# wildltr/ptranking

Measured on AMD Instinct MI355X. Metric: queries/sec fwd+bwd LambdaRank, MSLR-WEB30K-shaped list_len=128, higher is better.
Workload: dtype f32

## Files before the change

include/ptranking_amd.h:

```cpp
#ifndef PTRANKING_AMD_H
#define PTRANKING_AMD_H

#include <stddef.h>
#include <stdint.h>

#ifdef __cplusplus
extern "C" {
#endif

#define PTR_ABI_VERSION 8
#define PTR_MAX_LIST_LEN 4096
#define PTR_MAX_CUTOFFS 32
#define PTR_MAX_SUBTOPICS 32
#define PTR_MLP_ACT_LD 112

#define PTR_ERR_INVALID_ARG 1001
#define PTR_ERR_UNSUPPORTED 1002

#define PTR_LAMBDALOSS_NDCG_LOSS1 0
#define PTR_LAMBDALOSS_NDCG_LOSS2 1
#define PTR_LAMBDALOSS_NDCG_LOSS2PP 2

int ptr_abi_version(void);
const char *ptr_last_error(void);

int ptr_ranknet_fwd_bwd(const float *preds, const float *labels, const int32_t *lens, int B, int L, float sigma,
                        float *loss_out, float *loss_q, float *grad, void *stream);

int ptr_lambdarank_fwd_bwd(const float *preds, const float *labels, const int32_t *lens, int B, int L, float sigma,
                           float *loss_out, float *loss_q, float *grad, void *stream);

int ptr_lambdaloss_fwd_bwd(const float *preds, const float *labels, const int32_t *lens, int B, int L, int k,
                           float sigma, float mu, int loss_type, int presort, float *loss_out, float *loss_q,
                           float *grad, void *stream);

int ptr_softrank_fwd_bwd(const float *preds, const float *labels, const int32_t *lens, int B, int L, float delta, int top_k,
                         float *loss_out, float *loss_q, float *grad, void *stream);

int ptr_approxndcg_fwd_bwd(const float *preds, const float *labels, const int32_t *lens, int B, int L, float alpha,
                           int presort, int couple_batch, float grad_scale_override, float *loss_out, float *dcg_q,
                           float *inv_idcg_q, float *scale_out, float *grad, void *stream);

int ptr_listnet_fwd_bwd(const float *preds, const float *labels, const int32_t *lens, int B, int L, float *loss_out,
                        float *loss_q, float *grad, void *stream);

int ptr_stlistnet_fwd_bwd(const float *preds, const float *labels, const float *unif, const int32_t *lens, int B, int L,
                          float temperature, float *loss_out, float *loss_q, float *grad, void *stream);
int ptr_rankmse_fwd_bwd(const float *preds, const float *labels, const int32_t *lens, int B, int L, float *loss_out,
                        float *loss_q, float *grad, void *stream);
int ptr_rankcosine_fwd_bwd(const float *preds, const float *labels, const int32_t *lens, int B, int L, float *loss_out,
                           float *loss_q, float *grad, void *stream);

int ptr_listmle_fwd_bwd(const float *preds, const int64_t *perm, const int32_t *lens, int B, int L, float *loss_out,
                        float *loss_q, float *grad, void *stream);

int ptr_mdprank_fwd_bwd(const float *preds, const float *labels, const int64_t *perm, const int32_t *lens, int B, int L, int top_k,
                        float gamma, float *loss_out, float *loss_q, float *grad, void *stream);

#define PTR_WASS_COST_P1 0
#define PTR_WASS_COST_P2 1
#define PTR_WASS_COST_EG 2
#define PTR_WASS_COST_DG 3
#define PTR_WASS_COST_DDG 4

int ptr_wassrank_fwd_bwd(const float *preds, const float *labels, const int32_t *lens, int B, int L, int cost_type,
                         float gain_base, float non_rele_gap, float var_penalty, float lam, int sh_itr,
                         int scale_by_max_label, float *loss_out, float *loss_q, float *grad, void *stream);

#define PTR_ADCG_TOPK_SUBTOPICS 0
#define PTR_ADCG_TOPK_DOCUMENTS 1
int ptr_alphadcg_fwd_bwd(const float *preds, const float *rele, const int32_t *lens, const int32_t *ntopics, int B, int T, int L, float rt,
                         float alpha, int top_k, int top_k_axis, float *loss_out, float *loss_q, float *grad, void *stream);
int ptr_div_metrics_at_ks(const float *preds, const float *rele, const int32_t *lens, const int32_t *ntopics, int B, int T, int L,
                          const int32_t *ks, int nk, float alpha, float max_label, float *andcg, float *err_ia, float *nerr_ia,
                          int32_t *valid, void *stream);

#define PTR_DIVPROB_ANDCG 0
#define PTR_DIVPROB_ERRIA 1
#define PTR_DIVPROB_PAIRCLS 2
#define PTR_DIVPROB_LAMBDAPAIRCLS 3
int ptr_divprob_fwd_bwd(const float *mus, const float *vars, const float *rele, const int32_t *lens, const int32_t *ntopics, int B, int T, int L,
                        int objective, float beta, int top_k, int top_k_axis, float max_label, int norm, float *loss_out, float *loss_q,
                        float *grad_mu, float *grad_var, void *stream);
int ptr_divprob_expected_ranks(const float *mus, const float *vars, const int32_t *lens, int B, int L, float *ranks, void *stream);

#define PTR_TREE_PAIRS_ALL 0
#define PTR_TREE_PAIRS_NOTIES 1
#define PTR_TREE_PAIRS_NO00 2
#define PTR_TREE_PAIRS_00 3
#define PTR_TREE_W_NONE 0
#define PTR_TREE_W_DELTA_NDCG 1
#define PTR_TREE_W_DELTA_GAIN 2
#define PTR_TREE_HESS_REFERENCE 0
#define PTR_TREE_HESS_SUM 1
#define PTR_TREE_HESS_CONSTANT 2
#define PTR_TREE_GAIN_POWER 0
#define PTR_TREE_GAIN_LABEL 1
int ptr_tree_pair_grad_hess(const float *preds, const float *labels, const int64_t *offsets, int B, const int32_t *queries, int nq, int max_len,
                            int pair_type, int weighting, float epsilon, int hessian, float *grad, float *hess, void *stream);
int ptr_tree_listnet_grad_hess(const float *preds, const float *labels, const int64_t *offsets, int B, const int32_t *queries, int nq, int max_len,
                               int gain_type, int hessian, float *grad, float *hess, void *stream);

#define PTR_SMOOTH_P 0
#define PTR_SMOOTH_AP 1
#define PTR_SMOOTH_NERR 2
#define PTR_SMOOTH_NDCG 3
int ptr_smoothmetric_fwd_bwd(const float *preds, const float *labels, const int32_t *lens, int B, int L, int metric, int opt_ideal, int top_k,
                             float alpha, float max_label, float *loss_out, float *loss_q, float *valid_q, float *ranks, float *max_label_ws,
                             float *grad, void *stream);

#define PTR_PL_DIST_PL 0
#define PTR_PL_DIST_STPL 1
int ptr_pl_uniforms(int B, int L, int S, uint64_t seed, int64_t q0, float *unif, void *stream);
int ptr_pl_sample(const float *preds, const int32_t *lens, int B, int L, int S, float temperature, int distribution, uint64_t seed, int64_t q0,
                  const float *unif, int64_t *perm, float *action, void *stream);
int ptr_mdprank_sample_fwd_bwd(const float *preds, const float *labels, const int32_t *lens, int B, int L, int S, int top_k, float gamma,
                               float temperature, int distribution, uint64_t seed, int64_t q0, const float *unif, float *loss_out,
                               float *loss_q, float *grad, int64_t *perm_out, void *stream);

int ptr_shuffle_ties_order(const float *labels, const int32_t *lens, int B, int L, uint64_t seed, int64_t *perm,
                           void *stream);

int ptr_sort_desc(const float *preds, const int32_t *lens, int B, int L, float *vals, int64_t *idx, void *stream);

#define PTR_LABEL_MULTILABEL 0
#define PTR_LABEL_PERMUTATION 1
int ptr_metrics_at_ks(const float *preds, const float *labels, const int32_t *lens, int B, int L, const int32_t *ks,
                      int nk, int presort, int label_type, float max_label, float *max_label_ws, float *ndcg, float *nerr,
                      float *ap, float *prec, void *stream);

int ptr_sum_f32(const float *x, int n, float scale, float *out, void *stream);

size_t ptr_mlp_num_params(int F, int NL);
size_t ptr_mlp_backward_ws_floats(int F, int NL);
size_t ptr_mlp_backward_dz_floats(int R, int F, int NL);
size_t ptr_mlp_acts_floats(int R, int NL);
int ptr_mlp_forward(const float *X, const float *params, int R, int F, int NL, int train, float p_drop, uint64_t seed,
                    float *preds, float *acts, void *stream);
int ptr_mlp_backward(const float *X, const float *params, const float *acts, const float *dpreds, int R, int F, int NL,
                     float p_drop, uint64_t seed, float *dz, float *ws, float *grad, void *stream);
#define PTR_OPT_ADAM 1
#define PTR_OPT_ADAGRAD 2
#define PTR_OPT_RMSPROP 3
int ptr_mlp_backward_step(const float *X, float *params, const float *acts, const float *dpreds, int R, int F, int NL, float p_drop,
                          uint64_t seed, float *dz, float *ws, float *grad, int opt_kind, float lr, float hyper1, float hyper2, float eps,
                          float weight_decay, int step, float *state1, float *state2, const float *loss_q, int nq, float *loss_out,
                          void *stream);
int ptr_opt_step_loss(float *params, const float *grad, int64_t n, int opt_kind, float lr, float hyper1, float hyper2, float eps,
                      float weight_decay, int step, float *state1, float *state2, const float *loss_q, int nq, float *loss_out, void *stream);
int ptr_adam_step(float *param, const float *grad, float *exp_avg, float *exp_avg_sq, int64_t n, float lr, float beta1,
                  float beta2, float eps, float weight_decay, int step, void *stream);
int ptr_adagrad_step(float *param, const float *grad, float *state_sum, int64_t n, float lr, float lr_decay, float eps,
                     float weight_decay, int step, void *stream);
int ptr_rmsprop_step(float *param, const float *grad, float *square_avg, int64_t n, float lr, float alpha, float eps,
                     float weight_decay, void *stream);
size_t ptr_mlp_x6_ws_bytes(int F, int NL);
int ptr_mlp_forward_x6(const float *X, const float *params, int R, int F, int NL, int train, float p_drop, uint64_t seed,
                       float *preds, float *acts, void *wimg, void *stream);
#define PTR_LOSS_RANKNET 1
#define PTR_LOSS_LAMBDARANK 2
#define PTR_LOSS_LAMBDALOSS 3
#define PTR_LOSS_LISTNET 4
typedef struct ptr_train_step_desc {
    int32_t struct_bytes;
    int32_t loss_kind;
    int32_t B, L, F, NL;
    int32_t opt_kind, step;
    int32_t loss_i[4];
    float loss_f[4];
    float p_drop, lr, hyper1, hyper2, eps, weight_decay;
    uint64_t seed;
    const float *X, *labels;
    const int32_t *lens;
    float *params, *grad, *state1, *state2;
    float *preds, *acts, *loss_q, *dpreds, *dz, *ws;
    void *wimg;
    float *loss_out;
    void *events[4];
    int32_t wimg_current;
    int32_t reserved;
} ptr_train_step_desc;
int ptr_train_step(const ptr_train_step_desc *d, void *stream);
int ptr_mlp_dropout_mask(int R, int n_feat, int site, float p_drop, uint64_t seed, float *out, void *stream);

#define PTR_LINEAR_NONE 0
#define PTR_LINEAR_RELU 1
#define PTR_LINEAR_RELU_DROPOUT 2
#define PTR_LINEAR_GATE 3
int ptr_linear_forward(const float *X, int ldx, const float *W, const float *bias, int R, int K, int N, int act, float p_drop,
                       uint64_t seed, int site, float *Y, int ldy, void *stream);
int ptr_linear_backward_input(const float *dY, int ldy, const float *W, int R, int K, int N, const float *gate, int ldg, float p_drop,
                              float *dX, int ldx, void *stream);
size_t ptr_linear_backward_weight_ws_floats(int R, int K, int N);
int ptr_linear_backward_weight(const float *X, int ldx, const float *dY, int ldy, int R, int K, int N, float *ws, float *dW, float *db,
                               void *stream);
int ptr_dropout_apply(const float *x, int ldx, int R, int C, float p_drop, uint64_t seed, int site, float *out, int ldo, void *stream);
int ptr_relu_gate(const float *dy, const float *y, int64_t n, float *out, void *stream);

#define PTR_AF_NONE 0
#define PTR_AF_RELU 1
#define PTR_AF_LEAKY 2
#define PTR_AF_ELU 3
#define PTR_AF_SELU 4
#define PTR_AF_GELU 5
#define PTR_AF_SIGMOID 6
#define PTR_AF_TANH 7
size_t ptr_bn_ws_floats(int R, int N, int group_rows);
int ptr_bn_stats(const float *z, int ld, int R, int N, int group_rows, const int32_t *lens, int rows_per_query, float eps, float *ws,
                 float *mean, float *rstd, void *stream);
int ptr_bnact_forward(const float *z, int ld, int R, int N, int group_rows, const int32_t *lens, int rows_per_query, const float *mean,
                      const float *rstd, const float *gamma, const float *beta, int af, float p_drop, uint64_t seed, int site, float *out,
                      void *stream);
int ptr_bnact_backward(const float *z, const float *da, int ld, int R, int N, int group_rows, const int32_t *lens, int rows_per_query,
                       const float *mean, const float *rstd, const float *gamma, const float *beta, int af, float p_drop, uint64_t seed,
                       int site, float *ws, float *dz, float *dgamma, float *dbeta, void *stream);

size_t ptr_bn_slot_floats(int N);
int ptr_bn_stats_partial(const float *z, int ld, int R, int N, int group_rows, const int32_t *lens, int rows_per_query, float *ws,
                         float *slot, void *stream);
int ptr_bn_stats_combine(const float *slots, int W, int slot_stride, int N, float eps, float *mean, float *rstd, float *total_count,
                         void *stream);
int ptr_bnact_backward_sums(const float *z, const float *da, int ld, int R, int N, int group_rows, const int32_t *lens, int rows_per_query,
                            const float *mean, const float *rstd, const float *gamma, const float *beta, int af, float p_drop,
                            uint64_t seed, int site, float *ws, float *sums, void *stream);
int ptr_bnact_backward_apply(const float *z, const float *da, int ld, int R, int N, int group_rows, const int32_t *lens, int rows_per_query,
                             const float *mean, const float *rstd, const float *gamma, const float *beta, int af, float p_drop,
                             uint64_t seed, int site, const float *sums, int W, const float *total_count, float *ws, float *dz,
                             void *stream);

#define PTR_MHSA_MAX_HEAD_DIM 352
int ptr_mhsa_forward(const float *Q, const float *K, const float *V, int ld_qkv, const int32_t *lens, int B, int L, int F,
                     int n_heads, float p_drop, uint64_t seed, int site, float *O, float *lse, void *stream);
int ptr_mhsa_backward(const float *Q, const float *K, const float *V, int ld_qkv, const float *O, const float *dO, const float *lse,
                      const int32_t *lens, int B, int L, int F, int n_heads, float p_drop, uint64_t seed, int site, float *dvec,
                      float *dQ, float *dK, float *dV, float *ds_ws, void *stream);
int ptr_mhsa_dropout_mask(int B, int L, int n_heads, float p_drop, uint64_t seed, int site, float *out, void *stream);
int ptr_layernorm_forward(const float *X, const float *a2, const float *b2, int64_t R, int F, float eps, float *Y, float *stats,
                          void *stream);
size_t ptr_layernorm_backward_ws_floats(int F);
int ptr_layernorm_backward(const float *X, const float *a2, const float *dY, const float *stats, int64_t R, int F, float *ws,
                           float *dX, float *da2, float *db2, void *stream);

int ptr_letor_scan(const char *path, int one_indexed, int64_t *n_docs, int32_t *n_features, int64_t *n_queries);
int ptr_letor_load(const char *path, int one_indexed, float missing, int64_t n_docs, int32_t n_features, int64_t n_queries,
                   void *X, int x_is_f64, float *y, int64_t *qids, int64_t *qoff);

#ifdef __cplusplus
}
#endif
#endif
```

ptranking_amd/_lib.py:

```python
import ctypes as C
import os

import torch

_PKG = os.path.dirname(os.path.abspath(__file__))
LIB_PATH = os.environ.get("PTR_LIB") or os.path.join(_PKG, "libptranking_amd.so")

ABI_VERSION = 8
MAX_LIST_LEN = 4096
MAX_CUTOFFS = 32
MAX_SUBTOPICS = 32

_vp, _i, _f, _u64 = C.c_void_p, C.c_int, C.c_float, C.c_uint64

SIGNATURES = {
    "ptr_abi_version": [],
    "ptr_last_error": [],
    "ptr_ranknet_fwd_bwd": [_vp, _vp, _vp, _i, _i, _f, _vp, _vp, _vp, _vp],
    "ptr_lambdarank_fwd_bwd": [_vp, _vp, _vp, _i, _i, _f, _vp, _vp, _vp, _vp],
    "ptr_lambdaloss_fwd_bwd": [_vp, _vp, _vp, _i, _i, _i, _f, _f, _i, _i, _vp, _vp, _vp, _vp],
    "ptr_approxndcg_fwd_bwd": [_vp, _vp, _vp, _i, _i, _f, _i, _i, _f, _vp, _vp, _vp, _vp, _vp, _vp],
    "ptr_softrank_fwd_bwd": [_vp, _vp, _vp, _i, _i, _f, _i, _vp, _vp, _vp, _vp],
    "ptr_listnet_fwd_bwd": [_vp, _vp, _vp, _i, _i, _vp, _vp, _vp, _vp],
    "ptr_mdprank_fwd_bwd": [_vp, _vp, _vp, _vp, _i, _i, _i, _f, _vp, _vp, _vp, _vp],
    "ptr_listmle_fwd_bwd": [_vp, _vp, _vp, _i, _i, _vp, _vp, _vp, _vp],
    "ptr_stlistnet_fwd_bwd": [_vp, _vp, _vp, _vp, _i, _i, _f, _vp, _vp, _vp, _vp],
    "ptr_rankmse_fwd_bwd": [_vp, _vp, _vp, _i, _i, _vp, _vp, _vp, _vp],
    "ptr_rankcosine_fwd_bwd": [_vp, _vp, _vp, _i, _i, _vp, _vp, _vp, _vp],
    "ptr_wassrank_fwd_bwd": [_vp, _vp, _vp, _i, _i, _i, _f, _f, _f, _f, _i, _i, _vp, _vp, _vp, _vp],
    "ptr_alphadcg_fwd_bwd": [_vp, _vp, _vp, _vp, _i, _i, _i, _f, _f, _i, _i, _vp, _vp, _vp, _vp],
    "ptr_div_metrics_at_ks": [_vp, _vp, _vp, _vp, _i, _i, _i, C.POINTER(C.c_int32), _i, _f, _f, _vp, _vp, _vp, _vp, _vp],
    "ptr_divprob_fwd_bwd": [_vp, _vp, _vp, _vp, _vp, _i, _i, _i, _i, _f, _i, _i, _f, _i, _vp, _vp, _vp, _vp, _vp],
    "ptr_divprob_expected_ranks": [_vp, _vp, _vp, _i, _i, _vp, _vp],
    "ptr_tree_pair_grad_hess": [_vp, _vp, _vp, _i, _vp, _i, _i, _i, _i, _f, _i, _vp, _vp, _vp],
    "ptr_tree_listnet_grad_hess": [_vp, _vp, _vp, _i, _vp, _i, _i, _i, _i, _vp, _vp, _vp],
    "ptr_smoothmetric_fwd_bwd": [_vp, _vp, _vp, _i, _i, _i, _i, _i, _f, _f, _vp, _vp, _vp, _vp, _vp, _vp, _vp],
    "ptr_pl_uniforms": [_i, _i, _i, _u64, C.c_int64, _vp, _vp],
    "ptr_pl_sample": [_vp, _vp, _i, _i, _i, _f, _i, _u64, C.c_int64, _vp, _vp, _vp, _vp],
    "ptr_mdprank_sample_fwd_bwd": [_vp, _vp, _vp, _i, _i, _i, _i, _f, _f, _i, _u64, C.c_int64, _vp, _vp, _vp, _vp, _vp, _vp],
    "ptr_shuffle_ties_order": [_vp, _vp, _i, _i, _u64, _vp, _vp],
    "ptr_sort_desc": [_vp, _vp, _i, _i, _vp, _vp, _vp],
    "ptr_metrics_at_ks": [_vp, _vp, _vp, _i, _i, C.POINTER(C.c_int32), _i, _i, _i, _f, _vp, _vp, _vp, _vp, _vp, _vp],
    "ptr_sum_f32": [_vp, _i, _f, _vp, _vp],
    "ptr_mlp_num_params": [_i, _i],
    "ptr_mlp_backward_ws_floats": [_i, _i],
    "ptr_mlp_backward_dz_floats": [_i, _i, _i],
    "ptr_mlp_acts_floats": [_i, _i],
    "ptr_mlp_forward": [_vp, _vp, _i, _i, _i, _i, _f, _u64, _vp, _vp, _vp],
    "ptr_mlp_backward": [_vp, _vp, _vp, _vp, _i, _i, _i, _f, _u64, _vp, _vp, _vp, _vp],
    "ptr_mlp_backward_step": [_vp, _vp, _vp, _vp, _i, _i, _i, _f, _u64, _vp, _vp, _vp, _i, _f, _f, _f, _f, _f, _i, _vp, _vp, _vp, _i, _vp, _vp],
    "ptr_opt_step_loss": [_vp, _vp, C.c_int64, _i, _f, _f, _f, _f, _f, _i, _vp, _vp, _vp, _i, _vp, _vp],
    "ptr_train_step": [_vp, _vp],
    "ptr_mlp_x6_ws_bytes": [_i, _i],
    "ptr_mlp_forward_x6": [_vp, _vp, _i, _i, _i, _i, _f, _u64, _vp, _vp, _vp, _vp],
    "ptr_adam_step": [_vp, _vp, _vp, _vp, C.c_int64, _f, _f, _f, _f, _f, _i, _vp],
    "ptr_adagrad_step": [_vp, _vp, _vp, C.c_int64, _f, _f, _f, _f, _i, _vp],
    "ptr_rmsprop_step": [_vp, _vp, _vp, C.c_int64, _f, _f, _f, _f, _vp],
    "ptr_mlp_dropout_mask": [_i, _i, _i, _f, _u64, _vp, _vp],
    "ptr_linear_forward": [_vp, _i, _vp, _vp, _i, _i, _i, _i, _f, _u64, _i, _vp, _i, _vp],
    "ptr_linear_backward_input": [_vp, _i, _vp, _i, _i, _i, _vp, _i, _f, _vp, _i, _vp],
    "ptr_linear_backward_weight_ws_floats": [_i, _i, _i],
    "ptr_linear_backward_weight": [_vp, _i, _vp, _i, _i, _i, _i, _vp, _vp, _vp, _vp],
    "ptr_bn_ws_floats": [_i, _i, _i],
    "ptr_bn_stats": [_vp, _i, _i, _i, _i, _vp, _i, _f, _vp, _vp, _vp, _vp],
    "ptr_bnact_forward": [_vp, _i, _i, _i, _i, _vp, _i, _vp, _vp, _vp, _vp, _i, _f, _u64, _i, _vp, _vp],
    "ptr_bnact_backward": [_vp, _vp, _i, _i, _i, _i, _vp, _i, _vp, _vp, _vp, _vp, _i, _f, _u64, _i, _vp, _vp, _vp, _vp, _vp],
    "ptr_bn_slot_floats": [_i],
    "ptr_bn_stats_partial": [_vp, _i, _i, _i, _i, _vp, _i, _vp, _vp, _vp],
    "ptr_bn_stats_combine": [_vp, _i, _i, _i, _f, _vp, _vp, _vp, _vp],
    "ptr_bnact_backward_sums": [_vp, _vp, _i, _i, _i, _i, _vp, _i, _vp, _vp, _vp, _vp, _i, _f, _u64, _i, _vp, _vp, _vp],
    "ptr_bnact_backward_apply": [_vp, _vp, _i, _i, _i, _i, _vp, _i, _vp, _vp, _vp, _vp, _i, _f, _u64, _i, _vp, _i, _vp, _vp, _vp, _vp],
    "ptr_dropout_apply": [_vp, _i, _i, _i, _f, _u64, _i, _vp, _i, _vp],
    "ptr_relu_gate": [_vp, _vp, C.c_int64, _vp, _vp],
    "ptr_mhsa_forward": [_vp, _vp, _vp, _i, _vp, _i, _i, _i, _i, _f, _u64, _i, _vp, _vp, _vp],
    "ptr_mhsa_backward": [_vp, _vp, _vp, _i, _vp, _vp, _vp, _vp, _i, _i, _i, _i, _f, _u64, _i, _vp, _vp, _vp, _vp, _vp, _vp],
    "ptr_mhsa_dropout_mask": [_i, _i, _i, _f, _u64, _i, _vp, _vp],
    "ptr_layernorm_forward": [_vp, _vp, _vp, C.c_int64, _i, _f, _vp, _vp, _vp],
    "ptr_layernorm_backward_ws_floats": [_i],
    "ptr_layernorm_backward": [_vp, _vp, _vp, _vp, C.c_int64, _i, _vp, _vp, _vp, _vp, _vp],
    "ptr_letor_scan": [C.c_char_p, _i, _vp, _vp, _vp],
    "ptr_letor_load": [C.c_char_p, _i, _f, C.c_int64, C.c_int32, C.c_int64, _vp, _i, _vp, _vp, _vp],
}
_RESTYPES = {"ptr_last_error": C.c_char_p, "ptr_mlp_num_params": C.c_size_t, "ptr_mlp_backward_ws_floats": C.c_size_t,
             "ptr_mlp_backward_dz_floats": C.c_size_t, "ptr_mlp_acts_floats": C.c_size_t, "ptr_mlp_x6_ws_bytes": C.c_size_t, "ptr_linear_backward_weight_ws_floats": C.c_size_t, "ptr_bn_ws_floats": C.c_size_t,
             "ptr_bn_slot_floats": C.c_size_t,
             "ptr_layernorm_backward_ws_floats": C.c_size_t}
OPTIONAL = set()

_lib = None


class Loss:

    def __init__(self, entry, kind, params=()):
        self.entry, self.kind, self.params = entry, kind, tuple(params)

    def c_args(self, **values):
        return [C.c_float(float(values[n])) if t is _f else int(values[n]) for n, t in self.params]

    def desc_arrays(self, **values):
        return (tuple(int(values[n]) for n, t in self.params if t is _i), tuple(C.c_float(float(values[n])).value for n, t in self.params if t is _f))


LOSSES = {
    "ranknet": Loss("ptr_ranknet_fwd_bwd", 1, [("sigma", _f)]),
    "lambdarank": Loss("ptr_lambdarank_fwd_bwd", 2, [("sigma", _f)]),
    "lambdaloss": Loss("ptr_lambdaloss_fwd_bwd", 3, [("k", _i), ("sigma", _f), ("mu", _f), ("loss_type", _i), ("presort", _i)]),
    "listnet": Loss("ptr_listnet_fwd_bwd", 4),
}


class TrainStepDesc(C.Structure):
    _fields_ = [("struct_bytes", C.c_int32), ("loss_kind", C.c_int32),
                ("B", C.c_int32), ("L", C.c_int32), ("F", C.c_int32), ("NL", C.c_int32),
                ("opt_kind", C.c_int32), ("step", C.c_int32),
                ("loss_i", C.c_int32 * 4), ("loss_f", C.c_float * 4),
                ("p_drop", C.c_float), ("lr", C.c_float), ("hyper1", C.c_float), ("hyper2", C.c_float), ("eps", C.c_float), ("weight_decay", C.c_float),
                ("seed", C.c_uint64),
                ("X", C.c_void_p), ("labels", C.c_void_p), ("lens", C.c_void_p),
                ("params", C.c_void_p), ("grad", C.c_void_p), ("state1", C.c_void_p), ("state2", C.c_void_p),
                ("preds", C.c_void_p), ("acts", C.c_void_p), ("loss_q", C.c_void_p), ("dpreds", C.c_void_p), ("dz", C.c_void_p), ("ws", C.c_void_p),
                ("wimg", C.c_void_p), ("loss_out", C.c_void_p), ("events", C.c_void_p * 4), ("wimg_current", C.c_int32), ("reserved", C.c_int32)]


class NativeLibraryError(RuntimeError):
    pass


def load():
    global _lib
    if _lib is not None:
        return _lib
    if not os.path.exists(LIB_PATH):
        raise NativeLibraryError(
            f"{LIB_PATH} is missing: build the HIP extension first (python -m ptranking_amd.build, or "
            f"__graft_entry__.build()).  ptranking_amd has no CPU / eager fallback by design.")
    lib = C.CDLL(LIB_PATH, mode=C.RTLD_GLOBAL)
    for name, argtypes in SIGNATURES.items():
        try:
            fn = getattr(lib, name)
        except AttributeError:
            if name in OPTIONAL:
                continue
            raise NativeLibraryError(f"{LIB_PATH} does not export {name}; rebuild it")
        fn.argtypes = argtypes
        fn.restype = _RESTYPES.get(name, C.c_int)
    v = lib.ptr_abi_version()
    if v != ABI_VERSION:
        raise NativeLibraryError(f"ABI version mismatch: library {v}, binding {ABI_VERSION}")
    _lib = lib
    return lib


def has(name):
    return hasattr(load(), name)


TIMING = None


def query(name, *args):
    return getattr(load(), name)(*args)


def call(name, *args):
    lib = load()
    if TIMING is not None:
        ev0, ev1 = torch.cuda.Event(enable_timing=True), torch.cuda.Event(enable_timing=True)
        ev0.record()
        rc = getattr(lib, name)(*args)
        ev1.record()
        TIMING.setdefault(name, []).append((ev0, ev1))
    else:
        rc = getattr(lib, name)(*args)
    if rc != 0:
        msg = lib.ptr_last_error()
        raise RuntimeError(f"{name} failed (code {rc}): {msg.decode() if msg else ''}")


def ptr(t):
    return None if t is None else C.c_void_p(t.data_ptr())


def current_stream(device):
    return C.c_void_p(torch.cuda.current_stream(device).cuda_stream)
```

ptranking_amd/csrc/ptr_mlp.h:

```cpp
#pragma once
#include <stdlib.h>
#include <utility>

#include "ptr_device.h"
#include "ptr_dropout.h"
#include "ptr_x6.h"

namespace ptr {

constexpr int kH = 100;
constexpr int kHP = 112;
constexpr int kMT = 7;
constexpr int kMaxLayers = 8;
constexpr int kAL = 112;
constexpr int kActTile = 16 * kAL;
__host__ __device__ inline int act_row_tiles(int R) { return (R + 15) >> 4; }
__host__ __device__ inline size_t act_layer_floats(int R) { return (size_t)act_row_tiles(R) * kActTile; }
__host__ __device__ inline size_t act_off(int row, int col) {
    return (size_t)(row >> 4) * kActTile + (size_t)(((col >> 4) << 8) + ((row & 15) << 4) + (col & 15));
}

__host__ __device__ inline size_t off_W(int l, int F) { return l == 0 ? 0 : (size_t)kH * F + kH + (size_t)(l - 1) * (kH * kH + kH); }
__host__ __device__ inline size_t off_b(int l, int F) { return off_W(l, F) + (l == 0 ? (size_t)kH * F : (size_t)kH * kH); }
__host__ __device__ inline size_t off_wout(int NL, int F) { return off_W(NL, F); }
__host__ __device__ inline size_t n_params(int NL, int F) { return off_wout(NL, F) + kH + 1; }

struct MlpArgs {
    int R, F, NL;
    float p_drop;
    uint32_t seed_lo, seed_hi;
};

constexpr int kX6Rows = kHP;
constexpr int kX6PlaneBytes = kX6Rows * 32 * 2;
constexpr int kX6SliceBytes = 3 * kX6PlaneBytes;
__host__ __device__ inline int x6_n1(int F) { return (F + 31) / 32; }
__host__ __device__ inline int x6_nslices(int F, int NL) { return x6_n1(F) + 4 * (NL - 1); }
#if defined(__HIPCC__)
__device__ __forceinline__ void x6_img_put(uint8_t *__restrict__ img, int F, int NL, size_t i, float x) {
    const size_t w1 = (size_t)kH * F;
    int sl, row, g, e;
    if (i < w1) {
        row = (int)(i / F);
        const int k = (int)(i - (size_t)row * F), kk = k & 31;
        sl = k >> 5; g = kk >> 3; e = kk & 7;
    } else {
        if (i < w1 + kH) return;
        const size_t jv = i - (w1 + kH);
        const int l = 1 + (int)(jv / (kH * kH + kH));
        if (l > NL - 1) return;
        const int jj = (int)(jv - (size_t)(l - 1) * (kH * kH + kH));
        int k;
        if (jj < kH * kH) { row = jj / kH; k = jj - row * kH; } else { row = jj - kH * kH; k = kH; }
        const int kk = k & 31;
        sl = x6_n1(F) + 4 * (l - 1) + (k >> 5);
        g = (kk & 15) >> 2; e = 4 * (kk >> 4) + (kk & 3);
    }
    uint16_t p1, p2, p3;
    split_pack1(x, p1, p2, p3);
    uint8_t *at = img + (size_t)sl * kX6SliceBytes + (size_t)(row >> 4) * 1024 + g * 256 + (row & 15) * 16 + e * 2;
    *reinterpret_cast<uint16_t *>(at) = p1;
    *reinterpret_cast<uint16_t *>(at + kX6PlaneBytes) = p2;
    *reinterpret_cast<uint16_t *>(at + 2 * kX6PlaneBytes) = p3;
}
#endif

template <int N, class Fn> __device__ __forceinline__ void static_for(Fn &&f) {
    [&]<int... I>(std::integer_sequence<int, I...>) { (f(std::integral_constant<int, I>{}), ...); }(std::make_integer_sequence<int, N>{});
}

bool bwd_fused_supported(int F, int NL, const void *X, const void *acts);
int bwd_fused_grid(int R);
int launch_bwd_fused(const float *X, const float *params, const float *acts, const float *dpreds, const MlpArgs &a, float *ws,
                     hipStream_t st, const char *who);

bool bwd_tail_supported(int NL, const void *acts);
int launch_bwd_tail(const float *params, const float *acts, const float *dpreds, const MlpArgs &a, float *ws, float *dz0, hipStream_t st,
                    const char *who);

bool bwd_x6_supported(int R, int F, int NL, const void *X, const void *acts);
int launch_bwd_x6(const float *X, const float *params, const float *acts, const float *dpreds, const MlpArgs &a, float *ws, hipStream_t st,
                  const char *who);

bool bwd_x6_tail_supported(int R, int NL, const void *acts);
int launch_bwd_x6_tail(const float *params, const float *acts, const float *dpreds, const MlpArgs &a, float *ws, float *dz0, hipStream_t st,
                       const char *who);

bool dw_x6_supported(int R, int K, int lda, const void *A);
int launch_dw_x6(const float *A, int lda, const float *dZ, int K, int ntk, const MlpArgs &a, float *ws, size_t np_stride, size_t w_off, size_t b_off,
                 int nblk, hipStream_t st, const char *who);

int mlp_forward_x6_impl(const float *X, const float *params, int R, int F, int NL, int train, float p_drop, uint64_t seed, float *preds, float *acts,
                        void *wimg, bool prep, void *stream);
int mlp_backward_step_impl(const float *X, float *params, const float *acts, const float *dpreds, int R, int F, int NL, float p_drop, uint64_t seed, float *dz,
                           float *ws, float *grad, int opt_kind, float lr, float hyper1, float hyper2, float eps, float weight_decay, int step, float *state1,
                           float *state2, const float *loss_q, int nq, float *loss_out, void *wimg, void *stream);

}
```

ptranking_amd/csrc/scorer.hip:

```cpp
#include "ptr_mlp.h"

namespace ptr {

__host__ __device__ inline int ld_w1(int F) { return (F + 3) / 4 * 4 + 4; }


constexpr int kTailNone = 0, kTailSpread = 1, kTailReplicate = 2;
__device__ __forceinline__ void stage_matrix(float *dst, int ld, const float *src, int rows, int cols, bool transpose, int tid, int nthr,
                                             int tail = kTailNone) {
    constexpr int U = 8;
    const int n = rows * cols;
    const bool vec = ((cols & 3) == 0) && ((reinterpret_cast<uintptr_t>(src) & 15) == 0);
    const int reps = tail == kTailReplicate ? 4 : 1;
    if (vec) {
        const int n4 = n >> 2;
        for (int base = tid; base < n4; base += U * nthr) {
            f32x4 v[U];
#pragma unroll
            for (int u = 0; u < U; ++u) {
                const int i4 = base + u * nthr;
                v[u] = *reinterpret_cast<const f32x4 *>(src + 4 * (size_t)(i4 < n4 ? i4 : n4 - 1));
            }
#pragma unroll
            for (int u = 0; u < U; ++u) {
                const int i4 = base + u * nthr;
                if (i4 < n4) {
                    const int idx = 4 * i4, r = idx / cols, c = idx - r * cols;
                    if (!transpose) {
                        for (int rep = 0; rep < (r >= 96 ? reps : 1); ++rep) *reinterpret_cast<f32x4 *>(dst + (size_t)(r + 4 * rep) * ld + c) = v[u];
                    } else {
#pragma unroll
                        for (int e = 0; e < 4; ++e) dst[(size_t)(c + e) * ld + r] = v[u][e];
                    }
                }
            }
        }
    } else {
        for (int base = tid; base < n; base += U * nthr) {
            float v[U];
#pragma unroll
            for (int u = 0; u < U; ++u) { const int idx = base + u * nthr; v[u] = src[idx < n ? idx : n - 1]; }
#pragma unroll
            for (int u = 0; u < U; ++u) {
                const int idx = base + u * nthr;
                if (idx < n) {
                    const int r = idx / cols, c = idx - r * cols;
                    if (transpose) dst[(size_t)c * ld + r] = v[u];
                    else for (int rep = 0; rep < (r >= 96 ? reps : 1); ++rep) dst[(size_t)(r + 4 * rep) * ld + c] = v[u];
                }
            }
        }
    }
    const int vr = transpose ? cols : rows, vc = transpose ? rows : cols;
    for (int idx = tid; idx < kHP * ld; idx += nthr) {
        const int r = idx / ld, c = idx - r * ld;
        const bool real_row = (tail == kTailReplicate && r >= 96) ? 96 + ((r - 96) & 3) < vr : r < vr;
        if (!real_row || c >= vc) dst[idx] = 0.0f;
    }
}
__device__ __forceinline__ void stage_vector(float *dst, const float *src, int n, int tid, int nthr, int tail = kTailNone) {
    for (int i = tid; i < kHP; i += nthr) {
        if (tail != kTailSpread || i < 96) dst[i] = i < n ? src[i] : 0.0f;
        else dst[i] = (((i - 96) & 3) == 0 && 96 + ((i - 96) >> 2) < n) ? src[96 + ((i - 96) >> 2)] : 0.0f;
    }
}

constexpr int kSlabK = 48, kSlabLd = kSlabK + 4;
__host__ __device__ inline size_t fwd_lds_floats(int F, int NL, int w1_mode) {
    const size_t w1 = w1_mode == 0 ? (size_t)kHP * ld_w1(F) : (w1_mode == 2 ? (size_t)2 * kHP * kSlabLd : 0);
    return w1 + (size_t)(NL - 1) * kHP * kH + (size_t)NL * kHP + kHP + 16;
}
__host__ __device__ inline int fwd_w1_mode(int F, int NL) {
    if (fwd_lds_floats(F, NL, 0) * sizeof(float) <= 160 * 1024) return 0;
    return fwd_lds_floats(F, NL, 2) * sizeof(float) <= 160 * 1024 ? 2 : 1;
}

#ifdef PTR_FWD_TRACE
#define FWD_STAMP(i) do { if (blockIdx.x == 0 && lane == 0 && ntile_done < 8) { unsigned long long *tr_ = reinterpret_cast<unsigned long long *>(preds + ((R + 3) & ~3) + 4) + (ntile_done * 16 + wave) * 8; tr_[(i)] = clock64(); if ((i) == 0) tr_[4] = wall_clock64(); if ((i) == 3) tr_[5] = wall_clock64(); } } while (0)
#else
#define FWD_STAMP(i) do { } while (0)
#endif

template <int RT, int NTHR, bool TRAIN, bool VEC, int W1G>
__global__ void __launch_bounds__(NTHR)
mlp_fwd_kernel(const float *__restrict__ X, const float *__restrict__ P, MlpArgs a, float *__restrict__ preds,
               float *__restrict__ acts) {
    extern __shared__ __attribute__((aligned(16))) float smem[];
    const int F = a.F, NL = a.NL, R = a.R, ld1 = ld_w1(F), R16 = act_row_tiles(a.R) * 16;
    float *W1s = smem;
    float *Wh = W1s + (W1G == 0 ? (size_t)kHP * ld1 : (W1G == 2 ? (size_t)2 * kHP * kSlabLd : 0));
    float *Bs = Wh + (size_t)(NL - 1) * kHP * kH;
    float *Wo = Bs + (size_t)NL * kHP;
    const int tid = threadIdx.x, nthr = blockDim.x;
    if constexpr (W1G == 0) stage_matrix(W1s, ld1, P + off_W(0, F), kH, F, false, tid, nthr, kTailReplicate);
    for (int l = 1; l < NL; ++l) stage_matrix(Wh + (size_t)(l - 1) * kHP * kH, kH, P + off_W(l, F), kH, kH, false, tid, nthr, kTailReplicate);
    for (int l = 0; l < NL; ++l) stage_vector(Bs + (size_t)l * kHP, P + off_b(l, F), kH, tid, nthr);
    stage_vector(Wo, P + off_wout(NL, F), kH, tid, nthr, kTailSpread);
    if (tid < 16) Wo[kHP + tid] = tid == 0 ? P[off_wout(NL, F) + kH] : 0.0f;
    __syncthreads();
    const float b_out = Wo[kHP];

    const int lane = tid & 63, j = lane & 15, g = lane >> 4;
    const int wpb = nthr >> 6, wave = tid >> 6;
    const int rows_per_tile = 16 * RT;
    const int ntiles = (R + rows_per_tile - 1) / rows_per_tile;
    const uint32_t thr = drop_thr(a.p_drop);
    const float scale = TRAIN ? 1.0f / (1.0f - a.p_drop) : 1.0f;
    const int nS1 = (F + 15) >> 4;

    int ntile_done = 0;
    (void)ntile_done;
    auto prefetch_first = [&](int t, f32x4 (&xb)[RT]) {
        const int tt = t < ntiles ? t : ntiles - 1;
        const int k0 = 4 * g;
#pragma unroll
        for (int rt = 0; rt < RT; ++rt) {
            const int r = tt * rows_per_tile + 16 * rt + j;
            const float *xr = X + (size_t)(r < R ? r : R - 1) * F;
            if constexpr (VEC) {
                xb[rt] = *reinterpret_cast<const f32x4 *>(xr + (k0 < F ? k0 : 0));
            } else {
#pragma unroll
                for (int c = 0; c < 4; ++c) xb[rt][c] = xr[k0 + c < F ? k0 + c : 0];
            }
        }
    };
    f32x4 xpre[RT];
    constexpr bool kQueue = W1G != 2;
    const int tiles_per_block = (ntiles + gridDim.x - 1) / gridDim.x;
    const int tile_lo = kQueue ? blockIdx.x * tiles_per_block : 0, tile_hi = kQueue ? min(ntiles, tile_lo + tiles_per_block) : ntiles;
    int *queue = reinterpret_cast<int *>(Wo + kHP + 8);
    int tile = blockIdx.x * wpb + wave;
    if constexpr (kQueue) {
        if (tid == 0) *queue = tile_lo + wpb;
        __syncthreads();
        tile = tile_lo + wave;
    }
    constexpr int kSlabV = kHP * (kSlabK / 4);
    constexpr int kSlabU = (kSlabV + NTHR - 1) / NTHR;
    f32x4 slab_r[W1G == 2 ? kSlabU : 1];
    int slab_buf = 0;
    auto slab_load = [&](int sl) {
        if constexpr (W1G == 2) {
#pragma unroll
            for (int u = 0; u < kSlabU; ++u) {
                const int i4 = tid + u * NTHR, r = i4 / (kSlabK / 4), c = 4 * (i4 - r * (kSlabK / 4));
                const int wr = r < 96 ? r : 96 + ((r - 96) & 3), k = kSlabK * sl + c;
                slab_r[u] = *reinterpret_cast<const f32x4 *>(P + (size_t)(wr < kHP ? wr : 0) * F + (k < F ? k : 0));
            }
        }
    };
    auto slab_store = [&](int sl, int buf) {
        if constexpr (W1G == 2) {
#pragma unroll
            for (int u = 0; u < kSlabU; ++u) {
                const int i4 = tid + u * NTHR, r = i4 / (kSlabK / 4), c = 4 * (i4 - r * (kSlabK / 4));
                const bool real = kSlabK * sl + c < F;
                f32x4 v = slab_r[u];
                if (!real) v = f32x4{0.f, 0.f, 0.f, 0.f};
                if (i4 < kSlabV) *reinterpret_cast<f32x4 *>(W1s + (size_t)buf * kHP * kSlabLd + (size_t)r * kSlabLd + c) = v;
            }
        }
    };
    if constexpr (W1G == 2) { slab_load(0); slab_store(0, 0); }
    prefetch_first(tile, xpre);
    for (; (kQueue ? tile : tile - wave) < tile_hi; ++ntile_done) {
        int next_tile = tile_hi;
        auto advance = [&]() {
            if constexpr (kQueue) {
                int nxt = 0;
                if (lane == 0) nxt = atomicAdd(queue, 1);
                next_tile = __builtin_amdgcn_readfirstlane(nxt);
            } else {
                next_tile = tile + gridDim.x * wpb;
            }
            prefetch_first(next_tile, xpre);
        };
        const int row0 = tile * rows_per_tile;
        const bool tile_full = row0 + rows_per_tile <= R;
        int row[RT];
#pragma unroll
        for (int rt = 0; rt < RT; ++rt) row[rt] = row0 + 16 * rt + j;
        FWD_STAMP(0);

        const float *xrow[RT];
        bool rok[RT];
#pragma unroll
        for (int rt = 0; rt < RT; ++rt) {
            rok[rt] = row[rt] < R;
            xrow[rt] = X + (size_t)(rok[rt] ? row[rt] : R - 1) * F;
        }
        auto load_raw = [&](int S, f32x4 (&xb)[RT]) {
            const int k0 = 16 * S + 4 * g;
#pragma unroll
            for (int rt = 0; rt < RT; ++rt) {
                if constexpr (VEC) {
                    xb[rt] = *reinterpret_cast<const f32x4 *>(xrow[rt] + (k0 < F ? k0 : 0));
                } else {
#pragma unroll
                    for (int c = 0; c < 4; ++c) xb[rt][c] = xrow[rt][k0 + c < F ? k0 + c : 0];
                }
            }
        };
        auto finish_x = [&](int S, f32x4 (&xb)[RT]) {
            const int k0 = 16 * S + 4 * g;
#pragma unroll
            for (int rt = 0; rt < RT; ++rt) {
                f32x4 v = xb[rt];
                if (16 * S + 16 > F || !tile_full) {
#pragma unroll
                    for (int c = 0; c < 4; ++c) v[c] *= ((k0 + c < F) && rok[rt]) ? 1.0f : 0.0f;
                }
                if constexpr (TRAIN) {
                    uint32_t w0, w1;
                    drop_bits(a.seed_lo, a.seed_hi, 0, row[rt], k0 >> 2, w0, w1);
                    v = drop4(v, w0, w1, thr, scale);
                }
                xb[rt] = v;
            }
        };

        auto tail_store = [&](float v, float ones) -> f32x4 {
            const float h1 = __shfl(v, j + 16, 64), h2 = __shfl(v, j + 32, 64), h3 = __shfl(v, j + 48, 64);
            f32x4 o = f32x4{g == 1 ? ones : 0.0f, 0.0f, 0.0f, 0.0f};
            if (g == 0) o = f32x4{v, h1, h2, h3};
            return o;
        };
        auto mma = [&](auto mt_, float aop, float bop, f32x4 c) -> f32x4 {
            if constexpr (decltype(mt_)::value == kMT - 1) return __builtin_amdgcn_mfma_f32_4x4x1f32(aop, bop, c, 0, 0, 0);
            else return __builtin_amdgcn_mfma_f32_16x16x4f32(aop, bop, c, 0, 0, 0);
        };
        f32x4 acc[kMT][RT];
        auto tile6_finish = [&]() {
#pragma unroll
            for (int rt = 0; rt < RT; ++rt) {
                f32x4 t = acc[kMT - 1][rt];
#pragma unroll
                for (int c = 0; c < 4; ++c) { t[c] += __shfl_xor(t[c], 16, 64); t[c] += __shfl_xor(t[c], 32, 64); }
                acc[kMT - 1][rt][0] = g == 0 ? t[0] : (g == 1 ? t[1] : (g == 2 ? t[2] : t[3]));
            }
        };
        auto mma_tiles = [&](const f32x4 (&wa)[kMT], const f32x4 (&b)[RT], int nc) {
            auto one = [&]<int MT>(std::integral_constant<int, MT> mt_, int c) {
#pragma unroll
                for (int rt = 0; rt < RT; ++rt) acc[MT][rt] = mma(mt_, wa[MT][c], b[rt][c], acc[MT][rt]);
            };
            using std::integral_constant;
#pragma unroll
            for (int c = 0; c < 4; ++c) if (c < nc) { one(integral_constant<int, 0>{}, c); one(integral_constant<int, 1>{}, c); }
#pragma unroll
            for (int c = 0; c < 4; ++c) if (c < nc) { one(integral_constant<int, 2>{}, c); one(integral_constant<int, 3>{}, c); }
#pragma unroll
            for (int c = 0; c < 4; ++c) if (c < nc) { one(integral_constant<int, 4>{}, c); one(integral_constant<int, 5>{}, c); one(integral_constant<int, 6>{}, c); }
        };
        auto bias_init = [&](const float *b) {
#pragma unroll
            for (int mt = 0; mt < kMT; ++mt) {
                f32x4 b4 = *reinterpret_cast<const f32x4 *>(b + (mt < kMT - 1 ? 16 * mt + 4 * g : 96));
                if (mt == kMT - 1) { const float on = g == 0 ? 1.0f : 0.0f; b4 = b4 * on; }
#pragma unroll
                for (int rt = 0; rt < RT; ++rt) acc[mt][rt] = b4;
            }
        };
        bias_init(Bs);
        f32x4 xa[RT], xb[RT], xc[RT];
#pragma unroll
        for (int rt = 0; rt < RT; ++rt) xa[rt] = xpre[rt];
        if (NL == 1) advance();
        finish_x(0, xa);
        auto read_w1 = [&](int S, int sin, int mt) -> f32x4 {
            const int k0 = 16 * S + 4 * g;
            if constexpr (W1G == 2) {
                return *reinterpret_cast<const f32x4 *>(W1s + (size_t)slab_buf * kHP * kSlabLd + (size_t)(16 * mt + j) * kSlabLd + 16 * sin + 4 * g);
            } else if constexpr (W1G == 1) {
                const int wr = mt < kMT - 1 ? 16 * mt + j : 96 + (j & 3);
                return *reinterpret_cast<const f32x4 *>(P + (size_t)wr * F + (k0 < F ? k0 : 0));
            } else {
                return *reinterpret_cast<const f32x4 *>(W1s + (size_t)(16 * mt + j) * ld1 + k0);
            }
        };
        auto l1_step = [&](int S, int sin, f32x4 (&cur)[RT], f32x4 (&nxt)[RT], f32x4 (&nn)[RT]) {
            load_raw(S + 2 < nS1 ? S + 2 : 0, nn);
            __builtin_amdgcn_sched_barrier(0);
            f32x4 wa[kMT];
#pragma unroll
            for (int mt = 0; mt < kMT; ++mt) wa[mt] = read_w1(S, sin, mt);
            if constexpr (RT > 1) __builtin_amdgcn_sched_barrier(0);
            mma_tiles(wa, cur, 4);
            finish_x(S + 1, nxt);
        };
        auto slab_enter = [&](int S) {
            if constexpr (W1G == 2) {
                __syncthreads();
                slab_load(S + 3 < nS1 ? S / 3 + 1 : 0);
            }
        };
        auto slab_leave = [&](int S) {
            if constexpr (W1G == 2) {
                slab_store(S + 3 < nS1 ? S / 3 + 1 : 0, slab_buf ^ 1);
                slab_buf ^= 1;
            }
        };
        load_raw(nS1 > 1 ? 1 : 0, xb);
        int S1 = 0;
        for (; S1 + 3 <= nS1; S1 += 3) {
            slab_enter(S1);
            l1_step(S1, 0, xa, xb, xc);
            l1_step(S1 + 1, 1, xb, xc, xa);
            l1_step(S1 + 2, 2, xc, xa, xb);
            slab_leave(S1);
        }
        const int left = nS1 - S1;
        if (left == 0) {
        } else if (left == 1) {
            slab_enter(S1);
            l1_step(S1, 0, xa, xb, xc);
            slab_leave(S1);
        } else {
            slab_enter(S1);
            l1_step(S1, 0, xa, xb, xc);
            l1_step(S1 + 1, 1, xb, xc, xa);
            slab_leave(S1);
        }
        tile6_finish();

        FWD_STAMP(1);
        for (int l = 1; l < NL; ++l) {
            f32x4 hin[kMT][RT];
#pragma unroll
            for (int mt = 0; mt < kMT; ++mt)
#pragma unroll
                for (int rt = 0; rt < RT; ++rt) {
                    f32x4 h = acc[mt][rt];
#pragma unroll
                    for (int c = 0; c < 4; ++c) h[c] = fmaxf(h[c], 0.0f);
                    if constexpr (TRAIN) {
                        if (mt < kMT - 1) {
                            uint32_t w0, w1;
                            drop_bits(a.seed_lo, a.seed_hi, l, row[rt], 4 * mt + g, w0, w1);
                            h = drop4(h, w0, w1, thr, scale);
                        } else {
                            h[0] *= drop_keep1(a.seed_lo, a.seed_hi, l, row[rt], 96 + g, thr) ? scale : 0.0f;
                        }
                    }
                    hin[mt][rt] = h;
                }
            if (l == NL - 1) advance();
            const float *Wl = Wh + (size_t)(l - 1) * kHP * kH;
            bias_init(Bs + (size_t)l * kHP);
#pragma unroll
            for (int S = 0; S < kMT; ++S) {
                constexpr int kLast = kMT - 1;
                f32x4 wa[kMT];
#pragma unroll
                for (int mt = 0; mt < kMT; ++mt) {
                    const float *wp = Wl + (size_t)(16 * mt + j) * kH;
                    if (S < kLast) wa[mt] = *reinterpret_cast<const f32x4 *>(wp + 16 * S + 4 * g);
                    else wa[mt] = f32x4{wp[96 + g], 0.0f, 0.0f, 0.0f};
                }
                if constexpr (RT > 1) __builtin_amdgcn_sched_barrier(0);
                if constexpr (TRAIN) {
#pragma unroll
                    for (int rt = 0; rt < RT; ++rt) {
                        if (row[rt] < R16) {
                            float *arow = acts + (size_t)(l - 1) * act_layer_floats(R) + act_off(row[rt], 0);
                            *reinterpret_cast<f32x4 *>(arow + 256 * S + 4 * g) = S < kLast ? hin[S][rt] : tail_store(hin[S][rt][0], 1.0f);
                        }
                    }
                    if constexpr (RT > 1) __builtin_amdgcn_sched_barrier(0);
                }
                mma_tiles(wa, hin[S], S < kLast ? 4 : 1);
            }
            tile6_finish();
        }

        FWD_STAMP(2);
        float sc[RT];
#pragma unroll
        for (int rt = 0; rt < RT; ++rt) sc[rt] = 0.0f;
#pragma unroll
        for (int mt = 0; mt < kMT; ++mt) {
            const f32x4 w4 = *reinterpret_cast<const f32x4 *>(Wo + 16 * mt + 4 * g);
#pragma unroll
            for (int rt = 0; rt < RT; ++rt) {
                f32x4 h = acc[mt][rt];
#pragma unroll
                for (int c = 0; c < (mt == kMT - 1 ? 1 : 4); ++c) { h[c] = fmaxf(h[c], 0.0f); sc[rt] = fmaf(h[c], w4[c], sc[rt]); }
                if constexpr (TRAIN) {
                    if (row[rt] < R16) {
                        float *arow = acts + (size_t)(NL - 1) * act_layer_floats(R) + act_off(row[rt], 0);
                        *reinterpret_cast<f32x4 *>(arow + 256 * mt + 4 * g) = mt < kMT - 1 ? h : tail_store(h[0], 0.0f);
                    }
                }
            }
        }
#pragma unroll
        for (int rt = 0; rt < RT; ++rt) {
            float s = sc[rt];
            s += __shfl_xor(s, 16, 64);
            s += __shfl_xor(s, 32, 64);
            if (g == 0 && row[rt] < R) preds[row[rt]] = s + b_out;
        }
        FWD_STAMP(3);
        tile = next_tile;
    }
}

__host__ __device__ inline size_t dz_lds_floats(int NL) { return (size_t)(NL - 1) * kHP * kH + (kHP + 16) + 16 * (kHP + 16); }

template <int RT, int NTHR>
__global__ void __launch_bounds__(NTHR)
mlp_bwd_dz_kernel(const float *__restrict__ P, const float *__restrict__ acts, const float *__restrict__ dpreds, MlpArgs a,
                  float *__restrict__ dz, float *__restrict__ ws, size_t np_stride, size_t wout_off) {
    extern __shared__ __attribute__((aligned(16))) float smem[];
    const int F = a.F, NL = a.NL, R = a.R;
    float *WT = smem;
    float *Wo = WT + (size_t)(NL - 1) * kHP * kH;
    float *wrow = Wo + kHP + 16;
    const int tid = threadIdx.x, nthr = blockDim.x;
    for (int l = 1; l < NL; ++l) stage_matrix(WT + (size_t)(l - 1) * kHP * kH, kH, P + off_W(l, F), kH, kH, true, tid, nthr);
    stage_vector(Wo, P + off_wout(NL, F), kH, tid, nthr);
    if (tid < 16) Wo[kHP + tid] = 0.0f;
    __syncthreads();

    const int lane = tid & 63, j = lane & 15, g = lane >> 4;
    const int wpb = nthr >> 6, wave = tid >> 6;
    const int rows_per_tile = 16 * RT;
    const int ntiles = (R + rows_per_tile - 1) / rows_per_tile;
    const float inv_keep = a.p_drop > 0.0f ? 1.0f / (1.0f - a.p_drop) : 1.0f;

    f32x4 dwo[kMT];
#pragma unroll
    for (int mt = 0; mt < kMT; ++mt) dwo[mt] = f32x4{0.f, 0.f, 0.f, 0.f};
    float dbo = 0.0f;

    f32x4 hpf[kMT][RT];
    float dspf[RT];
    auto prefetch_top = [&](int tile) {
#pragma unroll
        for (int rt = 0; rt < RT; ++rt) {
            const int r = tile * rows_per_tile + 16 * rt + j;
            const int rc = r < R ? r : R - 1;
            dspf[rt] = dpreds[rc];
#pragma unroll
            for (int mt = 0; mt < kMT; ++mt)
                hpf[mt][rt] = *reinterpret_cast<const f32x4 *>(acts + (size_t)(NL - 1) * act_layer_floats(R) + act_off(rc, 16 * mt + 4 * g));
        }
    };
    const int tile_first = blockIdx.x * wpb + wave, tile_step = gridDim.x * wpb;
    if (tile_first < ntiles) prefetch_top(tile_first);
    for (int tile = tile_first; tile < ntiles; tile += tile_step) {
        const int row0 = tile * rows_per_tile;
        int row[RT];
        float ds[RT];
        f32x4 htop[kMT][RT];
#pragma unroll
        for (int rt = 0; rt < RT; ++rt) {
            row[rt] = row0 + 16 * rt + j;
            ds[rt] = dspf[rt] * (row[rt] < R ? 1.0f : 0.0f);
            if (g == 0) dbo += ds[rt];
#pragma unroll
            for (int mt = 0; mt < kMT; ++mt) htop[mt][rt] = hpf[mt][rt];
        }
        if (tile + tile_step < ntiles) prefetch_top(tile + tile_step);
        f32x4 cur[kMT][RT];
#pragma unroll
        for (int mt = 0; mt < kMT; ++mt) {
            const f32x4 w4 = *reinterpret_cast<const f32x4 *>(Wo + 16 * mt + 4 * g);
#pragma unroll
            for (int rt = 0; rt < RT; ++rt) {
                const bool ok = row[rt] < R;
                const size_t o = ((size_t)(NL - 1) * R + row[rt]) * kAL + 16 * mt + 4 * g;
                f32x4 h = htop[mt][rt];
                const float okf = ok ? 1.0f : 0.0f;
#pragma unroll
                for (int c = 0; c < 4; ++c) h[c] *= okf;
                f32x4 d;
#pragma unroll
                for (int c = 0; c < 4; ++c) { d[c] = (ds[rt] * w4[c]) * (h[c] > 0.0f ? 1.0f : 0.0f); dwo[mt][c] = fmaf(h[c], ds[rt], dwo[mt][c]); }
                if (ok) *reinterpret_cast<f32x4 *>(dz + o) = d;
                cur[mt][rt] = d;
            }
        }
        for (int l = NL - 1; l >= 1; --l) {
            const float *Wl = WT + (size_t)(l - 1) * kHP * kH;
            f32x4 gate[kMT][RT];
#pragma unroll
            for (int mt = 0; mt < kMT; ++mt)
#pragma unroll
                for (int rt = 0; rt < RT; ++rt) {
                    const bool ok = row[rt] < R;
                    const size_t o = (size_t)(l - 1) * act_layer_floats(R) + act_off(row[rt], 16 * mt + 4 * g);
                    gate[mt][rt] = *reinterpret_cast<const f32x4 *>(acts + (ok ? o : 0));
                }
            f32x4 acc[kMT][RT];
#pragma unroll
            for (int mt = 0; mt < kMT; ++mt)
#pragma unroll
                for (int rt = 0; rt < RT; ++rt) acc[mt][rt] = f32x4{0.f, 0.f, 0.f, 0.f};
#pragma unroll
            for (int S = 0; S < kMT; ++S) {
                f32x4 wa[kMT];
#pragma unroll
                for (int mt = 0; mt < kMT; ++mt) wa[mt] = *reinterpret_cast<const f32x4 *>(Wl + (size_t)(16 * mt + j) * kH + 16 * S + 4 * g);
                auto group = [&](int m0, int m1) {
#pragma unroll
                    for (int c = 0; c < 4; ++c)
#pragma unroll
                        for (int mt = m0; mt < m1; ++mt)
#pragma unroll
                            for (int rt = 0; rt < RT; ++rt)
                                acc[mt][rt] = __builtin_amdgcn_mfma_f32_16x16x4f32(wa[mt][c], cur[S][rt][c], acc[mt][rt], 0, 0, 0);
                };
                group(0, 2); group(2, 4); group(4, kMT);
            }
#pragma unroll
            for (int mt = 0; mt < kMT; ++mt)
#pragma unroll
                for (int rt = 0; rt < RT; ++rt) {
                    const bool ok = row[rt] < R;
                    const size_t o = ((size_t)(l - 1) * R + row[rt]) * kAL + 16 * mt + 4 * g;
                    f32x4 d;
#pragma unroll
                    for (int c = 0; c < 4; ++c) d[c] = acc[mt][rt][c] * ((ok && gate[mt][rt][c] > 0.0f) ? inv_keep : 0.0f);
                    if (ok) *reinterpret_cast<f32x4 *>(dz + o) = d;
                    cur[mt][rt] = d;
                }
        }
    }
#pragma unroll
    for (int mt = 0; mt < kMT; ++mt)
#pragma unroll
        for (int c = 0; c < 4; ++c) {
            float v = dwo[mt][c];
            v += __shfl_xor(v, 1, 64); v += __shfl_xor(v, 2, 64); v += __shfl_xor(v, 4, 64); v += __shfl_xor(v, 8, 64);
            if (j == 0) wrow[(size_t)wave * (kHP + 16) + 16 * mt + 4 * g + c] = v;
        }
    {
        float v = dbo;
        v += __shfl_xor(v, 1, 64); v += __shfl_xor(v, 2, 64); v += __shfl_xor(v, 4, 64); v += __shfl_xor(v, 8, 64);
        if (lane == 0) wrow[(size_t)wave * (kHP + 16) + kHP] = v;
    }
    __syncthreads();
    for (int i = tid; i < kH + 1; i += nthr) {
        const int src = i < kH ? i : kHP;
        float s = 0.0f;
        for (int w = 0; w < wpb; ++w) s += wrow[(size_t)w * (kHP + 16) + src];
        ws[(size_t)blockIdx.x * np_stride + wout_off + i] = s;
    }
}

template <int NTW, bool SITE0, int NWV>
__global__ void __launch_bounds__(NWV * 64)
mlp_bwd_dw_kernel(const float *__restrict__ A, int lda, const float *__restrict__ dZ, int K, int nt_base, MlpArgs a,
                  float *__restrict__ ws, size_t np_stride, size_t w_off, size_t b_off) {
    const int R = a.R;
    const int tid = threadIdx.x, lane = tid & 63, j = lane & 15, g = lane >> 4, wave = tid >> 6;
    constexpr int U = 4;
    const int chunk = ((R + gridDim.x - 1) / gridDim.x + 4 * U - 1) / (4 * U) * (4 * U);
    const int r_begin = blockIdx.x * chunk, r_end = min(R, r_begin + chunk);
    const uint32_t thr = drop_thr(a.p_drop);
    const float scale = (SITE0 && a.p_drop > 0.0f) ? 1.0f / (1.0f - a.p_drop) : 1.0f;
    const int ntk = (K + 15) >> 4;
    (void)ntk;

    f32x4 acc[NTW][kMT];
#pragma unroll
    for (int t = 0; t < NTW; ++t)
#pragma unroll
        for (int mt = 0; mt < kMT; ++mt) acc[t][mt] = f32x4{0.f, 0.f, 0.f, 0.f};
    float dbv[kMT];
#pragma unroll
    for (int mt = 0; mt < kMT; ++mt) dbv[mt] = 0.0f;

    int fa[kMT], kb[NTW];
    bool fa_ok[kMT], kb_ok[NTW];
#pragma unroll
    for (int mt = 0; mt < kMT; ++mt) { const int f = 16 * mt + j; fa_ok[mt] = true; fa[mt] = f; }
#pragma unroll
    for (int t = 0; t < NTW; ++t) { const int k = 16 * (nt_base + wave + NWV * t) + j; kb_ok[t] = k < K; kb[t] = kb_ok[t] ? k : 0; }
    float av[U][kMT], bv[U][NTW], avn[U][kMT], bvn[U][NTW];
    auto load = [&](int r0, bool guard, float (&pa)[U][kMT], float (&pb)[U][NTW]) {
#pragma unroll
        for (int u = 0; u < U; ++u) {
            const int r = r0 + 4 * u + g;
            const bool rok = !guard || r < r_end;
            const int rc = rok ? r : r_end - 1;
            const float *dzr = dZ + (size_t)rc * kAL;
            const float *ar = SITE0 ? A + (size_t)rc * lda : A + act_off(rc, 0);
#pragma unroll
            for (int mt = 0; mt < kMT; ++mt) pa[u][mt] = dzr[fa[mt]] * ((rok & fa_ok[mt]) ? 1.0f : 0.0f);
#pragma unroll
            for (int t = 0; t < NTW; ++t) {
                float v = SITE0 ? ar[kb[t]] : ar[((kb[t] >> 4) << 8) + (kb[t] & 15)];
                bool keep = rok & kb_ok[t];
                if constexpr (SITE0) keep = keep & drop_keep1(a.seed_lo, a.seed_hi, 0, rc, kb[t], thr);
                pb[u][t] = v * (keep ? scale : 0.0f);
            }
        }
    };
    auto mma = [&]() {
#pragma unroll
        for (int u = 0; u < U; ++u) {
#pragma unroll
            for (int mt = 0; mt < kMT; ++mt) dbv[mt] += av[u][mt];
#pragma unroll
            for (int t = 0; t < NTW; ++t)
#pragma unroll
                for (int mt = 0; mt < kMT; ++mt)
                    acc[t][mt] = __builtin_amdgcn_mfma_f32_16x16x4f32(av[u][mt], bv[u][t], acc[t][mt], 0, 0, 0);
        }
    };
    const int n_full = r_end > r_begin ? (r_end - r_begin) / (4 * U) : 0;
    int r0 = r_begin;
    if (n_full > 0) {
        load(r0, false, av, bv);
        for (int it = 0; it < n_full; ++it, r0 += 4 * U) {
            if (it + 1 < n_full) load(r0 + 4 * U, false, avn, bvn);
            mma();
#pragma unroll
            for (int u = 0; u < U; ++u) {
#pragma unroll
                for (int mt = 0; mt < kMT; ++mt) av[u][mt] = avn[u][mt];
#pragma unroll
                for (int t = 0; t < NTW; ++t) bv[u][t] = bvn[u][t];
            }
        }
    }
    if (r0 < r_end) { load(r0, true, av, bv); mma(); }
    float *out = ws + (size_t)blockIdx.x * np_stride + w_off;
    float *outb = ws + (size_t)blockIdx.x * np_stride + b_off;
#pragma unroll
    for (int t = 0; t < NTW; ++t) {
        const int nt = nt_base + wave + NWV * t, k = 16 * nt + j;
#pragma unroll
        for (int mt = 0; mt < kMT; ++mt)
#pragma unroll
            for (int c = 0; c < 4; ++c) {
                const int o = 16 * mt + 4 * g + c;
                if (nt < ntk && k < K && o < kH) out[(size_t)o * K + k] = acc[t][mt][c];
            }
    }
    if (wave == 0 && nt_base == 0) {
#pragma unroll
        for (int mt = 0; mt < kMT; ++mt) {
            float v = dbv[mt];
            v += __shfl_xor(v, 16, 64);
            v += __shfl_xor(v, 32, 64);
            const int f = 16 * mt + j;
            if (g == 0 && f < kH) outb[f] = v;
        }
    }
}

template <int NTW, bool SITE0, int RB>
__global__ void __launch_bounds__(256)
mlp_bwd_dw_lds_kernel(const float *__restrict__ A, int lda, const float *__restrict__ dZ, int K, int nt_base, MlpArgs a,
                      float *__restrict__ ws, size_t np_stride, size_t w_off, size_t b_off) {
    constexpr int WA4 = 16 * NTW;
    constexpr int LDA = 64 * NTW + 16;
    constexpr int LDZ = kAL;
    constexpr int SA = RB * WA4 / 256;
    constexpr int SZ = (RB * (kAL / 4) + 255) / 256;
    extern __shared__ __attribute__((aligned(16))) float smem[];
    auto zb = [&](int b) -> float * { return smem + b * (RB * LDZ); };
    auto ab = [&](int b) -> float * { return smem + 2 * RB * LDZ + b * (RB * LDA); };

    const int R = a.R;
    const int tid = threadIdx.x, lane = tid & 63, j = lane & 15, g = lane >> 4, wave = tid >> 6;
    const int chunk = ((R + gridDim.x - 1) / gridDim.x + RB - 1) / RB * RB;
    const int r_begin = blockIdx.x * chunk, r_end = min(R, r_begin + chunk);
    const uint32_t thr = drop_thr(a.p_drop);
    const float scale = (SITE0 && a.p_drop > 0.0f) ? 1.0f / (1.0f - a.p_drop) : 1.0f;
    const int col0 = 16 * nt_base;

    int a_row[SA], a_col[SA], z_row[SZ], z_col[SZ];
    bool a_ok[SA], z_ok[SZ];
#pragma unroll
    for (int s_ = 0; s_ < SA; ++s_) {
        const int idx = s_ * 256 + tid;
        a_row[s_] = idx / WA4;
        a_col[s_] = col0 + 4 * (idx % WA4);
        a_ok[s_] = a_col[s_] < K;
    }
#pragma unroll
    for (int s_ = 0; s_ < SZ; ++s_) {
        const int idx = s_ * 256 + tid;
        z_ok[s_] = idx < RB * (kAL / 4);
        z_row[s_] = z_ok[s_] ? idx / (kAL / 4) : 0;
        z_col[s_] = z_ok[s_] ? 4 * (idx % (kAL / 4)) : 0;
    }
    f32x4 ra[SA], rz[SZ];
    auto gload = [&](int r0) {
#pragma unroll
        for (int s_ = 0; s_ < SA; ++s_) {
            const int r = r0 + a_row[s_];
            const int rc = r < r_end ? r : r_end - 1;
            const int cc = a_ok[s_] ? a_col[s_] : 0;
            ra[s_] = *reinterpret_cast<const f32x4 *>(SITE0 ? A + (size_t)rc * lda + cc : A + act_off(rc, cc));
        }
#pragma unroll
        for (int s_ = 0; s_ < SZ; ++s_) {
            const int r = r0 + z_row[s_];
            const int rc = r < r_end ? r : r_end - 1;
            rz[s_] = *reinterpret_cast<const f32x4 *>(dZ + (size_t)rc * kAL + z_col[s_]);
        }
    };
    auto lstore = [&](int buf, int r0) {
#pragma unroll
        for (int s_ = 0; s_ < SA; ++s_) {
            const int r = r0 + a_row[s_];
            const bool rok = r < r_end;
            f32x4 v = ra[s_];
            if constexpr (SITE0) {
                uint32_t w0, w1;
                drop_bits(a.seed_lo, a.seed_hi, 0, rok ? r : r_end - 1, a_col[s_] >> 2, w0, w1);
                v = drop4(v, w0, w1, thr, scale);
            }
            const float okf = (rok & a_ok[s_]) ? 1.0f : 0.0f;
#pragma unroll
            for (int c = 0; c < 4; ++c) v[c] *= okf;
            *reinterpret_cast<f32x4 *>(ab(buf) + a_row[s_] * LDA + (a_col[s_] - col0)) = v;
        }
#pragma unroll
        for (int s_ = 0; s_ < SZ; ++s_) {
            if (z_ok[s_]) {
                const float okf = (r0 + z_row[s_] < r_end) ? 1.0f : 0.0f;
                f32x4 v = rz[s_];
#pragma unroll
                for (int c = 0; c < 4; ++c) v[c] *= okf;
                *reinterpret_cast<f32x4 *>(zb(buf) + z_row[s_] * LDZ + z_col[s_]) = v;
            }
        }
    };

    f32x4 acc[NTW][kMT];
#pragma unroll
    for (int t = 0; t < NTW; ++t)
#pragma unroll
        for (int mt = 0; mt < kMT; ++mt) acc[t][mt] = f32x4{0.f, 0.f, 0.f, 0.f};
    float dbv[kMT];
#pragma unroll
    for (int mt = 0; mt < kMT; ++mt) dbv[mt] = 0.0f;

    if (r_begin < r_end) {
        gload(r_begin);
        lstore(0, r_begin);
    }
    __syncthreads();
    int buf = 0;
    for (int r0 = r_begin; r0 < r_end; r0 += RB, buf ^= 1) {
        const bool more = r0 + RB < r_end;
        if (more) gload(r0 + RB);
        const float *zs = zb(buf), *as = ab(buf);
#pragma unroll
        for (int u = 0; u < RB / 4; ++u) {
            float av[kMT], bv[NTW];
#pragma unroll
            for (int mt = 0; mt < kMT; ++mt) { av[mt] = zs[(4 * u + g) * LDZ + 16 * mt + j]; dbv[mt] += av[mt]; }
#pragma unroll
            for (int t = 0; t < NTW; ++t) bv[t] = as[(4 * u + g) * LDA + 16 * (wave + 4 * t) + j];
#pragma unroll
            for (int t = 0; t < NTW; ++t)
#pragma unroll
                for (int mt = 0; mt < kMT; ++mt)
                    acc[t][mt] = __builtin_amdgcn_mfma_f32_16x16x4f32(av[mt], bv[t], acc[t][mt], 0, 0, 0);
        }
        if (more) lstore(buf ^ 1, r0 + RB);
        __syncthreads();
    }
    float *out = ws + (size_t)blockIdx.x * np_stride + w_off;
    float *outb = ws + (size_t)blockIdx.x * np_stride + b_off;
#pragma unroll
    for (int t = 0; t < NTW; ++t) {
        const int k = col0 + 16 * (wave + 4 * t) + j;
#pragma unroll
        for (int mt = 0; mt < kMT; ++mt)
#pragma unroll
            for (int c = 0; c < 4; ++c) {
                const int o = 16 * mt + 4 * g + c;
                if (k < K && o < kH) out[(size_t)o * K + k] = acc[t][mt][c];
            }
    }
    if (wave == 0 && nt_base == 0) {
#pragma unroll
        for (int mt = 0; mt < kMT; ++mt) {
            float v = dbv[mt];
            v += __shfl_xor(v, 16, 64);
            v += __shfl_xor(v, 32, 64);
            const int f = 16 * mt + j;
            if (g == 0 && f < kH) outb[f] = v;
        }
    }
}
__host__ __device__ constexpr size_t dw_lds_bytes(int NTW, int RB) { return (size_t)(2 * RB * kAL + 2 * RB * (64 * NTW + 16)) * sizeof(float); }

struct OptStep {
    int kind;
    float lr, h1, h2, eps, wd, bc1, bc2_sqrt;
    float *param, *s1, *s2;
    const float *loss_q; int nq; float *loss_out;
    uint8_t *wimg; int F, NL;
};
__global__ void __launch_bounds__(1024)
reduce_partials_kernel(const float *__restrict__ ws, int nblk, int nblk_tail, size_t tail_begin, size_t stride, size_t n,
                       float *__restrict__ grad, OptStep o) {
    __shared__ float part[16][64];
    const int lane = threadIdx.x & 63, w = threadIdx.x >> 6;
    if (o.loss_out && blockIdx.x == gridDim.x - 1) {
        const float tot = block1024_sum(o.loss_q, o.nq, &part[0][0]);
        if (threadIdx.x == 0) o.loss_out[0] = tot;
        return;
    }
    const size_t i = (size_t)blockIdx.x * 64 + lane;
    const bool ok = i < n;
    const size_t ic = ok ? i : n - 1;
    const int nb = ic >= tail_begin ? nblk_tail : nblk;
    float s0 = 0.f, s1 = 0.f, s2 = 0.f, s3 = 0.f;
    int b = w;
    for (; b + 48 < nb; b += 64) {
        s0 += ws[(size_t)b * stride + ic];
        s1 += ws[(size_t)(b + 16) * stride + ic];
        s2 += ws[(size_t)(b + 32) * stride + ic];
        s3 += ws[(size_t)(b + 48) * stride + ic];
    }
    for (; b < nb; b += 16) s0 += ws[(size_t)b * stride + ic];
    part[w][lane] = (s0 + s1) + (s2 + s3);
    __syncthreads();
    if (w == 0 && ok) {
        float s = part[0][lane];
#pragma unroll
        for (int k = 1; k < 16; ++k) s += part[k][lane];
        if (grad) grad[i] = s;
        if (o.kind == PTR_OPT_ADAM) {
            const float pi = o.param[i];
            const float gi = s + o.wd * pi;
            const float mi = o.h1 * o.s1[i] + (1.0f - o.h1) * gi;
            const float vi = o.h2 * o.s2[i] + (1.0f - o.h2) * gi * gi;
            o.s1[i] = mi; o.s2[i] = vi;
            const float denom = sqrtf(vi) / o.bc2_sqrt + o.eps;
            const float pn = pi - (o.lr / o.bc1) * (mi / denom);
            o.param[i] = pn;
            if (o.wimg) x6_img_put(o.wimg, o.F, o.NL, i, pn);
        } else if (o.kind == PTR_OPT_ADAGRAD) {
            const float pi = o.param[i];
            const float gi = s + o.wd * pi;
            const float si = o.s1[i] + gi * gi;
            o.s1[i] = si;
            const float pn = pi - o.lr * (gi / (sqrtf(si) + o.eps));
            o.param[i] = pn;
            if (o.wimg) x6_img_put(o.wimg, o.F, o.NL, i, pn);
        } else if (o.kind == PTR_OPT_RMSPROP) {
            const float pi = o.param[i];
            const float gi = s + o.wd * pi;
            const float si = o.h1 * o.s1[i] + (1.0f - o.h1) * gi * gi;
            o.s1[i] = si;
            const float pn = pi - o.lr * (gi / (sqrtf(si) + o.eps));
            o.param[i] = pn;
            if (o.wimg) x6_img_put(o.wimg, o.F, o.NL, i, pn);
        }
    }
}

__global__ void __launch_bounds__(256)
adam_kernel(float *__restrict__ p, const float *__restrict__ grad, float *__restrict__ m, float *__restrict__ v, size_t n, float lr,
            float b1, float b2, float eps, float wd, float bc1, float bc2_sqrt) {
    const size_t i = (size_t)blockIdx.x * 256 + threadIdx.x;
    if (i >= n) return;
    const float pi = p[i];
    const float gi = grad[i] + wd * pi;
    const float mi = b1 * m[i] + (1.0f - b1) * gi;
    const float vi = b2 * v[i] + (1.0f - b2) * gi * gi;
    m[i] = mi; v[i] = vi;
    const float denom = sqrtf(vi) / bc2_sqrt + eps;
    p[i] = pi - (lr / bc1) * (mi / denom);
}

__global__ void __launch_bounds__(256)
dropout_mask_kernel(MlpArgs a, int site, int n_feat, float *__restrict__ out) {
    const size_t i = (size_t)blockIdx.x * 256 + threadIdx.x;
    if (i >= (size_t)a.R * n_feat) return;
    const int row = (int)(i / n_feat), k = (int)(i % n_feat);
    out[i] = drop_keep1(a.seed_lo, a.seed_hi, site, row, k, drop_thr(a.p_drop)) ? 1.0f : 0.0f;
}

static int check_mlp(const char *who, int R, int F, int NL, float p) {
    if (R < 0 || F <= 0 || NL < 1 || NL > kMaxLayers) { set_error("%s: bad shape R=%d F=%d NL=%d", who, R, F, NL); return PTR_ERR_INVALID_ARG; }
    if (!(p >= 0.0f && p < 1.0f)) { set_error("%s: dropout p=%g out of [0,1)", who, (double)p); return PTR_ERR_INVALID_ARG; }
    const int w1g = fwd_w1_mode(F, NL);
    if (fwd_lds_floats(F, NL, w1g) * sizeof(float) > 160 * 1024 || (w1g && F % 4 != 0) || (F + 15) / 16 > 48) {
        set_error("%s: F=%d with %d hidden layers is outside the fused scorer's range (LDS %zu KB, max 160; F %% 4 == 0 needed "
                  "above ~157 features; F <= 768)", who, F, NL, fwd_lds_floats(F, NL, w1g) * sizeof(float) / 1024);
        return PTR_ERR_UNSUPPORTED;
    }
    return 0;
}

constexpr int kDwBlocksPerCu = 2;
constexpr int kDwRB = 16;

}

extern "C" size_t ptr_mlp_num_params(int F, int NL) { return ptr::n_params(NL, F); }

extern "C" size_t ptr_mlp_backward_ws_floats(int F, int NL) {
    return (size_t)ptr::kDwBlocksPerCu * ptr::num_cus() * ptr::n_params(NL, F);
}

extern "C" size_t ptr_mlp_acts_floats(int R, int NL) { return R > 0 && NL > 0 ? (size_t)NL * ptr::act_layer_floats(R) : 0; }
extern "C" size_t ptr_mlp_backward_dz_floats(int R, int F, int NL) {
    return ptr::bwd_fused_supported(F, NL, nullptr, nullptr) ? 0 : (size_t)NL * (size_t)R * ptr::kAL;
}

extern "C" int ptr_mlp_forward(const float *X, const float *params, int R, int F, int NL, int train, float p_drop, uint64_t seed,
                               float *preds, float *acts, void *stream) {
    using namespace ptr;
    const char *who = "ptr_mlp_forward";
    if (int rc = check_mlp(who, R, F, NL, p_drop)) return rc;
    if (R > 0 && (!X || !params || !preds || (train && !acts))) { set_error("%s: NULL pointer", who); return PTR_ERR_INVALID_ARG; }
    if (R == 0) return 0;
    MlpArgs a{R, F, NL, train ? p_drop : 0.0f, (uint32_t)seed, (uint32_t)(seed >> 32)};
    const int w1g = fwd_w1_mode(F, NL);
    const size_t lds = fwd_lds_floats(F, NL, w1g) * sizeof(float);
    const bool vec = (F % 4 == 0) && ((reinterpret_cast<uintptr_t>(X) & 15) == 0);
    const bool wide = train && !w1g;
    const int rows_per_tile = wide ? 16 : 32, wpb = wide ? 16 : 8;
    const int ntiles = (R + rows_per_tile - 1) / rows_per_tile;
    const int grid = ntiles < num_cus() ? ntiles : num_cus();
    auto launch = [&](auto kern) -> int {
        if (int e = allow_lds(kern, lds)) return e;
        hipLaunchKernelGGL(kern, dim3(grid > 0 ? grid : 1), dim3(wpb * 64), lds, as_stream(stream), X, params, a, preds, acts);
        return check_hip(hipGetLastError(), who);
    };
    if (w1g) {
        if (!vec) { set_error("%s: X must be 16-byte aligned for F=%d", who, F); return PTR_ERR_INVALID_ARG; }
        if (w1g == 2 && !env_int("PTR_FWD_W1_STREAM", 0))
            return train ? launch(mlp_fwd_kernel<2, 512, true, true, 2>) : launch(mlp_fwd_kernel<2, 512, false, true, 2>);
        return train ? launch(mlp_fwd_kernel<2, 512, true, true, 1>) : launch(mlp_fwd_kernel<2, 512, false, true, 1>);
    }
    if (wide) return vec ? launch(mlp_fwd_kernel<1, 1024, true, true, 0>) : launch(mlp_fwd_kernel<1, 1024, true, false, 0>);
    return vec ? launch(mlp_fwd_kernel<2, 512, false, true, 0>) : launch(mlp_fwd_kernel<2, 512, false, false, 0>);
}

namespace ptr {
int mlp_backward_impl(const char *who, const float *X, const float *params, const float *acts, const float *dpreds, int R, int F, int NL,
                             float p_drop, uint64_t seed, float *dz, float *ws, float *grad, void *stream, const OptStep &opt);
}
extern "C" int ptr_mlp_backward(const float *X, const float *params, const float *acts, const float *dpreds, int R, int F, int NL,
                                float p_drop, uint64_t seed, float *dz, float *ws, float *grad, void *stream) {
    return ptr::mlp_backward_impl("ptr_mlp_backward", X, params, acts, dpreds, R, F, NL, p_drop, seed, dz, ws, grad, stream, ptr::OptStep{});
}

extern "C" int ptr_mlp_backward_step(const float *X, float *params, const float *acts, const float *dpreds, int R, int F, int NL, float p_drop,
                                     uint64_t seed, float *dz, float *ws, float *grad, int opt_kind, float lr, float hyper1, float hyper2,
                                     float eps, float weight_decay, int step, float *state1, float *state2, const float *loss_q, int nq,
                                     float *loss_out, void *stream) {
    return ptr::mlp_backward_step_impl(X, params, acts, dpreds, R, F, NL, p_drop, seed, dz, ws, grad, opt_kind, lr, hyper1, hyper2, eps, weight_decay, step, state1,
                                       state2, loss_q, nq, loss_out, nullptr, stream);
}

int ptr::mlp_backward_step_impl(const float *X, float *params, const float *acts, const float *dpreds, int R, int F, int NL, float p_drop, uint64_t seed,
                                float *dz, float *ws, float *grad, int opt_kind, float lr, float hyper1, float hyper2, float eps, float weight_decay, int step,
                                float *state1, float *state2, const float *loss_q, int nq, float *loss_out, void *wimg, void *stream) {
    using namespace ptr;
    const char *who = "ptr_mlp_backward_step";
    if (opt_kind < PTR_OPT_ADAM || opt_kind > PTR_OPT_RMSPROP) { set_error("%s: unknown optimiser %d", who, opt_kind); return PTR_ERR_INVALID_ARG; }
    if (step < 1 || !state1 || (opt_kind == PTR_OPT_ADAM && !state2) || (loss_out && nq > 0 && !loss_q) || nq < 0) {
        set_error("%s: bad optimiser / loss arguments", who);
        return PTR_ERR_INVALID_ARG;
    }
    OptStep o{};
    o.kind = opt_kind; o.h1 = hyper1; o.h2 = hyper2; o.eps = eps; o.wd = weight_decay;
    o.param = params; o.s1 = state1; o.s2 = state2; o.loss_q = loss_q; o.nq = nq; o.loss_out = loss_out;
    o.wimg = reinterpret_cast<uint8_t *>(wimg); o.F = F; o.NL = NL;
    if (opt_kind == PTR_OPT_ADAM) {
        o.lr = lr; o.bc1 = 1.0f - powf(hyper1, (float)step); o.bc2_sqrt = sqrtf(1.0f - powf(hyper2, (float)step));
    } else if (opt_kind == PTR_OPT_ADAGRAD) {
        o.lr = lr / (1.0f + (float)(step - 1) * hyper1);
    } else {
        o.lr = lr;
    }
    return mlp_backward_impl(who, X, params, acts, dpreds, R, F, NL, p_drop, seed, dz, ws, grad, stream, o);
}

extern "C" int ptr_opt_step_loss(float *params, const float *grad, int64_t n, int opt_kind, float lr, float hyper1, float hyper2, float eps,
                                 float weight_decay, int step, float *state1, float *state2, const float *loss_q, int nq, float *loss_out,
                                 void *stream) {
    using namespace ptr;
    const char *who = "ptr_opt_step_loss";
    if (opt_kind < PTR_OPT_ADAM || opt_kind > PTR_OPT_RMSPROP) { set_error("%s: unknown optimiser %d", who, opt_kind); return PTR_ERR_INVALID_ARG; }
    if (n < 0 || step < 1 || nq < 0 || (n > 0 && (!params || !grad || !state1 || (opt_kind == PTR_OPT_ADAM && !state2))) || (loss_out && nq > 0 && !loss_q)) {
        set_error("%s: bad optimiser / loss arguments", who);
        return PTR_ERR_INVALID_ARG;
    }
    if (n == 0 && !loss_out) return 0;
    OptStep o{};
    o.kind = opt_kind; o.h1 = hyper1; o.h2 = hyper2; o.eps = eps; o.wd = weight_decay;
    o.param = params; o.s1 = state1; o.s2 = state2; o.loss_q = loss_q; o.nq = nq; o.loss_out = loss_out;
    if (opt_kind == PTR_OPT_ADAM) { o.lr = lr; o.bc1 = 1.0f - powf(hyper1, (float)step); o.bc2_sqrt = sqrtf(1.0f - powf(hyper2, (float)step)); }
    else if (opt_kind == PTR_OPT_ADAGRAD) o.lr = lr / (1.0f + (float)(step - 1) * hyper1);
    else o.lr = lr;
    const size_t nn = (size_t)n;
    hipLaunchKernelGGL(reduce_partials_kernel, dim3((unsigned)((nn + 63) / 64) + (loss_out ? 1 : 0)), dim3(1024), 0, as_stream(stream), grad, 1, 1, nn,
                       nn, nn, (float *)nullptr, o);
    return check_hip(hipGetLastError(), who);
}

int ptr::mlp_backward_impl(const char *who, const float *X, const float *params, const float *acts, const float *dpreds, int R, int F, int NL,
                                  float p_drop, uint64_t seed, float *dz, float *ws, float *grad, void *stream, const OptStep &opt) {
    using namespace ptr;
    if (int rc = check_mlp(who, R, F, NL, p_drop)) return rc;
    if (!X || !params || !acts || !dpreds || !ws || !grad) { set_error("%s: NULL pointer", who); return PTR_ERR_INVALID_ARG; }
    hipStream_t st = as_stream(stream);
    MlpArgs a{R, F, NL, p_drop, (uint32_t)seed, (uint32_t)(seed >> 32)};
    if (R > 0 && bwd_fused_supported(F, NL, X, acts)) {
        if (int e = bwd_x6_supported(R, F, NL, X, acts) ? launch_bwd_x6(X, params, acts, dpreds, a, ws, st, who)
                                                        : launch_bwd_fused(X, params, acts, dpreds, a, ws, st, who)) return e;
        const int nb = bwd_fused_grid(R);
        const size_t NPf = n_params(NL, F);
        hipLaunchKernelGGL(reduce_partials_kernel, dim3((unsigned)((NPf + 63) / 64) + (opt.loss_out ? 1 : 0)), dim3(1024), 0, st, ws, nb, nb, NPf, NPf, NPf,
                           grad, opt);
        return check_hip(hipGetLastError(), who);
    }
    if (!dz) { set_error("%s: dz scratch is required for this configuration (ptr_mlp_backward_dz_floats)", who); return PTR_ERR_INVALID_ARG; }
    const int ncu = num_cus();
    const int nblk = kDwBlocksPerCu * ncu;
    const size_t NP = n_params(NL, F);
    constexpr int wpb = 8;
    const int ntiles = (R + 15) / 16;
    int grid_dz = ntiles < wpb * ncu ? (ntiles + wpb - 1) / wpb : ncu;
    if (grid_dz < 1) grid_dz = 1;
    const bool tail = R > 0 && bwd_tail_supported(NL, acts);
    if (tail) {
        if (int e = bwd_x6_tail_supported(R, NL, acts) ? launch_bwd_x6_tail(params, acts, dpreds, a, ws, dz, st, who)
                                                       : launch_bwd_tail(params, acts, dpreds, a, ws, dz, st, who)) return e;
    } else {
        const size_t lds = dz_lds_floats(NL) * sizeof(float);
        auto go = [&](auto kern) -> int {
            if (int e = allow_lds(kern, lds)) return e;
            hipLaunchKernelGGL(kern, dim3(grid_dz), dim3(wpb * 64), lds, st, params, acts, dpreds, a, dz, ws, NP, off_wout(NL, F));
            return check_hip(hipGetLastError(), who);
        };
        if (int e = go(mlp_bwd_dz_kernel<1, 512>)) return e;
    }
    for (int l = 0; l < (tail ? 1 : NL); ++l) {
        const int K = l == 0 ? F : kH;
        const float *A = l == 0 ? X : acts + (size_t)(l - 1) * act_layer_floats(R);
        const int lda = l == 0 ? F : kAL;
        const float *dZ = dz + (size_t)l * R * kAL;
        const int ntk = (K + 15) / 16;
        auto go = [&](auto kern, int nt_base) -> int {
            hipLaunchKernelGGL(kern, dim3(nblk), dim3(256), 0, st, A, lda, dZ, K, nt_base, a, ws, NP, off_W(l, F), off_b(l, F));
            return check_hip(hipGetLastError(), who);
        };
        auto go_lds = [&](auto kern, int ntw, int nt_base) -> int {
            if (int e0 = allow_lds(kern, dw_lds_bytes(ntw, kDwRB))) return e0;
            hipLaunchKernelGGL(kern, dim3(nblk), dim3(256), dw_lds_bytes(ntw, kDwRB), st, A, lda, dZ, K, nt_base, a, ws, NP, off_W(l, F),
                               off_b(l, F));
            return check_hip(hipGetLastError(), who);
        };
        const bool aligned = (lda % 4 == 0) && ((reinterpret_cast<uintptr_t>(A) & 15) == 0);
        int e = 0;
        if (l == 0) {
            if (aligned) {
                if (ntk <= 12) e = go_lds(mlp_bwd_dw_lds_kernel<3, true, kDwRB>, 3, 0);
                else if (dw_x6_supported(R, K, lda, A))
                    e = launch_dw_x6(A, lda, dZ, K, ntk, a, ws, NP, off_W(l, F), off_b(l, F), nblk, st, who);
                else for (int base = 0; base < ntk && !e; base += 24) e = go_lds(mlp_bwd_dw_lds_kernel<6, true, kDwRB>, 6, base);
            } else if (ntk <= 12) e = go(mlp_bwd_dw_kernel<3, true, 4>, 0);
            else if (ntk <= 24) e = go(mlp_bwd_dw_kernel<6, true, 4>, 0);
            else if (ntk <= 48) { e = go(mlp_bwd_dw_kernel<6, true, 4>, 0); if (!e) e = go(mlp_bwd_dw_kernel<6, true, 4>, 24); }
            else { set_error("%s: F=%d not supported by the dW kernel", who, F); return PTR_ERR_UNSUPPORTED; }
        } else {
            if (!aligned) e = go(mlp_bwd_dw_kernel<2, false, 4>, 0);
            else e = go_lds(mlp_bwd_dw_lds_kernel<2, false, kDwRB>, 2, 0);
        }
        if (e) return e;
    }
    hipLaunchKernelGGL(reduce_partials_kernel, dim3((unsigned)((NP + 63) / 64) + (opt.loss_out ? 1 : 0)), dim3(1024), 0, st, ws, nblk,
                       tail ? bwd_fused_grid(R) : grid_dz, tail ? off_W(1, F) : off_wout(NL, F), NP, NP, grad, opt);
    return check_hip(hipGetLastError(), who);
}

namespace ptr {
__global__ void __launch_bounds__(256)
adagrad_kernel(float *__restrict__ p, const float *__restrict__ grad, float *__restrict__ sum, size_t n, float clr, float eps, float wd) {
    const size_t i = (size_t)blockIdx.x * 256 + threadIdx.x;
    if (i >= n) return;
    const float pi = p[i];
    const float gi = grad[i] + wd * pi;
    const float si = sum[i] + gi * gi;
    sum[i] = si;
    p[i] = pi - clr * (gi / (sqrtf(si) + eps));
}
__global__ void __launch_bounds__(256)
rmsprop_kernel(float *__restrict__ p, const float *__restrict__ grad, float *__restrict__ sq, size_t n, float lr, float alpha, float eps, float wd) {
    const size_t i = (size_t)blockIdx.x * 256 + threadIdx.x;
    if (i >= n) return;
    const float pi = p[i];
    const float gi = grad[i] + wd * pi;
    const float si = alpha * sq[i] + (1.0f - alpha) * gi * gi;
    sq[i] = si;
    p[i] = pi - lr * (gi / (sqrtf(si) + eps));
}
}

extern "C" int ptr_adagrad_step(float *param, const float *grad, float *state_sum, int64_t n, float lr, float lr_decay, float eps,
                                float weight_decay, int step, void *stream) {
    using namespace ptr;
    if (n < 0 || step < 1 || (n > 0 && (!param || !grad || !state_sum))) { set_error("ptr_adagrad_step: bad arguments"); return PTR_ERR_INVALID_ARG; }
    if (n == 0) return 0;
    const float clr = lr / (1.0f + (float)(step - 1) * lr_decay);
    hipLaunchKernelGGL(adagrad_kernel, dim3((unsigned)((n + 255) / 256)), dim3(256), 0, as_stream(stream), param, grad, state_sum, (size_t)n, clr, eps,
                       weight_decay);
    return check_hip(hipGetLastError(), "ptr_adagrad_step");
}

extern "C" int ptr_rmsprop_step(float *param, const float *grad, float *square_avg, int64_t n, float lr, float alpha, float eps,
                                float weight_decay, void *stream) {
    using namespace ptr;
    if (n < 0 || (n > 0 && (!param || !grad || !square_avg))) { set_error("ptr_rmsprop_step: bad arguments"); return PTR_ERR_INVALID_ARG; }
    if (n == 0) return 0;
    hipLaunchKernelGGL(rmsprop_kernel, dim3((unsigned)((n + 255) / 256)), dim3(256), 0, as_stream(stream), param, grad, square_avg, (size_t)n, lr, alpha,
                       eps, weight_decay);
    return check_hip(hipGetLastError(), "ptr_rmsprop_step");
}

extern "C" int ptr_adam_step(float *param, const float *grad, float *exp_avg, float *exp_avg_sq, int64_t n, float lr, float beta1,
                             float beta2, float eps, float weight_decay, int step, void *stream) {
    using namespace ptr;
    if (n < 0 || step < 1 || (n > 0 && (!param || !grad || !exp_avg || !exp_avg_sq))) { set_error("ptr_adam_step: bad arguments"); return PTR_ERR_INVALID_ARG; }
    if (n == 0) return 0;
    const float bc1 = 1.0f - powf(beta1, (float)step), bc2_sqrt = sqrtf(1.0f - powf(beta2, (float)step));
    hipLaunchKernelGGL(adam_kernel, dim3((unsigned)((n + 255) / 256)), dim3(256), 0, as_stream(stream), param, grad, exp_avg, exp_avg_sq,
                       (size_t)n, lr, beta1, beta2, eps, weight_decay, bc1, bc2_sqrt);
    return check_hip(hipGetLastError(), "ptr_adam_step");
}

extern "C" int ptr_mlp_dropout_mask(int R, int n_feat, int site, float p_drop, uint64_t seed, float *out, void *stream) {
    using namespace ptr;
    if (R < 0 || n_feat <= 0 || !out) { set_error("ptr_mlp_dropout_mask: bad arguments"); return PTR_ERR_INVALID_ARG; }
    MlpArgs a{R, n_feat, 1, p_drop, (uint32_t)seed, (uint32_t)(seed >> 32)};
    const size_t n = (size_t)R * n_feat;
    if (n == 0) return 0;
    hipLaunchKernelGGL(dropout_mask_kernel, dim3((unsigned)((n + 255) / 256)), dim3(256), 0, as_stream(stream), a, site, n_feat, out);
    return check_hip(hipGetLastError(), "ptr_mlp_dropout_mask");
}
```

ptranking_amd/csrc/scorer_bwd.hip:

```cpp
#include "ptr_mlp.h"

namespace ptr {

constexpr int kSR = 32;
constexpr int kBW = 8;
constexpr int kBT = kBW * 64;
constexpr int kSlabF = kSR * kAL;
#define PREP_BEGIN() __builtin_amdgcn_s_setprio(2)
#define PREP_END() __builtin_amdgcn_s_setprio(0)

__host__ __device__ constexpr int ldx_of(int NT1) { return (NT1 & 1) ? 16 * NT1 : 16 * NT1 + 16; }
__host__ __device__ constexpr size_t bwd_fused_lds_floats(int NL, int NT1) {
    return (size_t)2 * NL * kSlabF + (size_t)(NL - 1) * kSlabF + (size_t)2 * kSR * ldx_of(NT1) + 2 * kSR + kHP + kAL + 256 * 4;
}

template <int NL, int NT1> struct TileMap {
    static constexpr int CH = NL - 1;
    static constexpr int NPH = CH + 1;
    static constexpr int NT = 7 * NT1 + (NL - 1) * 49;
    static constexpr int MAXL = 64;
    int tl[NT], tn[NT], tm[NT], slot[NT];
    int cnt[kBW][NPH];
    int lst[kBW][NPH][MAXL];
    int ntiles[kBW];
    int maxtiles;
    static constexpr int ntl(int l) { return l == 0 ? NT1 : 7; }
    constexpr TileMap() : tl{}, tn{}, tm{}, slot{}, cnt{}, lst{}, ntiles{}, maxtiles(0) {
        int id = 0;
        for (int l = 0; l < NL; ++l)
            for (int n = 0; n < ntl(l); ++n)
                for (int m = 0; m < 7; ++m) { tl[id] = l; tn[id] = n; tm[id] = m; ++id; }
        bool taken[NT] = {};
        for (int c = 0; c < CH; ++c) {
            const int l = NL - 1 - c;
            for (int v = 7; v < kBW; ++v) {
                const int e = v - 7, n0 = ntl(l) - 2 - 2 * (e / 2), m0 = 3 * (e % 2);
                for (int t = 0; t < NT; ++t)
                    if (tl[t] == l && tn[t] >= n0 && tn[t] < n0 + 2 && tm[t] >= m0 && tm[t] < m0 + 3 && n0 >= 0) { taken[t] = true; lst[v][c][cnt[v][c]++] = t; }
            }
        }
        int T[NL] = {}, k[NL] = {}, take[NL] = {}, left[NL] = {};
        int rem = 0;
        for (int t = 0; t < NT; ++t)
            if (!taken[t]) { ++T[tl[t]]; ++rem; }
        const int base = rem / kBW;
        const int quota7 = base;
        int C[NL] = {}, Ctot = 0;
        for (int t = 0; t < NT; ++t)
            if (!taken[t]) { const int c = (tm[t] == 6 || (tl[t] >= 1 && tn[t] == 6)) ? 14 : 32; C[tl[t]] += c; Ctot += c; }
        const int budget = Ctot / kBW;
        int ksum = 0;
        for (int l = 0; l < NL; ++l) { k[l] = base > 0 ? T[l] / base : 0; ksum += k[l]; }
        while (ksum > kBW - 1) {
            int best = -1;
            for (int l = 0; l < NL; ++l)
                if (k[l] > 0 && (best < 0 || T[l] - k[l] * base < T[best] - k[best] * base)) best = l;
            --k[best]; --ksum;
        }
        while (ksum < kBW - 1) {
            int best = 0;
            for (int l = 1; l < NL; ++l)
                if (T[l] - k[l] * base > T[best] - k[best] * base) best = l;
            ++k[best]; ++ksum;
        }
        int L = 0;
        (void)quota7;
        for (int l = 0; l < NL; ++l) {
            int tk = k[l] > 0 && C[l] > 0 ? (budget * T[l]) / C[l] : 0;
            if (k[l] > 0 && tk > T[l] / k[l]) tk = T[l] / k[l];
            take[l] = tk; left[l] = T[l] - k[l] * take[l]; L += left[l];
        }
        {
            int w = 0;
            for (int l = 0; l < NL; ++l) {
                int given = 0, run = 0;
                for (int t = 0; t < NT; ++t) {
                    if (taken[t] || tl[t] != l) continue;
                    if (run < k[l]) {
                        lst[w][CH][cnt[w][CH]++] = t;
                        if (++given == take[l]) { given = 0; ++run; ++w; }
                    } else {
                        lst[kBW - 1][CH][cnt[kBW - 1][CH]++] = t;
                    }
                }
            }
        }
        for (int v = 0; v < kBW; ++v) {
            int s = 0;
            for (int ph = 0; ph < NPH; ++ph)
                for (int k = 0; k < cnt[v][ph]; ++k) slot[lst[v][ph][k]] = s++;
            ntiles[v] = s;
            if (s > maxtiles) maxtiles = s;
        }
    }
    constexpr bool first_a(int w, int ph, int k) const {
        const int t = lst[w][ph][k];
        for (int i = 0; i < k; ++i) { const int u = lst[w][ph][i]; if (tl[u] == tl[t] && tm[u] == tm[t]) return false; }
        return true;
    }
    constexpr bool is_nstrip(int t) const { return tl[t] >= 1 && tn[t] == 6 && tm[t] < 6; }
    constexpr bool first_nstrip(int w, int ph, int k) const {
        const int t = lst[w][ph][k];
        if (!is_nstrip(t)) return false;
        for (int i = 0; i < k; ++i) { const int u = lst[w][ph][i]; if (tl[u] == tl[t] && is_nstrip(u)) return false; }
        return true;
    }
    constexpr bool first_b(int w, int ph, int k) const {
        const int t = lst[w][ph][k];
        if (is_nstrip(t)) return false;
        for (int i = 0; i < k; ++i) { const int u = lst[w][ph][i]; if (tl[u] == tl[t] && tn[u] == tn[t] && !is_nstrip(u)) return false; }
        return true;
    }
};
template <int NL, int NT1> inline constexpr TileMap<NL, NT1> kTM{};

using lds_f = __attribute__((address_space(3))) float;

#ifdef PTR_BWD_TRACE
#define BWD_STAMP(i)                                                                                                    \
    do {                                                                                                                \
        if (blockIdx.x == 0 && lane == 0 && nslab_done < 8)                                                             \
        {                                                                                                               \
            unsigned long long *tr_ = reinterpret_cast<unsigned long long *>(ws + (size_t)gridDim.x * np_stride) + (nslab_done * kBW + W) * 16; \
            tr_[(i)] = clock64();                                                                                       \
            if ((i) == 0) tr_[15] = wall_clock64();                        \
        }                                                                                                               \
    } while (0)
#else
#define BWD_STAMP(i) do { } while (0)
#endif

template <int NL, int NT1, int W>
__device__ __forceinline__ void bwd_body(const float *__restrict__ X, const float *__restrict__ P, const float *__restrict__ acts,
                                         const float *__restrict__ dpreds, const MlpArgs a, float *__restrict__ ws, size_t np_stride,
                                         float *smem, float *__restrict__ dz0) {
    using TMt = TileMap<NL, NT1>;
    constexpr int CH = NL - 1, LDX = ldx_of(NT1), NTMAX = NT1 > 7 ? NT1 : 7;
    constexpr int NACC = kTM<NL, NT1>.ntiles[W] > 0 ? kTM<NL, NT1>.ntiles[W] : 1;
    constexpr bool TAIL = NT1 == 0;
    constexpr bool loader = W < 4;
    constexpr bool topper = W >= 4 && W < 8;
    const int F = a.F, R = a.R;
    const int tid = threadIdx.x, lane = tid & 63, j = lane & 15, g = lane >> 4;
    float *bufA = smem;
    float *Zb = bufA + 2 * NL * kSlabF;
    float *XSb = Zb + CH * kSlabF;
    float *dsb = XSb + 2 * kSR * LDX;
    float *wo = dsb + 2 * kSR;
    float *junk_row = wo + kHP;
    float *junk_x = junk_row + kAL;
    const uint32_t bufA_addr = lds_byte_addr(bufA);
    const int nslabs = (R + kSR - 1) / kSR;
    const uint32_t thr = drop_thr(a.p_drop);
    const float inv_keep = a.p_drop > 0.0f ? 1.0f / (1.0f - a.p_drop) : 1.0f;

    for (int i = tid; i < kHP; i += kBT) { wo[i] = i < kH ? P[off_wout(NL, F) + i] : 0.0f; junk_row[i] = 0.0f; }
    float wf[CH > 0 ? CH : 1][25];
    static_for<CH>([&](auto c_) {
        constexpr int c = c_, l = NL - 1 - c;
        const float *Wl = P + off_W(l, F);
        const int k = 16 * W + j;
        const bool kok = W < 7 && k < kH;
        const int kc = kok ? k : 0;
#pragma unroll
        for (int S = 0; S < 6; ++S)
#pragma unroll
            for (int c4 = 0; c4 < 4; ++c4) {
                const float v = Wl[(size_t)(16 * S + 4 * g + c4) * kH + kc];
                wf[c][4 * S + c4] = kok ? v : 0.0f;
            }
        const float v = Wl[(size_t)(96 + g) * kH + kc];
        wf[c][24] = kok ? v : 0.0f;
    });
#pragma unroll
    for (int c = 0; c < (CH > 0 ? CH : 1); ++c)
#pragma unroll
        for (int i = 0; i < 25; ++i) asm volatile("" : "+v"(wf[c][i]));

    constexpr int XTOT = kSR * 4 * NT1, XSL = (XTOT + 255) / 256, XW4 = TAIL ? 1 : 4 * NT1;
    auto x_slot = [&](int t, int u, int &xr, int &xc) -> bool {
        const int idx = t + 256 * u;
        const bool in = idx < XTOT;
        xr = in ? idx / XW4 : 0;
        xc = in ? idx - xr * XW4 : 0;
        return in;
    };
    f32x4 xraw[(loader && XSL > 0) ? XSL : 1];
    float dsraw = 0.0f;

    auto issue_dma = [&](int slab, int buf, int lane_o) {
        const int nrt = act_row_tiles(R);
#pragma unroll
        for (int q = 0; q < (NL * 14 + kBW - 1) / kBW; ++q) {
            const int k = W + kBW * q;
            if (k < NL * 14) {
                const int layer = k / 14, ch = k - 14 * layer;
                const int rt = min(2 * slab + (ch >= 7 ? 1 : 0), nrt - 1);
                const float *src = acts + (size_t)layer * act_layer_floats(R) + (size_t)rt * kActTile + (ch >= 7 ? ch - 7 : ch) * 256 + 4 * lane_o;
                const uint32_t dst = bufA_addr + (uint32_t)(((buf * NL + layer) * kSlabF + ch * 256) * 4);
                glds16(src, __builtin_amdgcn_readfirstlane(dst));
            }
        }
    };
    auto load_x = [&](int slab, int tid_o) {
        const int row0 = slab * kSR;
        if constexpr (loader) {
#pragma unroll
            for (int u = 0; u < XSL; ++u) {
                int xr, xc;
                x_slot(tid_o, u, xr, xc);
                const int gr = min(row0 + xr, R - 1);
                const int cc = 4 * xc < F ? 4 * xc : 0;
                xraw[u] = *reinterpret_cast<const f32x4 *>(X + (size_t)gr * F + cc);
            }
        }
        dsraw = dpreds[min(row0 + (tid_o & (kSR - 1)), R - 1)];
    };
    auto finish_x = [&](int slab, int buf, int tid_o) {
      if constexpr (loader) {
        const int row0 = slab * kSR;
        float *XS = XSb + buf * kSR * LDX;
        const uint32_t thr_e = a.p_drop > 0.0f ? thr : 0u;
#pragma unroll
        for (int u = 0; u < XSL; ++u) {
            int xr, xc;
            const bool in = x_slot(tid_o, u, xr, xc);
            uint32_t w0, w1;
            drop_bits(a.seed_lo, a.seed_hi, 0, min(row0 + xr, R - 1), xc, w0, w1);
            f32x4 v = drop4(xraw[u], w0, w1, thr_e, inv_keep);
            const float okf = 4 * xc < F ? 1.0f : 0.0f;
#pragma unroll
            for (int c = 0; c < 4; ++c) v[c] *= okf;
            v[0] = 4 * xc == F ? 1.0f : v[0];
            float *dst = in ? XS + xr * LDX + 4 * xc : junk_x + 4 * tid_o;
            *reinterpret_cast<f32x4 *>(dst) = v;
        }
      }
    };
    f32x4 dwo4 = f32x4{0.f, 0.f, 0.f, 0.f};
    float dbo = 0.0f;
    f32x4 dbc[CH > 1 ? CH - 1 : 1];
#pragma unroll
    for (int i = 0; i < (CH > 1 ? CH - 1 : 1); ++i) dbc[i] = f32x4{0.f, 0.f, 0.f, 0.f};
    f32x4 dbt4 = f32x4{0.f, 0.f, 0.f, 0.f};
    auto top_pass = [&](int buf, int tid_o) {
      if constexpr (topper) {
        const int t = tid_o - 256;
        const int rs = t / 28, f4 = t - rs * 28;
        const f32x4 w4 = *reinterpret_cast<const f32x4 *>(wo + 4 * f4);
        float *img = bufA + (buf * NL + NL - 1) * kSlabF;
        const float first = f4 == 0 ? 1.0f : 0.0f;
        float *pa[4];
        f32x4 h4[4];
        float ds[4];
#pragma unroll
        for (int h = 0; h < 4; ++h) {
            const int r = rs + 9 * h;
            const bool ok = rs < 9 && r < kSR;
            pa[h] = ok ? img + (r >> 4) * kActTile + (f4 >> 2) * 256 + (r & 15) * 16 + (f4 & 3) * 4 : junk_row + 4 * f4;
            h4[h] = *reinterpret_cast<const f32x4 *>(pa[h]);
            const float dsr = dsb[buf * kSR + (ok ? r : 0)];
            ds[h] = ok ? dsr : 0.0f;
        }
#pragma unroll
        for (int h = 0; h < 4; ++h) {
            f32x4 d;
#pragma unroll
            for (int c = 0; c < 4; ++c) {
                d[c] = (ds[h] * w4[c]) * (h4[h][c] > 0.0f ? 1.0f : 0.0f);
                dwo4[c] = fmaf(h4[h][c], ds[h], dwo4[c]);
                dbt4[c] += d[c];
            }
            *reinterpret_cast<f32x4 *>(pa[h]) = d;
            dbo = fmaf(first, ds[h], dbo);
        }
      }
    };

    f32x4 acc[NACC];
#pragma unroll
    for (int i = 0; i < NACC; ++i) acc[i] = f32x4{0.f, 0.f, 0.f, 0.f};

    auto dw_phase = [&](auto wv_, auto ph_, const float *cur, const float *XS) {
        constexpr int WV = wv_, PH = ph_;
        constexpr int CNT = kTM<NL, NT1>.cnt[WV][PH];
        if constexpr (CNT > 0) {
            float av[2][NL][kMT], bv[2][NL][NTMAX], bv6[2][NL];
            uint32_t zb[NL], ab[NL], zb6[NL], ab6[NL];
#pragma unroll
            for (int l = 0; l < NL; ++l) {
                zb[l] = lds_byte_addr(l == NL - 1 ? cur + (NL - 1) * kSlabF : Zb + l * kSlabF) + (uint32_t)((g * 16 + j) * 4);
                ab[l] = l == 0 ? lds_byte_addr(XS) + (uint32_t)((g * LDX + j) * 4)
                               : lds_byte_addr(cur + (l - 1) * kSlabF) + (uint32_t)((g * 16 + j) * 4);
                zb6[l] = zb[l] - (uint32_t)((j - (j & 3)) * 4);
                ab6[l] = ab[l] - (uint32_t)((j - (j & 3)) * 4);
                asm volatile("" : "+v"(zb[l]), "+v"(ab[l]), "+v"(zb6[l]), "+v"(ab6[l]));
            }
            auto rd = [&](int ks, auto set_) {
                constexpr int set = set_;
                static_for<CNT>([&](auto k_) {
                    constexpr int t = kTM<NL, NT1>.lst[WV][PH][k_];
                    constexpr int l = kTM<NL, NT1>.tl[t], n = kTM<NL, NT1>.tn[t], m = kTM<NL, NT1>.tm[t];
                    const int kso = (ks >> 2) * kActTile + (ks & 3) * 64;
                    if constexpr (kTM<NL, NT1>.first_a(WV, PH, k_))
                        av[set][l][m] = *reinterpret_cast<lds_f *>((uintptr_t)((m == kMT - 1 ? zb6[l] : zb[l]) + (uint32_t)((kso + 256 * m) * 4)));
                    if constexpr (kTM<NL, NT1>.first_b(WV, PH, k_))
                        bv[set][l][n] = *reinterpret_cast<lds_f *>((uintptr_t)(ab[l] + (uint32_t)((l == 0 ? 4 * ks * LDX + 16 * n : kso + 256 * n) * 4)));
                    if constexpr (kTM<NL, NT1>.first_nstrip(WV, PH, k_))
                        bv6[set][l] = *reinterpret_cast<lds_f *>((uintptr_t)(ab6[l] + (uint32_t)((kso + 256 * 6) * 4)));
                });
            };
            auto mma = [&](auto set_) {
                constexpr int set = set_;
                static_for<CNT>([&](auto k_) {
                    constexpr int t = kTM<NL, NT1>.lst[WV][PH][k_];
                    constexpr int l = kTM<NL, NT1>.tl[t], n = kTM<NL, NT1>.tn[t], m = kTM<NL, NT1>.tm[t], s = kTM<NL, NT1>.slot[t];
                    if constexpr (m == kMT - 1) {
                        acc[s] = __builtin_amdgcn_mfma_f32_4x4x1f32(av[set][l][m], bv[set][l][n], acc[s], 0, 0, 0);
                    } else if constexpr (kTM<NL, NT1>.is_nstrip(t)) {
                        acc[s] = __builtin_amdgcn_mfma_f32_4x4x1f32(bv6[set][l], av[set][l][m], acc[s], 0, 0, 0);
                    } else {
                        acc[s] = __builtin_amdgcn_mfma_f32_16x16x4f32(av[set][l][m], bv[set][l][n], acc[s], 0, 0, 0);
                    }
                });
            };
            using S0 = std::integral_constant<int, 0>;
            using S1 = std::integral_constant<int, 1>;
            rd(0, S0{});
#pragma unroll
            for (int ks = 0; ks < kSR / 4; ks += 2) {
                rd(ks + 1, S1{});
                mma(S0{});
                rd(ks + 2 < kSR / 4 ? ks + 2 : ks + 1, S0{});
                mma(S1{});
            }
        }
    };
    int slab = blockIdx.x, p = 0;
    int nslab_done = 0;
    (void)nslab_done;
    issue_dma(slab, 0, lane);
    load_x(slab, tid);
    asm volatile("s_waitcnt vmcnt(0)" ::: "memory");
    {
        const float dsv = slab * kSR + (tid & (kSR - 1)) < R ? dsraw : 0.0f;
        if (tid < kSR) dsb[tid] = dsv;
    }
    if (loader) finish_x(slab, 0, tid);
    wg_barrier();
    if (topper) top_pass(0, tid);
    wg_barrier();

    for (; slab < nslabs; slab += gridDim.x, p ^= 1) {
        const bool real_next = slab + gridDim.x < nslabs;
        const int next = real_next ? slab + gridDim.x : slab;
        float *cur = bufA + p * NL * kSlabF;
        int tid_o = tid, lane_o = lane;
        asm volatile("" : "+v"(tid_o), "+v"(lane_o));
        BWD_STAMP(0);

        static_for<CH>([&](auto c_) {
            constexpr int c = c_, l = NL - 1 - c;
            if constexpr (c == 0) {
                if constexpr (loader) { PREP_BEGIN(); issue_dma(next, p ^ 1, lane_o); load_x(next, tid_o); PREP_END(); }
            }
            if constexpr (W < 7) {
                const float *src = c == 0 ? cur + (NL - 1) * kSlabF : Zb + l * kSlabF;
                float *dst = Zb + (l - 1) * kSlabF;
                const float *gate = cur + (l - 1) * kSlabF;
#pragma unroll
                for (int rt = 0; rt < kSR / 16; ++rt) {
                    const int rbase = rt * kActTile + j * 16;
                    f32x4 b[6];
#pragma unroll
                    for (int S = 0; S < 6; ++S) b[S] = *reinterpret_cast<const f32x4 *>(src + rbase + 256 * S + 4 * g);
                    const float bt = src[rbase + 256 * 6 + g];
                    const f32x4 gt = *reinterpret_cast<const f32x4 *>(gate + rbase + 256 * W + 4 * g);
                    f32x4 ac0 = f32x4{0.f, 0.f, 0.f, 0.f}, ac1 = f32x4{0.f, 0.f, 0.f, 0.f};
#pragma unroll
                    for (int S = 0; S < 6; ++S) {
                        ac0 = __builtin_amdgcn_mfma_f32_16x16x4f32(wf[c][4 * S + 0], b[S][0], ac0, 0, 0, 0);
                        ac1 = __builtin_amdgcn_mfma_f32_16x16x4f32(wf[c][4 * S + 1], b[S][1], ac1, 0, 0, 0);
                        ac0 = __builtin_amdgcn_mfma_f32_16x16x4f32(wf[c][4 * S + 2], b[S][2], ac0, 0, 0, 0);
                        ac1 = __builtin_amdgcn_mfma_f32_16x16x4f32(wf[c][4 * S + 3], b[S][3], ac1, 0, 0, 0);
                    }
                    ac0 = __builtin_amdgcn_mfma_f32_16x16x4f32(wf[c][24], bt, ac0, 0, 0, 0);
                    f32x4 d;
#pragma unroll
                    for (int e = 0; e < 4; ++e) d[e] = (ac0[e] + ac1[e]) * (gt[e] > 0.0f ? inv_keep : 0.0f);
                    *reinterpret_cast<f32x4 *>(dst + rbase + 256 * W + 4 * g) = d;
                    if constexpr (c < CH - 1) dbc[c] += d;
                }
            } else {
                dw_phase(std::integral_constant<int, W>{}, c_, cur, XSb + p * kSR * LDX);
            }
            if constexpr (c == 0) {
                if constexpr (!loader) { PREP_BEGIN(); issue_dma(next, p ^ 1, lane_o); load_x(next, tid_o); PREP_END(); }
            }
            if constexpr (c == CH - 1) {
                asm volatile("s_waitcnt vmcnt(0)" ::: "memory");
                const float dsv = (real_next && next * kSR + (tid_o & (kSR - 1)) < R) ? dsraw : 0.0f;
                if (tid_o < kSR) dsb[(p ^ 1) * kSR + tid_o] = dsv;
            }
            BWD_STAMP(1 + 2 * c);
            wg_barrier();
            BWD_STAMP(2 + 2 * c);
        });

        if constexpr (loader && !TAIL) { PREP_BEGIN(); finish_x(next, p ^ 1, tid_o); PREP_END(); }
        if constexpr (loader && TAIL) {
            const int row0 = slab * kSR;
#pragma unroll
            for (int u = 0; u < (kSR * (kAL / 4) + 255) / 256; ++u) {
                const int idx = tid_o + 256 * u;
                const int r = idx / (kAL / 4), c4 = idx - r * (kAL / 4);
                if (idx < kSR * (kAL / 4) && row0 + r < R)
                    *reinterpret_cast<f32x4 *>(dz0 + (size_t)(row0 + r) * kAL + 4 * c4) = *reinterpret_cast<const f32x4 *>(Zb + act_off(r, 4 * c4));
            }
        }
        BWD_STAMP(1 + 2 * CH);
        dw_phase(std::integral_constant<int, W>{}, std::integral_constant<int, CH>{}, cur, XSb + p * kSR * LDX);
        BWD_STAMP(2 + 2 * CH);
        if constexpr (topper) { PREP_BEGIN(); top_pass(p ^ 1, tid_o); PREP_END(); }
        BWD_STAMP(3 + 2 * CH);
        wg_barrier();
        BWD_STAMP(4 + 2 * CH);
        ++nslab_done;
    }

    float *out = ws + (size_t)blockIdx.x * np_stride;
    auto store_tiles = [&](auto wv_) {
        constexpr int WV = wv_;
        static_for<TMt::NPH>([&](auto ph_) {
            constexpr int PH = ph_;
            static_for<kTM<NL, NT1>.cnt[WV][PH]>([&](auto k_) {
                constexpr int t = kTM<NL, NT1>.lst[WV][PH][k_];
                constexpr int l = kTM<NL, NT1>.tl[t], n = kTM<NL, NT1>.tn[t], m = kTM<NL, NT1>.tm[t], s = kTM<NL, NT1>.slot[t];
                const int K = l == 0 ? F : kH;
                const int k = 16 * n + j;
                float *o = out + off_W(l, F);
                if constexpr (m == kMT - 1) {
#pragma unroll
                    for (int c = 0; c < 4; ++c) {
                        float v = acc[s][c];
                        v += __shfl_xor(v, 16, 64);
                        v += __shfl_xor(v, 32, 64);
                        if (g == 0 && k < K) o[(size_t)(96 + c) * K + k] = v;
                        if (l == 0 && g == 0 && k == K) out[off_b(l, F) + 96 + c] = v;
                    }
                } else if constexpr (kTM<NL, NT1>.is_nstrip(t)) {
                    const int of = 16 * m + j;
#pragma unroll
                    for (int c = 0; c < 4; ++c) {
                        float v = acc[s][c];
                        v += __shfl_xor(v, 16, 64);
                        v += __shfl_xor(v, 32, 64);
                        if (g == 0) o[(size_t)of * K + 96 + c] = v;
                    }
                } else {
#pragma unroll
                    for (int c = 0; c < 4; ++c) {
                        const int of = 16 * m + 4 * g + c;
                        if (of < kH && k < K) o[(size_t)of * K + k] = acc[s][c];
                        if (l == 0 && of < kH && k == K) out[off_b(l, F) + of] = acc[s][c];
                    }
                }
            });
        });
    };
    store_tiles(std::integral_constant<int, W>{});
    if (topper) {
        const int t = tid - 256, rs = t / 28, f4 = t - rs * 28;
        if (rs < 9) {
            *reinterpret_cast<f32x4 *>(Zb + rs * kAL + 4 * f4) = dwo4;
            *reinterpret_cast<f32x4 *>(Zb + (9 + rs) * kAL + 4 * f4) = dbt4;
            if (f4 == 0) Zb[18 * kAL + rs] = dbo;
        }
    }
    if constexpr (W < 7) {
        static_for<(CH > 1 ? CH - 1 : 0)>([&](auto c_) {
            constexpr int c = c_, lyr = NL - 2 - c;
#pragma unroll
            for (int e = 0; e < 4; ++e) {
                float v = dbc[c][e];
                v += __shfl_xor(v, 1, 64); v += __shfl_xor(v, 2, 64); v += __shfl_xor(v, 4, 64); v += __shfl_xor(v, 8, 64);
                const int of = 16 * W + 4 * g + e;
                if (j == 0 && of < kH) out[off_b(lyr, F) + of] = v;
            }
        });
    }
    wg_barrier();
    if (tid < kH) {
        float s = 0.0f, sb = 0.0f;
#pragma unroll
        for (int r = 0; r < 9; ++r) { s += Zb[r * kAL + tid]; sb += Zb[(9 + r) * kAL + tid]; }
        out[off_wout(NL, F) + tid] = s;
        out[off_b(NL - 1, F) + tid] = sb;
    } else if (tid == kH) {
        float s = 0.0f;
#pragma unroll
        for (int r = 0; r < 9; ++r) s += Zb[18 * kAL + r];
        out[off_wout(NL, F) + kH] = s;
    }
}

template <int NL, int NT1>
__global__ void __launch_bounds__(kBT)
mlp_bwd_fused_kernel(const float *__restrict__ X, const float *__restrict__ P, const float *__restrict__ acts,
                     const float *__restrict__ dpreds, MlpArgs a, float *__restrict__ ws, size_t np_stride, float *__restrict__ dz0) {
    extern __shared__ __attribute__((aligned(16))) float smem[];
    const int wave = __builtin_amdgcn_readfirstlane(threadIdx.x >> 6);
    switch (wave) {
        case 0: bwd_body<NL, NT1, 0>(X, P, acts, dpreds, a, ws, np_stride, smem, dz0); break;
        case 1: bwd_body<NL, NT1, 1>(X, P, acts, dpreds, a, ws, np_stride, smem, dz0); break;
        case 2: bwd_body<NL, NT1, 2>(X, P, acts, dpreds, a, ws, np_stride, smem, dz0); break;
        case 3: bwd_body<NL, NT1, 3>(X, P, acts, dpreds, a, ws, np_stride, smem, dz0); break;
        case 4: bwd_body<NL, NT1, 4>(X, P, acts, dpreds, a, ws, np_stride, smem, dz0); break;
        case 5: bwd_body<NL, NT1, 5>(X, P, acts, dpreds, a, ws, np_stride, smem, dz0); break;
        case 6: bwd_body<NL, NT1, 6>(X, P, acts, dpreds, a, ws, np_stride, smem, dz0); break;
        default: bwd_body<NL, NT1, 7>(X, P, acts, dpreds, a, ws, np_stride, smem, dz0); break;
    }
}

bool bwd_fused_supported(int F, int NL, const void *X, const void *acts) {
    if (!env_int("PTR_BWD_FUSED", 1)) return false;
    const int NT1 = (F + 15) / 16;
    return NL == 3 && NT1 == 9 && F % 4 == 0 && F < 16 * NT1 && (reinterpret_cast<uintptr_t>(X) & 15) == 0 && (reinterpret_cast<uintptr_t>(acts) & 15) == 0;
}

int bwd_fused_grid(int R) {
    const int nslabs = (R + kSR - 1) / kSR;
    return nslabs < num_cus() ? nslabs : num_cus();
}

int launch_bwd_fused(const float *X, const float *params, const float *acts, const float *dpreds, const MlpArgs &a, float *ws,
                     hipStream_t st, const char *who) {
    const int grid = bwd_fused_grid(a.R);
    const size_t NP = n_params(a.NL, a.F);
    auto go = [&](auto kern, int NT1) -> int {
        const size_t lds = bwd_fused_lds_floats(a.NL, NT1) * sizeof(float);
        if (int e = allow_lds(kern, lds)) return e;
        hipLaunchKernelGGL(kern, dim3(grid), dim3(kBT), lds, st, X, params, acts, dpreds, a, ws, NP, (float *)nullptr);
        return check_hip(hipGetLastError(), who);
    };
    return go(mlp_bwd_fused_kernel<3, 9>, 9);
}

bool bwd_tail_supported(int NL, const void *acts) {
    if (!env_int("PTR_BWD_TAIL", 1)) return false;
    return (NL == 2 || NL == 3) && (reinterpret_cast<uintptr_t>(acts) & 15) == 0;
}

int launch_bwd_tail(const float *params, const float *acts, const float *dpreds, const MlpArgs &a, float *ws, float *dz0, hipStream_t st,
                    const char *who) {
    const int grid = bwd_fused_grid(a.R);
    const size_t NP = n_params(a.NL, a.F);
    auto go = [&](auto kern) -> int {
        const size_t lds = bwd_fused_lds_floats(a.NL, 0) * sizeof(float);
        if (int e = allow_lds(kern, lds)) return e;
        hipLaunchKernelGGL(kern, dim3(grid), dim3(kBT), lds, st, (const float *)nullptr, params, acts, dpreds, a, ws, NP, dz0);
        return check_hip(hipGetLastError(), who);
    };
    return a.NL == 2 ? go(mlp_bwd_fused_kernel<2, 0>) : go(mlp_bwd_fused_kernel<3, 0>);
}

}
```

ptranking_amd/csrc/scorer_bwd_x6.hip:

```cpp
#include "ptr_mlp.h"

namespace ptr {

constexpr int kB6S = 32;
constexpr int kB6ZRS = 224, kB6ZPL = kB6S * kB6ZRS, kB6ZIMG = 3 * kB6ZPL;
constexpr int kB6XRS = 288, kB6XPL = kB6S * kB6XRS, kB6XIMG = 3 * kB6XPL;
constexpr int kB6STG = kB6S * kAL * 4;
constexpr int kB6_ZA = 0, kB6_ZB = kB6ZIMG, kB6_A1 = 2 * kB6ZIMG, kB6_A2 = 3 * kB6ZIMG, kB6_XI = 4 * kB6ZIMG, kB6_ST = kB6_XI + kB6XIMG;
constexpr int kB6_WO = kB6_ST + 3 * kB6STG;
constexpr int kB6Lds = kB6_WO + 512;
static_assert(kB6Lds <= 160 * 1024, "LDS budget");

using b6_srd = __attribute__((ext_vector_type(4))) int;
using b6_rsrc = __amdgpu_buffer_rsrc_t;
__device__ __forceinline__ b6_srd b6_make_srd(const void *p, uint32_t bytes) {
    const uint64_t a = reinterpret_cast<uint64_t>(p);
    return b6_srd{(int)(uint32_t)a, (int)((uint32_t)(a >> 32) & 0xffffu), (int)bytes, 0x00020000};
}
__device__ __forceinline__ void b6_bdma16(b6_srd srd, uint32_t voff, uint32_t soff, uint32_t lds_dst) {
    unsigned keep;
    asm volatile("s_mov_b32 %0, m0\n\ts_mov_b32 m0, %4\n\ts_nop 0\n\tbuffer_load_dwordx4 %1, %2, %3 offen lds\n\ts_mov_b32 m0, %0"
                 : "=&s"(keep) : "v"(voff), "s"(srd), "s"(soff), "s"(lds_dst) : "memory");
}
__device__ __forceinline__ uint32_t b6_opaque(uint32_t x) { asm volatile("" : "+s"(x)); return x; }

template <int NT1>
__global__ void __launch_bounds__(512, 2)
mlp_bwd_x6_kernel(const float *__restrict__ X, const float *__restrict__ P, const float *__restrict__ acts, const float *__restrict__ dpreds,
                  MlpArgs a, float *__restrict__ ws, size_t np_stride, float *__restrict__ dz0) {
    static_assert(NT1 == 9 || NT1 == 0, "the X image is laid out for nine in-feature tiles; NT1 = 0 is the TAIL form");
    constexpr bool TAIL = NT1 == 0;
    extern __shared__ __attribute__((aligned(16))) uint8_t smem_b6[];
    constexpr int NL = 3;
    const int F = a.F, R = a.R;
    const int tid = threadIdx.x, lane = tid & 63, j = lane & 15, g = lane >> 4, W = __builtin_amdgcn_readfirstlane(tid >> 6);
    const uint32_t lds0 = lds_byte_addr(smem_b6);
#ifdef PTR_B6_TRACE_EDGE
    unsigned long long *etrace = reinterpret_cast<unsigned long long *>(ws + (size_t)gridDim.x * np_stride) + 8 * 256 + W * 16;
    int nedge = 0;
#define B6_EDGE() do { if (blockIdx.x == 0 && lane == 0 && nedge < 16) etrace[nedge++] = clock64(); } while (0)
#else
#define B6_EDGE() do { } while (0)
#endif
    B6_EDGE();
    const int nslabs = (R + kB6S - 1) / kB6S;
    const uint32_t thr = a.p_drop > 0.0f ? drop_thr(a.p_drop) : 0u;
    const float scale = a.p_drop > 0.0f ? 1.0f / (1.0f - a.p_drop) : 1.0f;
    const bool chain = W < 7;
    for (int i = tid; i < kB6Lds / 16; i += 512) reinterpret_cast<u32x4 *>(smem_b6)[i] = u32x4{0u, 0u, 0u, 0u};
    __syncthreads();
    B6_EDGE();

    f32x4 st[39];
#pragma unroll
    for (int i = 0; i < 39; ++i) st[i] = f32x4{0.0f, 0.0f, 0.0f, 0.0f};
    if (chain) {
#pragma unroll
        for (int c = 0; c < 2; ++c) {
            const float *Wl = P + off_W(2 - c, F);
            const int ri = 16 * W + j;
#pragma unroll
            for (int s = 0; s < 3; ++s) {
                float v[8];
#pragma unroll
                for (int e = 0; e < 8; ++e) {
                    const int k = 32 * s + 8 * g + e;
                    v[e] = ri < kH ? Wl[(size_t)k * kH + ri] : 0.0f;
                }
                Frag pl[3];
#pragma unroll
                for (int d = 0; d < 4; ++d) split_pack2(v[2 * d], v[2 * d + 1], pl[0].u[d], pl[1].u[d], pl[2].u[d]);
#pragma unroll
                for (int p = 0; p < 3; ++p) st[18 + 3 * (3 * c + s) + p] = __builtin_bit_cast(f32x4, pl[p].q);
            }
            {
                float v[4];
#pragma unroll
                for (int e = 0; e < 4; ++e) { const int k = 96 + 4 * g + e; v[e] = (ri < kH && k < kH) ? Wl[(size_t)k * kH + ri] : 0.0f; }
                uint32_t t0[3], t1[3];
                split_pack2(v[0], v[1], t0[0], t0[1], t0[2]);
                split_pack2(v[2], v[3], t1[0], t1[1], t1[2]);
#pragma unroll
                for (int p = 0; p < 3; ++p) {
                    const int d = 2 * (3 * c + p);
                    st[36 + d / 4][d % 4] = __uint_as_float(t0[p]);
                    st[36 + d / 4][d % 4 + 1] = __uint_as_float(t1[p]);
                }
            }
        }
    }
    B6_EDGE();
    if (tid < kHP) reinterpret_cast<float *>(smem_b6 + kB6_WO)[tid] = tid < kH ? P[off_wout(NL, F) + tid] : 0.0f;
    float awo[4] = {0.0f, 0.0f, 0.0f, 0.0f}, abo = 0.0f;

    const uint32_t swz = (uint32_t)((j >> 2) & 1);
    const uint32_t wr_z = (uint32_t)(j * kB6ZRS) + 8u * ((uint32_t)g ^ (2u * swz));
    const uint32_t wr_x = (uint32_t)(j * kB6XRS) + 8u * ((uint32_t)g ^ (2u * swz));
    const uint32_t rd_b = (uint32_t)(j * kB6ZRS + 32 * (g >> 1)) + 16u * (((uint32_t)g & 1u) ^ swz);
    const uint32_t tr_z = (uint32_t)((4 * g + (j >> 2)) * kB6ZRS) + 8u * (((uint32_t)j & 3u) ^ (2u * ((uint32_t)g & 1u)));
    const uint32_t tr_x = (uint32_t)((4 * g + (j >> 2)) * kB6XRS) + 8u * (((uint32_t)j & 3u) ^ (2u * ((uint32_t)g & 1u)));

    auto mma6w = [&](f32x4 &c, int w0, const Frag (&bf)[3]) __attribute__((always_inline)) {
        Frag af[3];
#pragma unroll
        for (int p = 0; p < 3; ++p) af[p].q = __builtin_bit_cast(u32x4, st[w0 + p]);
        mma6(c, af, bf);
    };
    auto mma6t = [&](f32x4 &c, int cl, const u32x2 (&bt)[3]) __attribute__((always_inline)) {
        i16x4 at[3], bb[3];
#pragma unroll
        for (int p = 0; p < 3; ++p) {
            const int d = 2 * (3 * cl + p);
            at[p] = __builtin_bit_cast(i16x4, u32x2{__float_as_uint(st[36 + d / 4][d % 4]), __float_as_uint(st[36 + d / 4][d % 4 + 1])});
            bb[p] = __builtin_bit_cast(i16x4, bt[p]);
        }
#pragma unroll
        for (int q = 0; q < 6; ++q) c = __builtin_amdgcn_mfma_f32_16x16x16bf16_1k(at[kSixA[q]], bb[kSixB[q]], c, 0, 0, 0);
    };
    auto dw_row = [&](auto nn_, auto pipe_, int acc0, uint32_t zimg, int mo, uint32_t aimg_lane, int a_plane, int a_row, int n0) __attribute__((always_inline)) {
        constexpr int NN = decltype(nn_)::value;
        constexpr bool PIPE = decltype(pipe_)::value;
        Frag za[3];
        read_tr(za, zimg + tr_z + (uint32_t)(32 * mo), kB6ZPL, kB6ZRS, 0);
        if constexpr (PIPE && NN > 1) {
            Frag ab[2][3];
            read_tr(ab[0], aimg_lane, a_plane, a_row, n0);
#pragma unroll
            for (int n = 0; n < NN; ++n) {
                if (n + 1 < NN) read_tr(ab[(n + 1) & 1], aimg_lane, a_plane, a_row, n0 + n + 1);
                __builtin_amdgcn_sched_barrier(0);
                mma6(st[acc0 + n], za, ab[n & 1]);
                __builtin_amdgcn_sched_barrier(0);
            }
        } else {
#pragma unroll
            for (int n = 0; n < NN; ++n) {
                Frag ab[3];
                read_tr(ab, aimg_lane, a_plane, a_row, n0 + n);
                mma6(st[acc0 + n], za, ab);
                __builtin_amdgcn_sched_barrier(0);
            }
        }
    };

    f32x4 xr[2][2];
    float dsv[2];
    const b6_rsrc xsrd = __builtin_amdgcn_make_buffer_rsrc(const_cast<float *>(X), 0, TAIL ? 0 : (int)((uint32_t)R * (uint32_t)(F * 4)), 0x00020000);
    const b6_rsrc zsrd = __builtin_amdgcn_make_buffer_rsrc(dz0, 0, TAIL ? (int)((uint32_t)R * (uint32_t)(kAL * 4)) : 0, 0x00020000);
    const b6_rsrc dsrd = __builtin_amdgcn_make_buffer_rsrc(const_cast<float *>(dpreds), 0, (int)((uint32_t)R * 4u), 0x00020000);
    const b6_srd asrd = b6_make_srd(acts, (uint32_t)NL * (uint32_t)(act_layer_floats(R) * 4));
    uint32_t jx = (uint32_t)j * (uint32_t)(F * 4) + (uint32_t)g * 16, j4 = (uint32_t)j * 4, l16 = (uint32_t)lane * 16;
    asm volatile("" : "+v"(jx), "+v"(j4), "+v"(l16));
    auto load_x = [&](int slab) __attribute__((always_inline)) {
        const int row0 = slab * kB6S;
#pragma unroll
        for (int dt = 0; dt < 2; ++dt)
#pragma unroll
            for (int sl = 0; sl < 2; ++sl) {
                const int t = chain ? W : 7 + sl;
                if (!(chain && sl == 1))
                    xr[sl][dt] = __builtin_bit_cast(f32x4, __builtin_amdgcn_raw_buffer_load_b128(xsrd, (int)jx, (int)((uint32_t)(row0 + 16 * dt) * (uint32_t)(F * 4) + (uint32_t)(64 * t)), 0));
            }
    };
    uint32_t jk = (uint32_t)j * kDropRowMul + (uint32_t)g * kDropFgMul + a.seed_lo;
    asm volatile("" : "+v"(jk));
    auto stage_x_tile = [&](int row0, int t_, const f32x4 (&x2)[2]) __attribute__((always_inline)) {
        const int t = (int)b6_opaque((uint32_t)t_);
        int col = 16 * t + 4 * g;
        asm volatile("" : "+v"(col));
#pragma unroll
        for (int dt = 0; dt < 2; ++dt) {
            uint32_t w0, w1;
            drop_bits_key(jk + ((uint32_t)(row0 + 16 * dt) * kDropRowMul + (uint32_t)(4 * t) * kDropFgMul), a.seed_hi, w0, w1);
            f32x4 v = drop4(x2[dt], w0, w1, thr, scale);
#pragma unroll
            for (int r = 0; r < 4; ++r) v[r] = col + r < F ? v[r] : (col + r == F ? 1.0f : 0.0f);
            split_write4(b6_opaque(lds0 + kB6_XI + (uint32_t)(32 * t)) + wr_x + (uint32_t)(16 * dt * kB6XRS), kB6XPL, v);
        }
    };
    auto stage_x = [&](int slab) __attribute__((always_inline)) {
        if (chain) stage_x_tile(slab * kB6S, W, xr[0]);
        else { stage_x_tile(slab * kB6S, 7, xr[0]); stage_x_tile(slab * kB6S, 8, xr[1]); }
    };
    auto prefetch = [&](int slab) __attribute__((always_inline)) {
        const int row0 = slab * kB6S;
#pragma unroll
        for (int q = 0; q < 6; ++q) {
            const int k = chain ? W + 7 * q : 3 * 14;
            if (k < 3 * 14) {
                const int layer = k / 14, ch = k - 14 * layer;
                b6_bdma16(asrd, l16, (uint32_t)layer * (uint32_t)(act_layer_floats(R) * 4) + (uint32_t)row0 * (kAL * 4) + (uint32_t)ch * 1024,
                          __builtin_amdgcn_readfirstlane(lds0 + (uint32_t)(kB6_ST + layer * kB6STG + ch * 1024)));
            }
        }
#pragma unroll
        for (int dt = 0; dt < 2; ++dt)
            dsv[dt] = __builtin_bit_cast(float, __builtin_amdgcn_raw_buffer_load_b32(dsrd, (int)j4, (int)((uint32_t)(row0 + 16 * dt) * 4u), 0));
    };
    uint32_t m2 = 0u, m1 = 0u;
    auto staging = [&](uint32_t zdst) __attribute__((always_inline)) {
        m2 = 0u; m1 = 0u;
        if (chain) {
            const f32x4 wo4 = *reinterpret_cast<lds_f32x4 *>((uintptr_t)(b6_opaque(lds0 + (uint32_t)(kB6_WO + 64 * W)) + (uint32_t)(16 * g)));
#pragma unroll
            for (int dt = 0; dt < 2; ++dt) {
                const uint32_t so = b6_opaque(lds0 + (uint32_t)(kB6_ST + 1024 * W)) + (uint32_t)(j * 64 + 16 * g) + (uint32_t)(dt * kActTile * 4);
                const f32x4 a1 = *reinterpret_cast<lds_f32x4 *>((uintptr_t)so);
                const f32x4 a2 = *reinterpret_cast<lds_f32x4 *>((uintptr_t)(so + kB6STG));
                const f32x4 a3 = *reinterpret_cast<lds_f32x4 *>((uintptr_t)(so + 2 * kB6STG));
                const float ds = dsv[dt];
                f32x4 z3;
#pragma unroll
                for (int r = 0; r < 4; ++r) {
                    z3[r] = a3[r] > 0.0f ? ds * wo4[r] : 0.0f;
                    awo[r] = fmaf(ds, a3[r], awo[r]);
                    m2 |= (a2[r] > 0.0f ? 1u : 0u) << (4 * dt + r);
                    m1 |= (a1[r] > 0.0f ? 1u : 0u) << (4 * dt + r);
                }
                if (W == 0 && g == 0) abo += ds;
                const uint32_t wo = wr_z + b6_opaque(lds0 + (uint32_t)(32 * W)) + (uint32_t)(16 * dt * kB6ZRS);
                split_write4(wo + b6_opaque(zdst), kB6ZPL, z3);
                split_write4(wo + kB6_A2, kB6ZPL, a2);
                split_write4(wo + kB6_A1, kB6ZPL, a1);
            }
        }
    };
    const int slab0 = blockIdx.x;
    prefetch(slab0 < nslabs ? slab0 : nslabs - 1);
    asm volatile("s_waitcnt vmcnt(0)" ::: "memory");
    __syncthreads();
    B6_EDGE();

#ifdef PTR_B6_TRACE
    unsigned long long *trace = reinterpret_cast<unsigned long long *>(ws + (size_t)gridDim.x * np_stride) + W * 256;
    int nstamp = 0;
#define B6_STAMP() do { if (blockIdx.x == 0 && lane == 0 && nstamp < 256) trace[nstamp++] = clock64(); } while (0)
#else
#define B6_STAMP() do { } while (0)
#endif
#if defined(PTR_B6_TRACE) && defined(PTR_B6_TRACE2)
#define B6_STAMP2() B6_STAMP()
#else
#define B6_STAMP2() do { } while (0)
#endif
    uint32_t zi = kB6_ZA, zo = kB6_ZB;
    staging(zi);
    wg_barrier();
    {
        const int nxt = slab0 + (int)gridDim.x;
        prefetch(nxt < nslabs ? nxt : nslabs - 1);
    }
    for (int slab = slab0; slab < nslabs; slab += gridDim.x) {
        B6_STAMP();
#pragma unroll
        for (int c = 0; c < 2; ++c) {
            if constexpr (!TAIL) { if (c == 1) load_x(slab); }
            const uint32_t zin = b6_opaque(lds0 + (c == 0 ? zi : zo)), zout = b6_opaque(lds0 + (c == 0 ? zo : zi) + (uint32_t)(32 * W));
            const uint32_t aim = b6_opaque(lds0 + (c == 0 ? kB6_A2 : kB6_A1));
            if (chain) {
              auto chain_part = [&]() __attribute__((always_inline)) {
                f32x4 cc[2] = {f32x4{0.f, 0.f, 0.f, 0.f}, f32x4{0.f, 0.f, 0.f, 0.f}};
                auto read_b = [&](Frag (&b)[3], int u) __attribute__((always_inline)) {
#pragma unroll
                    for (int p = 0; p < 3; ++p)
                        b[p].q = *reinterpret_cast<lds_u32x4 *>((uintptr_t)(zin + rd_b + (uint32_t)(p * kB6ZPL + 16 * (u & 1) * kB6ZRS + 64 * (u >> 1))));
                };
                u32x2 bt[2][3];
                auto read_bt = [&]() __attribute__((always_inline)) {
#pragma unroll
                    for (int dt = 0; dt < 2; ++dt)
#pragma unroll
                        for (int p = 0; p < 3; ++p)
                            bt[dt][p] = *reinterpret_cast<lds_u32x2 *>((uintptr_t)(zin + wr_z + (uint32_t)(192 + p * kB6ZPL + 16 * dt * kB6ZRS)));
                };
                if (c == 0) {
                    Frag b[2][3];
                    read_b(b[0], 0);
#pragma unroll
                    for (int u = 0; u < 6; ++u) {
                        if (u + 1 < 6) read_b(b[(u + 1) & 1], u + 1);
                        else read_bt();
                        __builtin_amdgcn_sched_barrier(0);
                        mma6w(cc[u & 1], 18 + 3 * (3 * c + (u >> 1)), b[u & 1]);
                        __builtin_amdgcn_sched_barrier(0);
                    }
                } else {
#pragma unroll
                    for (int u = 0; u < 6; ++u) {
                        Frag b[3];
                        read_b(b, u);
                        if (u == 5) read_bt();
                        mma6w(cc[u & 1], 18 + 3 * (3 * c + (u >> 1)), b);
                        __builtin_amdgcn_sched_barrier(0);
                    }
                }
#pragma unroll
                for (int dt = 0; dt < 2; ++dt) {
                    mma6t(cc[dt], c, bt[dt]);
                    __builtin_amdgcn_sched_barrier(0);
                }
                B6_STAMP2();
                const uint32_t m = c == 0 ? m2 : m1;
#pragma unroll
                for (int dt = 0; dt < 2; ++dt) {
                    f32x4 dz;
#pragma unroll
                    for (int r = 0; r < 4; ++r) dz[r] = (m >> (4 * dt + r)) & 1u ? cc[dt][r] * scale : 0.0f;
                    if (TAIL && c == 1) {
                        const uint32_t row = (uint32_t)(slab * kB6S + 16 * dt + j);
                        __builtin_amdgcn_raw_buffer_store_b128(__builtin_bit_cast(u32x4, dz), zsrd, (int)(row < (uint32_t)R ? row * (kAL * 4) + (uint32_t)(64 * W + 16 * g) : 0xFFFFF000u), 0, 0);
                    } else {
                        split_write4(zout + wr_z + (uint32_t)(16 * dt * kB6ZRS), kB6ZPL, dz);
                    }
                }
                B6_STAMP2();
              };
              auto dw_part = [&]() __attribute__((always_inline)) {
                if (c == 0) dw_row(std::integral_constant<int, 5>{}, std::true_type{}, 0, zin, W, aim + tr_z, kB6ZPL, kB6ZRS, 0);
                else dw_row(std::integral_constant<int, 5>{}, std::false_type{}, 5, zin, W, aim + tr_z, kB6ZPL, kB6ZRS, 0);
              };
              chain_part();
              dw_part();
            } else {
                B6_STAMP2(); B6_STAMP2();
                constexpr int ZD = 2;
                Frag ab5[3], ab6[3], zr[ZD][3];
                read_tr(zr[0], zin + tr_z, kB6ZPL, kB6ZRS, 0);
                read_tr(ab5, aim + tr_z, kB6ZPL, kB6ZRS, 5);
                read_tr(ab6, aim + tr_z, kB6ZPL, kB6ZRS, 6);
#pragma unroll
                for (int d = 1; d < ZD - 1; ++d) read_tr(zr[d], zin + tr_z + (uint32_t)(32 * d), kB6ZPL, kB6ZRS, 0);
#pragma unroll
                for (int mo = 0; mo < 7; ++mo) {
                    if (mo + ZD - 1 < 7) read_tr(zr[(mo + ZD - 1) % ZD], zin + tr_z + (uint32_t)(32 * (mo + ZD - 1)), kB6ZPL, kB6ZRS, 0);
                    __builtin_amdgcn_sched_barrier(0);
                    mma6(st[14 * c + 2 * mo], zr[mo % ZD], ab5);
                    mma6(st[14 * c + 2 * mo + 1], zr[mo % ZD], ab6);
                    __builtin_amdgcn_sched_barrier(0);
                }
            }
            if constexpr (!TAIL) { if (c == 1) stage_x(slab); }
            if (c == 0 && slab != slab0) {
                const int nxt = slab + (int)gridDim.x;
                prefetch(nxt < nslabs ? nxt : nslabs - 1);
            }
            if (c == 1) asm volatile("s_waitcnt vmcnt(0)" ::: "memory");
            B6_STAMP();
            wg_barrier();
            B6_STAMP();
        }
        const bool more = slab + (int)gridDim.x < nslabs;
        if constexpr (TAIL) {
            if (more) staging(zo);
        } else {
            const uint32_t za = b6_opaque(lds0 + zi), xi = b6_opaque(lds0 + kB6_XI) + tr_x;
            if (more) staging(zo);
            __builtin_amdgcn_sched_barrier(0);
            B6_STAMP2();
            if (chain) {
                dw_row(std::integral_constant<int, 8>{}, std::true_type{}, 10, za, W, xi, kB6XPL, kB6XRS, 0);
            } else {
                Frag xb[3], zr[2][3];
                read_tr(zr[0], za + tr_z, kB6ZPL, kB6ZRS, 0);
                read_tr(xb, xi, kB6XPL, kB6XRS, 8);
#pragma unroll
                for (int mo = 0; mo < 7; ++mo) {
                    if (mo + 1 < 7) read_tr(zr[(mo + 1) & 1], za + tr_z + (uint32_t)(32 * (mo + 1)), kB6ZPL, kB6ZRS, 0);
                    __builtin_amdgcn_sched_barrier(0);
                    mma6(st[28 + mo], zr[mo & 1], xb);
                    __builtin_amdgcn_sched_barrier(0);
                }
            }
        }
        B6_STAMP();
        wg_barrier();
        B6_STAMP();
        const uint32_t tz = zi; zi = zo; zo = tz;
    }
    asm volatile("s_waitcnt vmcnt(0)" ::: "memory");
    B6_EDGE();

    float *out = ws + (size_t)blockIdx.x * np_stride;
    auto store_tile = [&](const f32x4 &c, int layer, int mo, int ni) __attribute__((always_inline)) {
        const int K = layer == 0 ? F : kH;
        const int in = 16 * ni + j;
#pragma unroll
        for (int r = 0; r < 4; ++r) {
            const int o = 16 * mo + 4 * g + r;
            if (o < kH) {
                if (in < K) out[off_W(layer, F) + (size_t)o * K + in] = c[r];
                else if (in == K) out[off_b(layer, F) + o] = c[r];
            }
        }
    };
    if (chain) {
#pragma unroll
        for (int n = 0; n < 5; ++n) { store_tile(st[n], 2, W, n); store_tile(st[5 + n], 1, W, n); }
        if constexpr (!TAIL) {
#pragma unroll
            for (int n = 0; n < 8; ++n) store_tile(st[10 + n], 0, W, n);
        }
#pragma unroll
        for (int r = 0; r < 4; ++r) {
            float v = awo[r];
#pragma unroll
            for (int m = 1; m < 16; m <<= 1) v += __shfl_xor(v, m, 64);
            const int f = 16 * W + 4 * g + r;
            if (j == 0 && f < kH) out[off_wout(NL, F) + f] = v;
        }
        if (W == 0) {
            float v = abo;
#pragma unroll
            for (int m = 1; m < 16; m <<= 1) v += __shfl_xor(v, m, 64);
            if (lane == 0) out[off_wout(NL, F) + kH] = v;
        }
    } else {
#pragma unroll
        for (int mo = 0; mo < 7; ++mo) {
#pragma unroll
            for (int q = 0; q < 2; ++q) { store_tile(st[2 * mo + q], 2, mo, 5 + q); store_tile(st[14 + 2 * mo + q], 1, mo, 5 + q); }
            if constexpr (!TAIL) store_tile(st[28 + mo], 0, mo, 8);
        }
    }
#ifdef PTR_B6_TRACE_EDGE
    asm volatile("s_waitcnt vmcnt(0)" ::: "memory");
    B6_EDGE();
#endif
}

bool bwd_x6_supported(int R, int F, int NL, const void *X, const void *acts) {
    if (!env_int("PTR_BWD_X6", 1)) return false;
    const int NT1 = (F + 15) / 16;
    if ((uint64_t)NL * (uint64_t)act_layer_floats(R) * 4 >= 0xFFFFF000ull || (uint64_t)R * (uint64_t)F * 4 >= 0xFFFFF000ull) return false;
    return NL == 3 && NT1 == 9 && F % 4 == 0 && F < 16 * NT1 && (reinterpret_cast<uintptr_t>(X) & 15) == 0 && (reinterpret_cast<uintptr_t>(acts) & 15) == 0;
}
int launch_bwd_x6(const float *X, const float *params, const float *acts, const float *dpreds, const MlpArgs &a, float *ws, hipStream_t st,
                  const char *who) {
    const int grid = bwd_fused_grid(a.R);
    const size_t NP = n_params(a.NL, a.F);
    auto kern = mlp_bwd_x6_kernel<9>;
    if (int e = allow_lds(kern, kB6Lds)) return e;
    hipLaunchKernelGGL(kern, dim3(grid), dim3(512), kB6Lds, st, X, params, acts, dpreds, a, ws, NP, (float *)nullptr);
    return check_hip(hipGetLastError(), who);
}

bool bwd_x6_tail_supported(int R, int NL, const void *acts) {
    if (!env_int("PTR_BWD_X6", 1)) return false;
    if ((uint64_t)NL * (uint64_t)act_layer_floats(R) * 4 >= 0xFFFFF000ull || (uint64_t)R * (kAL * 4) >= 0xFFFFF000ull) return false;
    return NL == 3 && (reinterpret_cast<uintptr_t>(acts) & 15) == 0;
}
int launch_bwd_x6_tail(const float *params, const float *acts, const float *dpreds, const MlpArgs &a, float *ws, float *dz0, hipStream_t st,
                       const char *who) {
    const int grid = bwd_fused_grid(a.R);
    const size_t NP = n_params(a.NL, a.F);
    auto kern = mlp_bwd_x6_kernel<0>;
    if (int e = allow_lds(kern, kB6Lds)) return e;
    hipLaunchKernelGGL(kern, dim3(grid), dim3(512), kB6Lds, st, (const float *)nullptr, params, acts, dpreds, a, ws, NP, dz0);
    return check_hip(hipGetLastError(), who);
}

}
```

ptranking_amd/csrc/scorer_x6.hip:

```cpp
#include "ptr_mlp.h"

namespace ptr {

constexpr int kX6Pieces = kX6SliceBytes / 1024;
constexpr int kX6Ring = 6;

__host__ __device__ inline size_t x6_lds_bytes(int NL) { return (size_t)kX6Ring * kX6SliceBytes + ((size_t)NL * kHP + kHP + 16) * sizeof(float); }

__device__ __forceinline__ float relu1(float x) { return __builtin_amdgcn_fmed3f(x, 0.0f, 3.0e38f); }

__global__ void __launch_bounds__(256) x6_prep_kernel(const float *__restrict__ P, int F, int NL, uint8_t *__restrict__ img) {
    const int idx = blockIdx.x * 256 + threadIdx.x;
    const int n1 = x6_n1(F), ns = x6_nslices(F, NL);
    if (idx >= ns * kX6Rows * 4) return;
    const int g = idx & 3, row = (idx >> 2) % kX6Rows, sl = idx / (4 * kX6Rows);
    const int layer = sl < n1 ? 0 : 1 + (sl - n1) / 4, s = sl < n1 ? sl : (sl - n1) % 4;
    const int K = layer == 0 ? F : kH;
    const float *W = P + off_W(layer, F);
    Frag f[3];
#pragma unroll
    for (int h = 0; h < 2; ++h) {
        f32x4 v;
#pragma unroll
        for (int c = 0; c < 4; ++c) {
            const int k = layer == 0 ? 32 * s + 8 * g + 4 * h + c : 32 * s + 16 * h + 4 * g + c;
            v[c] = (row < kH && k < K) ? W[(size_t)row * K + k] : 0.0f;
            if (layer > 0 && row < kH && k == kH) v[c] = P[off_b(layer, F) + row];
        }
        split_pack4(v, f, 2 * h);
    }
#pragma unroll
    for (int p = 0; p < 3; ++p)
        *reinterpret_cast<u32x4 *>(img + (size_t)sl * kX6SliceBytes + (size_t)p * kX6PlaneBytes + (size_t)(row >> 4) * 1024 + g * 256 + (row & 15) * 16) = f[p].q;
}

using x6_rsrc = __amdgpu_buffer_rsrc_t;
__device__ __forceinline__ x6_rsrc x6_srd(void *p, uint32_t bytes) { return __builtin_amdgcn_make_buffer_rsrc(p, 0, (int)bytes, 0x00020000); }
__device__ __forceinline__ void x6_store16(x6_rsrc srd, uint32_t off, f32x4 v) {
    __builtin_amdgcn_raw_buffer_store_b128(__builtin_bit_cast(u32x4, v), srd, (int)off, 0, 0);
}
__device__ __forceinline__ f32x4 x6_load16(x6_rsrc srd, uint32_t voff, uint32_t soff) {
    return __builtin_bit_cast(f32x4, __builtin_amdgcn_raw_buffer_load_b128(srd, (int)voff, (int)soff, 0));
}
__device__ __forceinline__ void x6_store4(x6_rsrc srd, uint32_t off, float v) { __builtin_amdgcn_raw_buffer_store_b32(__builtin_bit_cast(uint32_t, v), srd, (int)off, 0, 0); }
constexpr uint32_t kX6Oob = 0xFFFFC000u;
constexpr uint64_t kX6BufLimit = 0xFFFFC000ull;

#define X6_MFMA(A, B, C) __builtin_amdgcn_mfma_f32_16x16x32_bf16((A).v, (B).v, (C), 0, 0, 0)

#define X6_SB() __builtin_amdgcn_sched_barrier(0)
#define X6_TSTRIDE 1024
#define X6_MIX(NM, NV)                                                                                     \
    do {                                                                                                   \
        _Pragma("unroll") for (int i_ = 0; i_ < (NM); ++i_) {                                              \
            __builtin_amdgcn_sched_group_barrier(0x008, 1, 0);                                             \
            __builtin_amdgcn_sched_group_barrier(0x002, (NV), 0);                                          \
        }                                                                                                  \
    } while (0)
template <int... Ks> struct X6K {};
template <int R, int K0, int... Ks> constexpr int x6_kget(X6K<K0, Ks...>) { if constexpr (R == 0) return K0; else return x6_kget<R - 1>(X6K<Ks...>{}); }

template <bool TRAIN, bool STORE, int DT>
__global__ void __launch_bounds__(16 / DT * 64, DT == 4 ? 1 : 2)
mlp_fwd_x6_kernel(const float *__restrict__ X, const float *__restrict__ P, const uint8_t *__restrict__ img, MlpArgs a,
                  float *__restrict__ preds, float *__restrict__ acts) {
    extern __shared__ __attribute__((aligned(16))) uint8_t smem_x6[];
    constexpr int NW = 16 / DT, RPT = 16 * DT, PW = (kX6Pieces + NW - 1) / NW;
    const int F = a.F, NL = a.NL, R = a.R;
    float *Bs = reinterpret_cast<float *>(smem_x6 + (size_t)kX6Ring * kX6SliceBytes);
    float *Wo = Bs + (size_t)NL * kHP;
    const int tid = threadIdx.x;
    for (int i = tid; i < NL * kHP; i += NW * 64) { const int l = i / kHP, c = i - l * kHP; Bs[i] = c < kH ? P[off_b(l, F) + c] : 0.0f; }
    for (int i = tid; i < kHP + 16; i += NW * 64) Wo[i] = i < kH ? P[off_wout(NL, F) + i] : (i == kHP ? P[off_wout(NL, F) + kH] : 0.0f);
    __syncthreads();
    const float b_out = Wo[kHP];

    const int lane = tid & 63, j = lane & 15, g = lane >> 4, wave = __builtin_amdgcn_readfirstlane(tid >> 6);
    const int ntiles = (R + RPT - 1) / RPT;
    const uint32_t thr = drop_thr(a.p_drop);
    const float scale = TRAIN ? 1.0f / (1.0f - a.p_drop) : 1.0f;
    const int n1 = x6_n1(F), ns = n1 + 4 * (NL - 1);
    const uint32_t ring = lds_byte_addr(smem_x6);
    const uint32_t lane_a = ring + (uint32_t)(lane * 16);

    int dma_slice = 0, dma_slot = 0;
    auto dma_issue = [&]() __attribute__((always_inline)) {
        const uint8_t *src = img + (size_t)dma_slice * kX6SliceBytes + lane * 16;
        const uint32_t dst = ring + (uint32_t)dma_slot * kX6SliceBytes;
#pragma unroll
        for (int i = 0; i < PW; ++i) {
            int q = wave * PW + i;
            q = q < kX6Pieces ? q : kX6Pieces - 1;
            glds16(src + q * 1024, __builtin_amdgcn_readfirstlane(dst + (uint32_t)q * 1024));
        }
        dma_slice = dma_slice + 1 == ns ? 0 : dma_slice + 1;
        dma_slot = dma_slot + 1 == kX6Ring ? 0 : dma_slot + 1;
    };
#pragma unroll 1
    for (int d = 0; d < kX6Ring - 1; ++d) dma_issue();
    static_assert(kX6Ring == 6 && (PW == 3 || PW == 6), "the vmcnt immediates below are PW * (kX6Ring - 2) and PW * (kX6Ring - 3) (+ the store margin)");
    if constexpr (STORE && DT == 2) {
#pragma unroll
        for (int i = 0; i < 6; ++i)
            glds16(img + (size_t)i * 1024 + lane * 16, __builtin_amdgcn_readfirstlane(ring + (uint32_t)(kX6Ring - 1) * kX6SliceBytes + (uint32_t)i * 1024));
    }
    if constexpr (DT == 4) asm volatile("s_waitcnt vmcnt(24)\n\ts_barrier" ::: "memory");
    else if constexpr (STORE) asm volatile("s_waitcnt vmcnt(18)\n\ts_barrier" ::: "memory");
    else asm volatile("s_waitcnt vmcnt(12)\n\ts_barrier" ::: "memory");
    int cur_slot = 0;
#ifdef PTR_X6_TRACE
    unsigned long long *trace = reinterpret_cast<unsigned long long *>(const_cast<uint8_t *>(img) + (size_t)ns * kX6SliceBytes) + wave * 256;
    int nstamp = 0;
#define X6_STAMP() do { if (blockIdx.x == 0 && lane == 0 && nstamp < 254) { trace[nstamp++] = clock64(); trace[nstamp & 1 ? 255 : 254] = wall_clock64(); if (nstamp == 1) trace[253] = wall_clock64(); } } while (0)
#else
#define X6_STAMP() do { } while (0)
#endif
    auto slice_sync = [&]() __attribute__((always_inline)) -> uint32_t {
        X6_STAMP();
        if constexpr (DT == 4) { if constexpr (STORE) asm volatile("s_waitcnt vmcnt(46)\n\ts_barrier" ::: "memory"); else asm volatile("s_waitcnt vmcnt(18)\n\ts_barrier" ::: "memory"); }
        else if constexpr (STORE) asm volatile("s_waitcnt vmcnt(23)\n\ts_barrier" ::: "memory");
        else asm volatile("s_waitcnt vmcnt(9)\n\ts_barrier" ::: "memory");
        X6_STAMP();
        dma_issue();
        cur_slot = cur_slot + 1 == kX6Ring ? 0 : cur_slot + 1;
        return lane_a + (uint32_t)cur_slot * kX6SliceBytes;
    };

    uint32_t bs_base = lds_byte_addr(Bs) + (uint32_t)g * 16;
    asm volatile("" : "+v"(bs_base));
    uint32_t wo_delta = (uint32_t)NL * (kHP * 4);
    asm volatile("" : "+s"(wo_delta));
    auto lds4 = [](uint32_t base, int byte_off) __attribute__((always_inline)) { return *reinterpret_cast<lds_f32x4 *>((uintptr_t)(base + (uint32_t)byte_off)); };
    const uint32_t nrt = (uint32_t)act_row_tiles(R), layer_bytes = nrt * (uint32_t)(kActTile * 4);
    const x6_rsrc xsrd = x6_srd(const_cast<float *>(X), (uint32_t)R * (uint32_t)(F * 4));
    const x6_rsrc psrd = x6_srd(preds, (uint32_t)R * 4u);
    const x6_rsrc asrd = x6_srd(acts, STORE ? (uint32_t)NL * layer_bytes : 0u);
    f32x4 acc[kMT][DT];
    Frag bp[4][DT][3];
    Frag bfx[2][DT][3];
    f32x4 raw[2][DT][2];
    Frag af[2][3];
    using I0 = std::integral_constant<int, 0>; using I1 = std::integral_constant<int, 1>;

    auto read_a = [&](Frag (&buf)[3], uint32_t abase, int mt) __attribute__((always_inline)) {
#pragma unroll
        for (int p = 0; p < 3; ++p) buf[p].q = *reinterpret_cast<lds_u32x4 *>((uintptr_t)(abase + (uint32_t)(p * kX6PlaneBytes + mt * 1024)));
    };
    auto mma_tile = [&](const Frag (&buf)[3], auto mt_, const Frag (&bf)[DT][3]) __attribute__((always_inline)) {
        constexpr int mt = decltype(mt_)::value;
#pragma unroll
        for (int q = 0; q < 6; ++q)
#pragma unroll
            for (int dt = 0; dt < DT; ++dt) acc[mt][dt] = X6_MFMA(buf[kSixA[q]], bf[dt][kSixB[q]], acc[mt][dt]);
    };
    auto mma_tile_tail = [&](const Frag (&buf)[3], auto mt_, const Frag (&bf)[DT][3]) __attribute__((always_inline)) {
        constexpr int mt = decltype(mt_)::value;
#pragma unroll
        for (int q = 0; q < 6; ++q)
#pragma unroll
            for (int dt = 0; dt < DT; ++dt)
                acc[mt][dt] = __builtin_amdgcn_mfma_f32_16x16x16bf16_1k(__builtin_bit_cast(i16x4, u32x2{buf[kSixA[q]].u[0], buf[kSixA[q]].u[1]}),
                                                                         __builtin_bit_cast(i16x4, u32x2{bf[dt][kSixB[q]].u[0], bf[dt][kSixB[q]].u[1]}), acc[mt][dt], 0, 0, 0);
    };
    auto slice_step = [&](auto ap_, uint32_t abase, const Frag (&bf)[DT][3], auto &&work, auto ks_, auto late_, auto tail_) __attribute__((always_inline)) -> uint32_t {
        constexpr int AP = decltype(ap_)::value;
        constexpr bool LATE = decltype(late_)::value;
        constexpr bool TAIL16 = decltype(tail_)::value;
        uint32_t nb = 0;
        static_for<kMT>([&](auto r_) __attribute__((always_inline)) {
            constexpr int r = decltype(r_)::value;
            constexpr int K = x6_kget<r>(decltype(ks_){});
            if constexpr (r == 3) nb = slice_sync();
            if constexpr (!LATE) {
                if constexpr (r < kMT - 1) read_a(af[AP ^ ((r + 1) & 1)], abase, r + 1);
                else read_a(af[AP ^ 1], nb, 0);
                X6_SB();
            }
            if constexpr (TAIL16) mma_tile_tail(af[AP ^ (r & 1)], r_, bf); else mma_tile(af[AP ^ (r & 1)], r_, bf);
            work(r_);
            if constexpr (K > 0) X6_MIX(6 * DT, K);
            X6_SB();
            if constexpr (LATE) {
                if constexpr (r < kMT - 1) read_a(af[AP ^ ((r + 1) & 1)], abase, r + 1);
                else read_a(af[AP ^ 1], nb, 0);
                X6_SB();
            }
        });
        return nb;
    };
    using Early = std::false_type;
    using Full = std::false_type;
    using Tail16 = std::true_type;
    using LateE = std::bool_constant<TRAIN>;
    using KNone = X6K<0, 0, 0, 0, 0, 0, 0>;
    auto nowork = [](auto) __attribute__((always_inline)) {};

    const int npass = (ntiles + NW * (int)gridDim.x - 1) / (NW * (int)gridDim.x);
    auto tile_of = [&](int it) __attribute__((always_inline)) { return (it * (int)gridDim.x + (int)blockIdx.x) * NW + wave; };
    uint32_t jX = (uint32_t)j * (uint32_t)(F * 4) + (uint32_t)g * 32, l16 = (uint32_t)(j * 64 + g * 16);
    uint32_t jH = (uint32_t)j * kDropRowMul + (uint32_t)g * kDropFgMul + a.seed_lo, jK = jH + (uint32_t)g * kDropFgMul;
    asm volatile("" : "+v"(jX), "+v"(l16), "+v"(jH), "+v"(jK));
    auto load_xq = [&](f32x4 (&rw)[DT][2], int t32, int s, int q) __attribute__((always_inline)) {
        const int dt = q >> 1, h = q & 1;
        const int left = F * 4 - 128 * s - 16 * h;
        const int ng = left <= 0 ? 0 : (left + 31) >> 5;
        const uint64_t cmask = ng >= 4 ? ~0ull : ((1ull << (16 * ng)) - 1ull);
        const uint64_t m = __builtin_amdgcn_ballot_w64(j < R - t32 - 16 * dt) & cmask;
        const uint32_t vo = __builtin_amdgcn_inverse_ballot_w64(m) ? jX : kX6Oob;
        const uint32_t so = (uint32_t)(t32 + 16 * dt) * (uint32_t)(F * 4);
        rw[dt][h] = x6_load16(xsrd, vo, so + (uint32_t)(128 * s + 16 * h));
    };
    auto make_bq = [&](const f32x4 (&rw)[DT][2], int t32, int s, Frag (&bf)[DT][3], int q) __attribute__((always_inline)) {
        const int dt = q >> 1, h = q & 1;
        f32x4 v = rw[dt][h];
        if constexpr (TRAIN) {
            uint32_t w0, w1;
            drop_bits_key(jK + ((uint32_t)(t32 + 16 * dt) * kDropRowMul + (uint32_t)(8 * s + h) * kDropFgMul), a.seed_hi, w0, w1);
            v = drop4(v, w0, w1, thr, scale);
        }
        split_pack4(v, bf[dt], 2 * h);
    };
    auto bias_init = [&]() __attribute__((always_inline)) {
#pragma unroll
        for (int mt = 0; mt < kMT; ++mt) {
            const f32x4 b4 = lds4(bs_base, 64 * mt);
            acc[mt][0] = b4; acc[mt][1] = b4;
        }
    };

    {
        const int t0 = tile_of(0) * RPT;
#pragma unroll
        for (int q = 0; q < 2 * DT; ++q) { load_xq(raw[0], t0, 0, q); load_xq(raw[1], t0, n1 > 1 ? 1 : 0, q); }
#pragma unroll
        for (int q = 0; q < 2 * DT; ++q) { make_bq(raw[0], t0, 0, bfx[0], q); load_xq(raw[0], t0, n1 > 2 ? 2 : 0, q); }
    }
    bias_init();
    uint32_t abase = lane_a;
    read_a(af[0], abase, 0);
    constexpr int KX = TRAIN ? 4 : 2, KE = TRAIN ? 9 : 5;

#pragma unroll 1
    for (int it = 0; it < npass; ++it) {
        const int tile = tile_of(it), tile_next = tile_of(it + 1);
        const int t32 = tile * RPT, t32n = tile_next * RPT;
        auto store_off = [&](int layer, int dt) __attribute__((always_inline)) {
            const uint32_t rt = (uint32_t)(t32 + 16 * dt) >> 4;
            uint32_t o = rt < nrt ? l16 + (rt * (uint32_t)(kActTile * 4) + (uint32_t)layer * layer_bytes) : kX6Oob;
            asm volatile("" : "+v"(o));
            return o;
        };
        auto epilogue = [&](auto mt_, int site) __attribute__((always_inline)) {
            constexpr int mt = decltype(mt_)::value;
#pragma unroll
            for (int dt = 0; dt < DT; ++dt) {
                f32x4 h = acc[mt][dt];
                acc[mt][dt] = f32x4{0.0f, 0.0f, 0.0f, 0.0f};
#pragma unroll
                for (int c = 0; c < 4; ++c) h[c] = relu1(h[c]);
                if constexpr (TRAIN) {
                    uint32_t w0, w1;
                    drop_bits_key(jH + ((uint32_t)(t32 + 16 * dt) * kDropRowMul + (uint32_t)(4 * mt) * kDropFgMul + (uint32_t)site * kDropSiteMul), a.seed_hi, w0, w1);
                    h = drop4(h, w0, w1, thr, scale);
                }
                if constexpr (STORE) {
                    f32x4 o = h;
                    if (mt == kMT - 1 && g == 1) o[0] = 1.0f;
                    x6_store16(asrd, store_off(site - 1, dt) + X6_TSTRIDE * mt, o);
                }
                split_pack4(h, bp[mt >> 1][dt], 2 * (mt & 1));
                if (mt == kMT - 1) {
                    bp[3][dt][0].u[0] |= g == 1 ? 0x3F80u : 0u;
                }
            }
        };
        float sc[DT];
#pragma unroll
        for (int dt = 0; dt < DT; ++dt) sc[dt] = 0.0f;
        auto epilogue_out = [&](auto mt_) __attribute__((always_inline)) {
            constexpr int mt = decltype(mt_)::value;
            const f32x4 w4 = lds4(bs_base + wo_delta, 64 * mt);
            const f32x4 bn = lds4(bs_base, 64 * mt);
#pragma unroll
            for (int dt = 0; dt < DT; ++dt) {
                f32x4 h = acc[mt][dt];
                acc[mt][dt] = bn;
#pragma unroll
                for (int c = 0; c < 4; ++c) { h[c] = relu1(h[c]); sc[dt] = fmaf(h[c], w4[c], sc[dt]); }
                if constexpr (STORE) x6_store16(asrd, store_off(NL - 1, dt) + X6_TSTRIDE * mt, h);
            }
        };

        auto l1_step = [&](auto par_, int s) __attribute__((always_inline)) {
            constexpr int PAR = decltype(par_)::value;
            abase = slice_step(par_, abase, bfx[PAR], [&](auto r_) __attribute__((always_inline)) {
                constexpr int r = decltype(r_)::value;
                auto quarter = [&](int q) __attribute__((always_inline)) { make_bq(raw[PAR ^ 1], t32, s + 1, bfx[PAR ^ 1], q); load_xq(raw[PAR ^ 1], t32, s + 3 < n1 ? s + 3 : 0, q); };
                if constexpr (DT == 2) {
                    constexpr int q = r == 0 ? 0 : r == 1 ? 1 : r == 3 ? 2 : r == 4 ? 3 : -1;
                    if constexpr (q >= 0) quarter(q);
                } else {
                    if constexpr (r == 0) { quarter(0); quarter(1); } else quarter(r + 1);
                }
            }, std::conditional_t<DT == 2, X6K<KX, KX, 0, KX, KX, 0, 0>, X6K<KX, KX / 2, KX / 2, KX / 2, KX / 2, KX / 2, KX / 2>>{}, Early{}, Full{});
        };
        auto l1_last = [&](auto par_) __attribute__((always_inline)) {
            constexpr int PAR = decltype(par_)::value;
            abase = slice_step(par_, abase, bfx[PAR], [&](auto r_) __attribute__((always_inline)) {
                constexpr int r = decltype(r_)::value;
                if constexpr (r > 0) epilogue(std::integral_constant<int, r - 1>{}, 1);
            }, X6K<0, KE, KE, KE, KE, KE, KE>{}, LateE{}, Full{});
            epilogue(std::integral_constant<int, kMT - 1>{}, 1);
            if constexpr (PAR == 0) {
#pragma unroll
                for (int p = 0; p < 3; ++p) af[0][p].q = af[1][p].q;
            }
        };
        int s = 0;
        for (; s + 2 <= n1 - 1; s += 2) { l1_step(I0{}, s); l1_step(I1{}, s + 1); }
        if (s < n1 - 1) { l1_step(I0{}, s); l1_last(I1{}); } else { l1_last(I0{}); }

        auto hidden = [&](auto lastlayer_, int l) __attribute__((always_inline)) {
            constexpr bool LAST = decltype(lastlayer_)::value;
            abase = slice_step(I0{}, abase, bp[0], nowork, KNone{}, Early{}, Full{});
            abase = slice_step(I1{}, abase, bp[1], nowork, KNone{}, Early{}, Full{});
            if constexpr (LAST) {
#pragma unroll
                for (int q = 0; q < 2 * DT; ++q) { load_xq(raw[0], t32n, 0, q); load_xq(raw[1], t32n, n1 > 1 ? 1 : 0, q); }
                X6_SB();
            }
            abase = slice_step(I0{}, abase, bp[2], nowork, KNone{}, Early{}, Full{});
            if constexpr (LAST) {
                abase = slice_step(I1{}, abase, bp[3], [&](auto r_) __attribute__((always_inline)) {
                    constexpr int r = decltype(r_)::value;
                    auto quarter = [&](int q) __attribute__((always_inline)) { make_bq(raw[0], t32n, 0, bfx[0], q); load_xq(raw[0], t32n, n1 > 2 ? 2 : 0, q); };
                    if constexpr (DT == 2) { if constexpr (r < 4) quarter(r); }
                    else if constexpr (r < 4) { quarter(2 * r); quarter(2 * r + 1); }
                    if constexpr (r > 0) epilogue_out(std::integral_constant<int, r - 1>{});
                }, X6K<KX, KX + 1, KX + 1, KX + 1, 1, 1, 1>{}, LateE{}, Tail16{});
                epilogue_out(std::integral_constant<int, kMT - 1>{});
            } else {
                abase = slice_step(I1{}, abase, bp[3], [&](auto r_) __attribute__((always_inline)) {
                    constexpr int r = decltype(r_)::value;
                    if constexpr (r > 0) epilogue(std::integral_constant<int, r - 1>{}, l + 1);
                }, X6K<0, KE, KE, KE, KE, KE, KE>{}, LateE{}, Tail16{});
                epilogue(std::integral_constant<int, kMT - 1>{}, l + 1);
            }
        };
#pragma unroll 1
        for (int l = 1; l < NL - 1; ++l) hidden(std::false_type{}, l);
        hidden(std::true_type{}, NL - 1);
#pragma unroll
        for (int dt = 0; dt < DT; ++dt) {
            float t = sc[dt];
            t += __shfl_xor(t, 16, 64);
            t += __shfl_xor(t, 32, 64);
            x6_store4(psrd, (g == 0 && j < R - t32 - 16 * dt) ? (uint32_t)(t32 + 16 * dt + j) * 4u : kX6Oob, t + b_out);
        }
    }
    asm volatile("s_waitcnt vmcnt(0)" ::: "memory");
}

bool x6_supported(int F, int NL) { return F % 4 == 0 && F >= 4 && NL >= 2 && NL <= kMaxLayers && x6_lds_bytes(NL) <= 160 * 1024; }

}

extern "C" size_t ptr_mlp_x6_ws_bytes(int F, int NL) {
    return ptr::x6_supported(F, NL) ? (size_t)ptr::x6_nslices(F, NL) * ptr::kX6SliceBytes + 16384 : 0;
}

extern "C" int ptr_mlp_forward_x6(const float *X, const float *params, int R, int F, int NL, int train, float p_drop, uint64_t seed,
                                  float *preds, float *acts, void *wimg, void *stream) {
    return ptr::mlp_forward_x6_impl(X, params, R, F, NL, train, p_drop, seed, preds, acts, wimg, true, stream);
}

int ptr::mlp_forward_x6_impl(const float *X, const float *params, int R, int F, int NL, int train, float p_drop, uint64_t seed, float *preds, float *acts,
                             void *wimg, bool prep, void *stream) {
    using namespace ptr;
    const char *who = "ptr_mlp_forward_x6";
    if (R < 0 || F <= 0 || NL < 1 || NL > kMaxLayers) { set_error("%s: bad shape R=%d F=%d NL=%d", who, R, F, NL); return PTR_ERR_INVALID_ARG; }
    if (!(p_drop >= 0.0f && p_drop < 1.0f)) { set_error("%s: dropout p=%g out of [0,1)", who, (double)p_drop); return PTR_ERR_INVALID_ARG; }
    if (!x6_supported(F, NL)) { set_error("%s: F=%d NL=%d is outside the bf16x6 scorer's range (F %% 4 == 0, 2 <= NL <= 8)", who, F, NL); return PTR_ERR_UNSUPPORTED; }
    if (R > 0 && (!X || !params || !preds || !wimg || (train && !acts))) { set_error("%s: NULL pointer", who); return PTR_ERR_INVALID_ARG; }
    if ((reinterpret_cast<uintptr_t>(X) & 15) || (reinterpret_cast<uintptr_t>(wimg) & 15) || (acts && (reinterpret_cast<uintptr_t>(acts) & 15))) {
        set_error("%s: X, acts and wimg must be 16-byte aligned", who); return PTR_ERR_INVALID_ARG;
    }
    if (R == 0) return 0;
    if ((uint64_t)R * (uint64_t)F * 4 >= kX6BufLimit) {
        set_error("%s: R * F * 4 bytes of X exceed the 4 GB a buffer resource addresses (R=%d, F=%d): split the batch", who, R, F);
        return PTR_ERR_UNSUPPORTED;
    }
    if (train && (uint64_t)NL * (uint64_t)act_layer_floats(R) * 4 >= kX6BufLimit) {
        set_error("%s: NL * ceil16(R) * 448 bytes of activations exceed the 4 GB a buffer resource addresses (R=%d): split the batch", who, R);
        return PTR_ERR_UNSUPPORTED;
    }
    MlpArgs a{R, F, NL, train ? p_drop : 0.0f, (uint32_t)seed, (uint32_t)(seed >> 32)};
    hipStream_t st = as_stream(stream);
    if (prep) {
        const int nthreads = x6_nslices(F, NL) * kX6Rows * 4;
        hipLaunchKernelGGL(x6_prep_kernel, dim3((nthreads + 255) / 256), dim3(256), 0, st, params, F, NL, reinterpret_cast<uint8_t *>(wimg));
        if (int e = check_hip(hipGetLastError(), who)) return e;
    }
    const size_t lds = x6_lds_bytes(NL);
    constexpr int dt = 2, nw = 16 / dt, rpt = 16 * dt;
    const int ntiles = (R + rpt - 1) / rpt, nblk = (ntiles + nw - 1) / nw;
    const int grid = nblk < num_cus() ? nblk : num_cus();
    auto launch = [&](auto kern) -> int {
        if (int e = allow_lds(kern, lds)) return e;
        hipLaunchKernelGGL(kern, dim3(grid), dim3(nw * 64), lds, st, X, params, reinterpret_cast<const uint8_t *>(wimg), a, preds, acts);
        return check_hip(hipGetLastError(), who);
    };
    return train ? launch(mlp_fwd_x6_kernel<true, true, 2>) : launch(mlp_fwd_x6_kernel<false, false, 2>);
}
```

ptranking_amd/scorer.py:

```python
import ctypes as C
import math
import os

import torch
import torch.nn as nn

from . import _lib
from . import dp

HIDDEN = 100
ACT_LD = 112


def acts_floats(R, NL):
    return NL * ((R + 15) // 16) * 16 * ACT_LD


def alloc_acts(R, NL, device):
    return torch.empty(acts_floats(R, NL), device=device, dtype=torch.float32)


def acts_rowmajor(acts, R, NL):
    T = (R + 15) // 16
    return acts[:NL * T * 16 * ACT_LD].view(NL, T, 7, 16, 16).permute(0, 1, 3, 2, 4).reshape(NL, T * 16, ACT_LD)[:, :R]


_STACK_AF = {'R', 'LR', 'E', 'SE', 'CE', 'GE', 'S', 'T'}


def fused_kind(num_features=None, h_dim=100, out_dim=1, num_layers=3, AF='R', TL_AF='S', apply_tl_af=False, BN=True, bn_type=None,
               bn_affine=False, dropout=0.1, **_):
    if AF == 'R' and not BN and not apply_tl_af and h_dim == HIDDEN and out_dim == 1 and 1 <= num_layers <= 8:
        hidden = (num_layers - 1) * 112 * 100 + num_layers * 112 + 112 + 16
        w1 = 112 * ((num_features + 3) // 4 * 4 + 4)
        if (w1 + hidden) * 4 <= 160 * 1024:
            return 'single'
        if hidden * 4 <= 160 * 1024 and num_features % 4 == 0 and (num_features + 15) // 16 <= 48:
            return 'single'
    if AF in _STACK_AF and (not apply_tl_af or TL_AF in _STACK_AF) and (not BN or bn_type in ('BN', 'BN2')) and \
            (dropout == 0.0 or num_features % 4 == 0 or num_layers == 0):
        return 'stack'
    return None


def fusable(**kw):
    return fused_kind(**kw) is not None


X6_MIN_ROWS = 98304


def x6_mode():
    return os.environ.get("PTR_MLP_X6", "1")


X6_BUFFER_LIMIT = 0xFFFFC000


def x6_serves(X2d, R, F, NL, train):
    if X2d.data_ptr() % 16:
        return False
    if R * F * 4 >= X6_BUFFER_LIMIT:
        return False
    if train and acts_floats(R, NL) * 4 >= X6_BUFFER_LIMIT:
        return False
    return True


_X6_WS = {}
_X6_IMG_TAG = {}


def x6_image_tag(dev, F, NL):
    return _X6_IMG_TAG.get((torch.device(dev), F, NL))


def x6_set_image_tag(dev, F, NL, tag):
    _X6_IMG_TAG[(torch.device(dev), F, NL)] = tag


def x6_workspace(dev, F, NL):
    n = _lib.query("ptr_mlp_x6_ws_bytes", F, NL)
    if n == 0:
        return None
    key = (torch.device(dev), F, NL)
    ws = _X6_WS.get(key)
    if ws is None:
        ws = _X6_WS[key] = torch.empty(n, device=dev, dtype=torch.uint8)
    return ws


def x6_wimg_for(X2d, R, F, NL, train, dev):
    mode = x6_mode()
    ws = x6_workspace(dev, F, NL) if (mode == "2" or (mode != "0" and R >= X6_MIN_ROWS)) else None
    if ws is not None and not x6_serves(X2d, R, F, NL, train):
        ws = None
    return ws


def mlp_forward(X2d, flat, R, F, NL, train, p, seed, preds, acts, dev):
    ws = x6_wimg_for(X2d, R, F, NL, train, dev)
    if ws is not None:
        x6_set_image_tag(dev, F, NL, None)
        _lib.call("ptr_mlp_forward_x6", _lib.ptr(X2d), _lib.ptr(flat), R, F, NL, int(train), C.c_float(p), C.c_uint64(seed),
                  _lib.ptr(preds), _lib.ptr(acts), _lib.ptr(ws), _lib.current_stream(dev))
    else:
        _lib.call("ptr_mlp_forward", _lib.ptr(X2d), _lib.ptr(flat), R, F, NL, int(train), C.c_float(p), C.c_uint64(seed),
                  _lib.ptr(preds), _lib.ptr(acts), _lib.current_stream(dev))


class _ScorerFn(torch.autograd.Function):
    @staticmethod
    def forward(ctx, X2d, flat, F, NL, p, seed, store):
        R = X2d.shape[0]
        dev = X2d.device
        preds = torch.empty(R, device=dev, dtype=torch.float32)
        train = bool(store or p > 0.0)
        acts = alloc_acts(R, NL, dev) if train else None
        with torch.cuda.device(dev):
            mlp_forward(X2d, flat, R, F, NL, train, p, seed, preds, acts, dev)
        if store:
            ctx.save_for_backward(X2d, flat, acts)
            ctx.meta = (R, F, NL, p, seed)
        return preds

    @staticmethod
    def backward(ctx, dpreds):
        X2d, flat, acts = ctx.saved_tensors
        R, F, NL, p, seed = ctx.meta
        dev = X2d.device
        dpreds = dpreds.contiguous()
        ndz = _lib.query("ptr_mlp_backward_dz_floats", R, F, NL)
        dz = torch.empty(ndz, device=dev, dtype=torch.float32) if ndz else None
        ws = torch.empty(_lib.query("ptr_mlp_backward_ws_floats", F, NL), device=dev, dtype=torch.float32)
        grad = torch.empty_like(flat)
        with torch.cuda.device(dev):
            _lib.call("ptr_mlp_backward", _lib.ptr(X2d), _lib.ptr(flat), _lib.ptr(acts), _lib.ptr(dpreds), R, F, NL, C.c_float(p),
                      C.c_uint64(seed), _lib.ptr(dz), _lib.ptr(ws), _lib.ptr(grad), _lib.current_stream(dev))
        return None, grad, None, None, None, None, None


class FusedPointScorer(nn.Module):
    def __init__(self, num_features, num_layers=3, dropout=0.1):
        super().__init__()
        self.num_features, self.num_layers, self.dropout = int(num_features), int(num_layers), float(dropout)
        n = 100 * self.num_features + 100 + (self.num_layers - 1) * (100 * 100 + 100) + 100 + 1
        self.flat = nn.Parameter(torch.empty(n, dtype=torch.float32))
        self.reset_parameters()

    def layout(self):
        F, NL = self.num_features, self.num_layers
        out, off = [], 0
        for l in range(NL):
            k = F if l == 0 else HIDDEN
            out.append((f"ff_{l + 2}.weight", off, (HIDDEN, k))); off += HIDDEN * k
            out.append((f"ff_{l + 2}.bias", off, (HIDDEN,))); off += HIDDEN
        out.append((f"ff_{NL + 2}.weight", off, (1, HIDDEN))); off += HIDDEN
        out.append((f"ff_{NL + 2}.bias", off, (1,))); off += 1
        assert off == self.flat.numel()
        return out

    def views(self, grad=False):
        src = self.flat.grad if grad else self.flat.data
        return {k: src[o:o + math.prod(s)].view(s) for k, o, s in self.layout()}

    def reset_parameters(self):
        with torch.no_grad():
            for k, v in self.views().items():
                if k.endswith("weight"):
                    nn.init.xavier_normal_(v)
                else:
                    fan_in = self.num_features if k == "ff_2.bias" else HIDDEN
                    bound = 1.0 / math.sqrt(fan_in)
                    nn.init.uniform_(v, -bound, bound)

    def _save_to_state_dict(self, destination, prefix, keep_vars):
        for k, v in self.views().items():
            destination[prefix + k] = v if keep_vars else v.detach().clone()

    def _load_from_state_dict(self, state_dict, prefix, local_metadata, strict, missing_keys, unexpected_keys, error_msgs):
        with torch.no_grad():
            for k, v in self.views().items():
                key = prefix + k
                if key in state_dict:
                    v.copy_(state_dict[key].reshape(v.shape))
                elif strict:
                    missing_keys.append(key)
        known = {prefix + k for k, _, _ in self.layout()}
        for key in state_dict:
            if key.startswith(prefix) and key not in known and strict:
                unexpected_keys.append(key)

    def forward(self, X):
        if not X.is_cuda:
            raise RuntimeError(f"FusedPointScorer input is on {X.device}: the fused scorer runs on the MI355X HIP path only")
        lead = X.shape[:-1]
        if X.shape[-1] != self.num_features:
            raise ValueError(f"expected {self.num_features} features, got {X.shape[-1]}")
        X2d = X.reshape(-1, self.num_features)
        if X2d.dtype != torch.float32:
            X2d = X2d.float()
        X2d = X2d.contiguous()
        p = self.dropout if self.training else 0.0
        store = torch.is_grad_enabled() and self.flat.requires_grad
        seed = int(torch.randint(0, 2 ** 62, (1,)).item()) if p > 0.0 else 0
        if p > 0.0:
            seed = dp.local_dropout_seed(seed, X2d.shape[0], local_queries=lead[0] if len(lead) == 2 else None)
        preds = _ScorerFn.apply(X2d, self.flat, self.num_features, self.num_layers, p, seed, store)
        return preds.view(*lead, 1)

    def dropout_mask(self, R, site, seed):
        n_feat = self.num_features if site == 0 else HIDDEN
        out = torch.empty((R, n_feat), device=self.flat.device, dtype=torch.float32)
        _lib.call("ptr_mlp_dropout_mask", R, n_feat, site, C.c_float(self.dropout), C.c_uint64(seed), _lib.ptr(out),
                  _lib.current_stream(out.device))
        return out


class FlatAdam(torch.optim.Optimizer):

    def __init__(self, params, lr=1e-3, betas=(0.9, 0.999), eps=1e-8, weight_decay=0.0):
        super().__init__(params, dict(lr=lr, betas=betas, eps=eps, weight_decay=weight_decay))

    def _step_param(self, p, group):
        if not (p.is_cuda and p.dtype == torch.float32 and p.is_contiguous() and p.grad.is_contiguous()):
            raise RuntimeError("FlatAdam needs contiguous CUDA float32 parameters / gradients")
        st = self.state[p]
        if not st:
            st["step"] = 0
            st["exp_avg"] = torch.zeros_like(p)
            st["exp_avg_sq"] = torch.zeros_like(p)
        st["step"] += 1
        b1, b2 = group["betas"]
        with torch.cuda.device(p.device):
            _lib.call("ptr_adam_step", _lib.ptr(p), _lib.ptr(p.grad), _lib.ptr(st["exp_avg"]), _lib.ptr(st["exp_avg_sq"]),
                      C.c_int64(p.numel()), C.c_float(group["lr"]), C.c_float(b1), C.c_float(b2), C.c_float(group["eps"]),
                      C.c_float(group["weight_decay"]), int(st["step"]), _lib.current_stream(p.device))

    def fused_step_args(self, p):
        group, st = self.param_groups[0], self.state[p]
        if not st:
            st["step"] = 0
            st["exp_avg"] = torch.zeros_like(p)
            st["exp_avg_sq"] = torch.zeros_like(p)
        st["step"] += 1
        b1, b2 = group["betas"]
        self._opt_called = True
        return 1, group["lr"], b1, b2, group["eps"], group["weight_decay"], int(st["step"]), st["exp_avg"], st["exp_avg_sq"]

    @torch.no_grad()
    def step(self, closure=None):
        loss = None
        if closure is not None:
            with torch.enable_grad():
                loss = closure()
        for group in self.param_groups:
            for p in group["params"]:
                if p.grad is not None:
                    self._step_param(p, group)
        return loss

    def step_flat(self, p):
        self._step_param(p, self.param_groups[0])
        self._opt_called = True


class FlatAdagrad(FlatAdam):

    def __init__(self, params, lr=1e-2, lr_decay=0.0, eps=1e-10, weight_decay=0.0):
        torch.optim.Optimizer.__init__(self, params, dict(lr=lr, lr_decay=lr_decay, eps=eps, weight_decay=weight_decay))

    def _step_param(self, p, group):
        if not (p.is_cuda and p.dtype == torch.float32 and p.is_contiguous() and p.grad.is_contiguous()):
            raise RuntimeError("FlatAdagrad needs contiguous CUDA float32 parameters / gradients")
        st = self.state[p]
        if not st:
            st["step"] = 0
            st["sum"] = torch.zeros_like(p)
        st["step"] += 1
        with torch.cuda.device(p.device):
            _lib.call("ptr_adagrad_step", _lib.ptr(p), _lib.ptr(p.grad), _lib.ptr(st["sum"]), C.c_int64(p.numel()), C.c_float(group["lr"]),
                      C.c_float(group["lr_decay"]), C.c_float(group["eps"]), C.c_float(group["weight_decay"]), int(st["step"]),
                      _lib.current_stream(p.device))


    def fused_step_args(self, p):
        group, st = self.param_groups[0], self.state[p]
        if not st:
            st["step"] = 0
            st["sum"] = torch.zeros_like(p)
        st["step"] += 1
        self._opt_called = True
        return 2, group["lr"], group["lr_decay"], 0.0, group["eps"], group["weight_decay"], int(st["step"]), st["sum"], None


class FlatRMSprop(FlatAdam):

    def __init__(self, params, lr=1e-2, alpha=0.99, eps=1e-8, weight_decay=0.0):
        torch.optim.Optimizer.__init__(self, params, dict(lr=lr, alpha=alpha, eps=eps, weight_decay=weight_decay))

    def _step_param(self, p, group):
        if not (p.is_cuda and p.dtype == torch.float32 and p.is_contiguous() and p.grad.is_contiguous()):
            raise RuntimeError("FlatRMSprop needs contiguous CUDA float32 parameters / gradients")
        st = self.state[p]
        if not st:
            st["step"] = 0
            st["square_avg"] = torch.zeros_like(p)
        st["step"] += 1
        with torch.cuda.device(p.device):
            _lib.call("ptr_rmsprop_step", _lib.ptr(p), _lib.ptr(p.grad), _lib.ptr(st["square_avg"]), C.c_int64(p.numel()), C.c_float(group["lr"]),
                      C.c_float(group["alpha"]), C.c_float(group["eps"]), C.c_float(group["weight_decay"]), _lib.current_stream(p.device))


    def fused_step_args(self, p):
        group, st = self.param_groups[0], self.state[p]
        if not st:
            st["step"] = 0
            st["square_avg"] = torch.zeros_like(p)
        st["step"] += 1
        self._opt_called = True
        return 3, group["lr"], group["alpha"], 0.0, group["eps"], group["weight_decay"], int(st["step"]), st["square_avg"], None


FLAT_OPTIMIZERS = {'Adam': FlatAdam, 'Adagrad': FlatAdagrad, 'RMS': FlatRMSprop}


class _FlatViewMixin:

    def __init__(self, stack, **kw):
        flat, gflat = stack.flatten_parameters()
        self.stack = stack
        self.flat_param = torch.nn.Parameter(flat)
        self.flat_param.grad = gflat
        super().__init__([self.flat_param], **kw)

    def zero_grad(self, set_to_none=True):
        self.flat_param.grad.zero_()
        self.stack._grads_fresh = True

    @torch.no_grad()
    def step(self, closure=None):
        self.stack.reattach_grads()
        return super().step(closure)

    def grad_bucket(self, extra):
        n = self.flat_param.numel()
        return dp.ViewGradBucket(self.stack._gbuf, n, extra, self.zero_grad, before_reduce=self.stack.reattach_grads)


class FlatViewAdam(_FlatViewMixin, FlatAdam):
    def __init__(self, stack, lr=1e-3, betas=(0.9, 0.999), eps=1e-8, weight_decay=0.0):
        super().__init__(stack, lr=lr, betas=betas, eps=eps, weight_decay=weight_decay)


class FlatViewAdagrad(_FlatViewMixin, FlatAdagrad):
    def __init__(self, stack, lr=1e-2, lr_decay=0.0, eps=1e-10, weight_decay=0.0):
        super().__init__(stack, lr=lr, lr_decay=lr_decay, eps=eps, weight_decay=weight_decay)


class FlatViewRMSprop(_FlatViewMixin, FlatRMSprop):
    def __init__(self, stack, lr=1e-2, alpha=0.99, eps=1e-8, weight_decay=0.0):
        super().__init__(stack, lr=lr, alpha=alpha, eps=eps, weight_decay=weight_decay)


FLAT_VIEW_OPTIMIZERS = {'Adam': FlatViewAdam, 'Adagrad': FlatViewAdagrad, 'RMS': FlatViewRMSprop}


class FusedScorerMixin:

    use_fused_scorer = True
    use_flat_stack_optimizer = True

    def ini_pointsf(self, **kw):
        on_gpu = bool(getattr(self, "gpu", False)) and torch.cuda.is_available()
        kind = fused_kind(**kw) if (self.use_fused_scorer and on_gpu) else None
        if kind == 'single':
            return FusedPointScorer(kw["num_features"], num_layers=kw.get("num_layers", 3), dropout=kw.get("dropout", 0.1))
        if kind == 'stack':
            from .host import build_pointsf
            allowed = ("num_features", "h_dim", "out_dim", "num_layers", "AF", "TL_AF", "apply_tl_af", "BN", "bn_type", "bn_affine", "dropout")
            return build_pointsf(**{k: v for k, v in kw.items() if k in allowed})
        return super().ini_pointsf(**kw)

    def config_optimizer(self):
        sf = getattr(self, "point_sf", None)
        if isinstance(sf, FusedPointScorer) and self.opt in FLAT_OPTIMIZERS:
            self.optimizer = FLAT_OPTIMIZERS[self.opt](self.get_parameters(), lr=self.lr, weight_decay=self.weight_decay)
            self.scheduler = torch.optim.lr_scheduler.StepLR(self.optimizer, step_size=20, gamma=0.5)
        elif (self.opt in FLAT_VIEW_OPTIMIZERS and type(sf).__name__ == 'FusedStack' and self.use_flat_stack_optimizer
              and all(p.is_cuda and p.dtype == torch.float32 for p in sf.parameters())):
            self.optimizer = FLAT_VIEW_OPTIMIZERS[self.opt](sf, lr=self.lr, weight_decay=self.weight_decay)
            self.scheduler = torch.optim.lr_scheduler.StepLR(self.optimizer, step_size=20, gamma=0.5)
            self._dp_single = self.optimizer.flat_param
        else:
            super().config_optimizer()
```

Baseline: 5.403 million.

## Compact stored MLP activations to 104 columns per row tile

Shrinks the tiled activation buffer from 112 to 104 floats per row by storing the last 16-column feature tile as 16x8, since columns past 104 were padding. Forward stores, backward loads (including LDS DMA paths) and host helpers are updated for the new offsets, and the backward kernel zero-fills the missing columns in LDS. This cuts activation write/read traffic by about 7%, at the cost of special-case addressing for the last tile.

```diff
diff --git a/include/ptranking_amd.h b/include/ptranking_amd.h
--- a/include/ptranking_amd.h
+++ b/include/ptranking_amd.h
@@ -13,6 +13,7 @@
 #define PTR_MAX_CUTOFFS 32
 #define PTR_MAX_SUBTOPICS 32
 #define PTR_MLP_ACT_LD 112
+#define PTR_MLP_ACT_COLS 104
 
 #define PTR_ERR_INVALID_ARG 1001
 #define PTR_ERR_UNSUPPORTED 1002
@@ -135,6 +136,7 @@
 size_t ptr_mlp_backward_ws_floats(int F, int NL);
 size_t ptr_mlp_backward_dz_floats(int R, int F, int NL);
 size_t ptr_mlp_acts_floats(int R, int NL);
+size_t ptr_mlp_act_offset(int R, int layer, int row, int col);
 int ptr_mlp_forward(const float *X, const float *params, int R, int F, int NL, int train, float p_drop, uint64_t seed,
                     float *preds, float *acts, void *stream);
 int ptr_mlp_backward(const float *X, const float *params, const float *acts, const float *dpreds, int R, int F, int NL,
diff --git a/ptranking_amd/_lib.py b/ptranking_amd/_lib.py
--- a/ptranking_amd/_lib.py
+++ b/ptranking_amd/_lib.py
@@ -46,6 +46,7 @@
     "ptr_mlp_backward_ws_floats": [_i, _i],
     "ptr_mlp_backward_dz_floats": [_i, _i, _i],
     "ptr_mlp_acts_floats": [_i, _i],
+    "ptr_mlp_act_offset": [_i, _i, _i, _i],
     "ptr_mlp_forward": [_vp, _vp, _i, _i, _i, _i, _f, _u64, _vp, _vp, _vp],
     "ptr_mlp_backward": [_vp, _vp, _vp, _vp, _i, _i, _i, _f, _u64, _vp, _vp, _vp, _vp],
     "ptr_mlp_backward_step": [_vp, _vp, _vp, _vp, _i, _i, _i, _f, _u64, _vp, _vp, _vp, _i, _f, _f, _f, _f, _f, _i, _vp, _vp, _vp, _i, _vp, _vp],
@@ -82,7 +83,7 @@
     "ptr_letor_load": [C.c_char_p, _i, _f, C.c_int64, C.c_int32, C.c_int64, _vp, _i, _vp, _vp, _vp],
 }
 _RESTYPES = {"ptr_last_error": C.c_char_p, "ptr_mlp_num_params": C.c_size_t, "ptr_mlp_backward_ws_floats": C.c_size_t,
-             "ptr_mlp_backward_dz_floats": C.c_size_t, "ptr_mlp_acts_floats": C.c_size_t, "ptr_mlp_x6_ws_bytes": C.c_size_t, "ptr_linear_backward_weight_ws_floats": C.c_size_t, "ptr_bn_ws_floats": C.c_size_t,
+             "ptr_mlp_backward_dz_floats": C.c_size_t, "ptr_mlp_acts_floats": C.c_size_t, "ptr_mlp_act_offset": C.c_size_t, "ptr_mlp_x6_ws_bytes": C.c_size_t, "ptr_linear_backward_weight_ws_floats": C.c_size_t, "ptr_bn_ws_floats": C.c_size_t,
              "ptr_bn_slot_floats": C.c_size_t,
              "ptr_layernorm_backward_ws_floats": C.c_size_t}
 OPTIONAL = set()
diff --git a/ptranking_amd/csrc/ptr_mlp.h b/ptranking_amd/csrc/ptr_mlp.h
--- a/ptranking_amd/csrc/ptr_mlp.h
+++ b/ptranking_amd/csrc/ptr_mlp.h
@@ -13,11 +13,14 @@
 constexpr int kMT = 7;
 constexpr int kMaxLayers = 8;
 constexpr int kAL = 112;
-constexpr int kActTile = 16 * kAL;
+constexpr int kActCols = 104;
+constexpr int kActTile = 16 * kActCols;
+constexpr int kActLastOff = (kMT - 1) * 256;
 __host__ __device__ inline int act_row_tiles(int R) { return (R + 15) >> 4; }
 __host__ __device__ inline size_t act_layer_floats(int R) { return (size_t)act_row_tiles(R) * kActTile; }
 __host__ __device__ inline size_t act_off(int row, int col) {
-    return (size_t)(row >> 4) * kActTile + (size_t)(((col >> 4) << 8) + ((row & 15) << 4) + (col & 15));
+    const int ft = col >> 4, in = ft < kMT - 1 ? ((row & 15) << 4) + (col & 15) : ((row & 15) << 3) + (col & 7);
+    return (size_t)(row >> 4) * kActTile + (size_t)((ft << 8) + in);
 }
 
 __host__ __device__ inline size_t off_W(int l, int F) { return l == 0 ? 0 : (size_t)kH * F + kH + (size_t)(l - 1) * (kH * kH + kH); }
diff --git a/ptranking_amd/csrc/scorer.hip b/ptranking_amd/csrc/scorer.hip
--- a/ptranking_amd/csrc/scorer.hip
+++ b/ptranking_amd/csrc/scorer.hip
@@ -362,10 +362,9 @@
                 if constexpr (TRAIN) {
 #pragma unroll
                     for (int rt = 0; rt < RT; ++rt) {
-                        if (row[rt] < R16) {
-                            float *arow = acts + (size_t)(l - 1) * act_layer_floats(R) + act_off(row[rt], 0);
-                            *reinterpret_cast<f32x4 *>(arow + 256 * S + 4 * g) = S < kLast ? hin[S][rt] : tail_store(hin[S][rt][0], 1.0f);
-                        }
+                        const f32x4 sv = S < kLast ? hin[S][rt] : tail_store(hin[S][rt][0], 1.0f);
+                        if (row[rt] < R16 && (S < kLast || g < 2))
+                            *reinterpret_cast<f32x4 *>(acts + (size_t)(l - 1) * act_layer_floats(R) + act_off(row[rt], 16 * S + 4 * g)) = sv;
                     }
                     if constexpr (RT > 1) __builtin_amdgcn_sched_barrier(0);
                 }
@@ -387,10 +386,9 @@
 #pragma unroll
                 for (int c = 0; c < (mt == kMT - 1 ? 1 : 4); ++c) { h[c] = fmaxf(h[c], 0.0f); sc[rt] = fmaf(h[c], w4[c], sc[rt]); }
                 if constexpr (TRAIN) {
-                    if (row[rt] < R16) {
-                        float *arow = acts + (size_t)(NL - 1) * act_layer_floats(R) + act_off(row[rt], 0);
-                        *reinterpret_cast<f32x4 *>(arow + 256 * mt + 4 * g) = mt < kMT - 1 ? h : tail_store(h[0], 0.0f);
-                    }
+                    const f32x4 sv = mt < kMT - 1 ? h : tail_store(h[0], 0.0f);
+                    if (row[rt] < R16 && (mt < kMT - 1 || g < 2))
+                        *reinterpret_cast<f32x4 *>(acts + (size_t)(NL - 1) * act_layer_floats(R) + act_off(row[rt], 16 * mt + 4 * g)) = sv;
                 }
             }
         }
@@ -406,6 +404,9 @@
     }
 }
 
+__device__ __forceinline__ f32x4 act_ld4(const float *__restrict__ layer, int row, int col) {
+    return col < kActCols ? *reinterpret_cast<const f32x4 *>(layer + act_off(row, col)) : f32x4{0.f, 0.f, 0.f, 0.f};
+}
 __host__ __device__ inline size_t dz_lds_floats(int NL) { return (size_t)(NL - 1) * kHP * kH + (kHP + 16) + 16 * (kHP + 16); }
 
 template <int RT, int NTHR>
@@ -444,7 +445,7 @@
             dspf[rt] = dpreds[rc];
 #pragma unroll
             for (int mt = 0; mt < kMT; ++mt)
-                hpf[mt][rt] = *reinterpret_cast<const f32x4 *>(acts + (size_t)(NL - 1) * act_layer_floats(R) + act_off(rc, 16 * mt + 4 * g));
+                hpf[mt][rt] = act_ld4(acts + (size_t)(NL - 1) * act_layer_floats(R), rc, 16 * mt + 4 * g);
         }
     };
     const int tile_first = blockIdx.x * wpb + wave, tile_step = gridDim.x * wpb;
@@ -490,8 +491,7 @@
 #pragma unroll
                 for (int rt = 0; rt < RT; ++rt) {
                     const bool ok = row[rt] < R;
-                    const size_t o = (size_t)(l - 1) * act_layer_floats(R) + act_off(row[rt], 16 * mt + 4 * g);
-                    gate[mt][rt] = *reinterpret_cast<const f32x4 *>(acts + (ok ? o : 0));
+                    gate[mt][rt] = act_ld4(acts + (size_t)(l - 1) * act_layer_floats(R), ok ? row[rt] : 0, 16 * mt + 4 * g);
                 }
             f32x4 acc[kMT][RT];
 #pragma unroll
@@ -587,12 +587,12 @@
             const bool rok = !guard || r < r_end;
             const int rc = rok ? r : r_end - 1;
             const float *dzr = dZ + (size_t)rc * kAL;
-            const float *ar = SITE0 ? A + (size_t)rc * lda : A + act_off(rc, 0);
+            const float *ar = SITE0 ? A + (size_t)rc * lda : A;
 #pragma unroll
             for (int mt = 0; mt < kMT; ++mt) pa[u][mt] = dzr[fa[mt]] * ((rok & fa_ok[mt]) ? 1.0f : 0.0f);
 #pragma unroll
             for (int t = 0; t < NTW; ++t) {
-                float v = SITE0 ? ar[kb[t]] : ar[((kb[t] >> 4) << 8) + (kb[t] & 15)];
+                float v = SITE0 ? ar[kb[t]] : ar[act_off(rc, kb[t])];
                 bool keep = rok & kb_ok[t];
                 if constexpr (SITE0) keep = keep & drop_keep1(a.seed_lo, a.seed_hi, 0, rc, kb[t], thr);
                 pb[u][t] = v * (keep ? scale : 0.0f);
@@ -908,6 +908,10 @@
 }
 
 extern "C" size_t ptr_mlp_acts_floats(int R, int NL) { return R > 0 && NL > 0 ? (size_t)NL * ptr::act_layer_floats(R) : 0; }
+extern "C" size_t ptr_mlp_act_offset(int R, int layer, int row, int col) {
+    if (R <= 0 || layer < 0 || row < 0 || row >= 16 * ptr::act_row_tiles(R) || col < 0 || col >= ptr::kActCols) return (size_t)-1;
+    return (size_t)layer * ptr::act_layer_floats(R) + ptr::act_off(row, col);
+}
 extern "C" size_t ptr_mlp_backward_dz_floats(int R, int F, int NL) {
     return ptr::bwd_fused_supported(F, NL, nullptr, nullptr) ? 0 : (size_t)NL * (size_t)R * ptr::kAL;
 }
diff --git a/ptranking_amd/csrc/scorer_bwd.hip b/ptranking_amd/csrc/scorer_bwd.hip
--- a/ptranking_amd/csrc/scorer_bwd.hip
+++ b/ptranking_amd/csrc/scorer_bwd.hip
@@ -6,6 +6,8 @@
 constexpr int kBW = 8;
 constexpr int kBT = kBW * 64;
 constexpr int kSlabF = kSR * kAL;
+constexpr int kImgTile = 16 * kAL;
+__device__ inline int img_off(int row, int col) { return (row >> 4) * kImgTile + ((col >> 4) << 8) + ((row & 15) << 4) + (col & 15); }
 #define PREP_BEGIN() __builtin_amdgcn_s_setprio(2)
 #define PREP_END() __builtin_amdgcn_s_setprio(0)
 
@@ -155,6 +157,7 @@
     const float inv_keep = a.p_drop > 0.0f ? 1.0f / (1.0f - a.p_drop) : 1.0f;
 
     for (int i = tid; i < kHP; i += kBT) { wo[i] = i < kH ? P[off_wout(NL, F) + i] : 0.0f; junk_row[i] = 0.0f; }
+    for (int i = tid; i < 2 * NL * kSR * 8; i += kBT) bufA[(i >> 8) * kSlabF + img_off((i >> 3) & (kSR - 1), 104 + (i & 7))] = 0.0f;
     float wf[CH > 0 ? CH : 1][25];
     static_for<CH>([&](auto c_) {
         constexpr int c = c_, l = NL - 1 - c;
@@ -196,9 +199,11 @@
             if (k < NL * 14) {
                 const int layer = k / 14, ch = k - 14 * layer;
                 const int rt = min(2 * slab + (ch >= 7 ? 1 : 0), nrt - 1);
-                const float *src = acts + (size_t)layer * act_layer_floats(R) + (size_t)rt * kActTile + (ch >= 7 ? ch - 7 : ch) * 256 + 4 * lane_o;
-                const uint32_t dst = bufA_addr + (uint32_t)(((buf * NL + layer) * kSlabF + ch * 256) * 4);
-                glds16(src, __builtin_amdgcn_readfirstlane(dst));
+                const int ft = ch >= 7 ? ch - 7 : ch;
+                const float *src = acts + (size_t)layer * act_layer_floats(R) + (size_t)rt * kActTile + ft * 256;
+                const uint32_t dst = __builtin_amdgcn_readfirstlane(bufA_addr + (uint32_t)(((buf * NL + layer) * kSlabF + ch * 256) * 4));
+                if (ft < kMT - 1) glds16(src + 4 * lane_o, dst);
+                else if ((lane_o & 3) < 2) glds16(src + 8 * (lane_o >> 2) + 4 * (lane_o & 3), dst);
             }
         }
     };
@@ -257,7 +262,7 @@
         for (int h = 0; h < 4; ++h) {
             const int r = rs + 9 * h;
             const bool ok = rs < 9 && r < kSR;
-            pa[h] = ok ? img + (r >> 4) * kActTile + (f4 >> 2) * 256 + (r & 15) * 16 + (f4 & 3) * 4 : junk_row + 4 * f4;
+            pa[h] = ok ? img + (r >> 4) * kImgTile + (f4 >> 2) * 256 + (r & 15) * 16 + (f4 & 3) * 4 : junk_row + 4 * f4;
             h4[h] = *reinterpret_cast<const f32x4 *>(pa[h]);
             const float dsr = dsb[buf * kSR + (ok ? r : 0)];
             ds[h] = ok ? dsr : 0.0f;
@@ -301,7 +306,7 @@
                 static_for<CNT>([&](auto k_) {
                     constexpr int t = kTM<NL, NT1>.lst[WV][PH][k_];
                     constexpr int l = kTM<NL, NT1>.tl[t], n = kTM<NL, NT1>.tn[t], m = kTM<NL, NT1>.tm[t];
-                    const int kso = (ks >> 2) * kActTile + (ks & 3) * 64;
+                    const int kso = (ks >> 2) * kImgTile + (ks & 3) * 64;
                     if constexpr (kTM<NL, NT1>.first_a(WV, PH, k_))
                         av[set][l][m] = *reinterpret_cast<lds_f *>((uintptr_t)((m == kMT - 1 ? zb6[l] : zb[l]) + (uint32_t)((kso + 256 * m) * 4)));
                     if constexpr (kTM<NL, NT1>.first_b(WV, PH, k_))
@@ -370,7 +375,7 @@
                 const float *gate = cur + (l - 1) * kSlabF;
 #pragma unroll
                 for (int rt = 0; rt < kSR / 16; ++rt) {
-                    const int rbase = rt * kActTile + j * 16;
+                    const int rbase = rt * kImgTile + j * 16;
                     f32x4 b[6];
 #pragma unroll
                     for (int S = 0; S < 6; ++S) b[S] = *reinterpret_cast<const f32x4 *>(src + rbase + 256 * S + 4 * g);
@@ -415,7 +420,7 @@
                 const int idx = tid_o + 256 * u;
                 const int r = idx / (kAL / 4), c4 = idx - r * (kAL / 4);
                 if (idx < kSR * (kAL / 4) && row0 + r < R)
-                    *reinterpret_cast<f32x4 *>(dz0 + (size_t)(row0 + r) * kAL + 4 * c4) = *reinterpret_cast<const f32x4 *>(Zb + act_off(r, 4 * c4));
+                    *reinterpret_cast<f32x4 *>(dz0 + (size_t)(row0 + r) * kAL + 4 * c4) = *reinterpret_cast<const f32x4 *>(Zb + img_off(r, 4 * c4));
             }
         }
         BWD_STAMP(1 + 2 * CH);
diff --git a/ptranking_amd/csrc/scorer_bwd_x6.hip b/ptranking_amd/csrc/scorer_bwd_x6.hip
--- a/ptranking_amd/csrc/scorer_bwd_x6.hip
+++ b/ptranking_amd/csrc/scorer_bwd_x6.hip
@@ -22,6 +22,7 @@
     asm volatile("s_mov_b32 %0, m0\n\ts_mov_b32 m0, %4\n\ts_nop 0\n\tbuffer_load_dwordx4 %1, %2, %3 offen lds\n\ts_mov_b32 m0, %0"
                  : "=&s"(keep) : "v"(voff), "s"(srd), "s"(soff), "s"(lds_dst) : "memory");
 }
+constexpr uint32_t kB6Oob = 0xFFFFF000u;
 __device__ __forceinline__ uint32_t b6_opaque(uint32_t x) { asm volatile("" : "+s"(x)); return x; }
 
 template <int NT1>
@@ -150,6 +151,7 @@
     const b6_rsrc dsrd = __builtin_amdgcn_make_buffer_rsrc(const_cast<float *>(dpreds), 0, (int)((uint32_t)R * 4u), 0x00020000);
     const b6_srd asrd = b6_make_srd(acts, (uint32_t)NL * (uint32_t)(act_layer_floats(R) * 4));
     uint32_t jx = (uint32_t)j * (uint32_t)(F * 4) + (uint32_t)g * 16, j4 = (uint32_t)j * 4, l16 = (uint32_t)lane * 16;
+    if (W == kMT - 1) l16 = (lane & 3) < 2 ? (uint32_t)(32 * (lane >> 2) + 16 * (lane & 3)) : kB6Oob;
     asm volatile("" : "+v"(jx), "+v"(j4), "+v"(l16));
     auto load_x = [&](int slab) __attribute__((always_inline)) {
         const int row0 = slab * kB6S;
@@ -189,7 +191,7 @@
             const int k = chain ? W + 7 * q : 3 * 14;
             if (k < 3 * 14) {
                 const int layer = k / 14, ch = k - 14 * layer;
-                b6_bdma16(asrd, l16, (uint32_t)layer * (uint32_t)(act_layer_floats(R) * 4) + (uint32_t)row0 * (kAL * 4) + (uint32_t)ch * 1024,
+                b6_bdma16(asrd, l16, (uint32_t)layer * (uint32_t)(act_layer_floats(R) * 4) + (uint32_t)((row0 >> 4) + (q & 1)) * (kActTile * 4) + (uint32_t)W * 1024,
                           __builtin_amdgcn_readfirstlane(lds0 + (uint32_t)(kB6_ST + layer * kB6STG + ch * 1024)));
             }
         }
@@ -204,7 +206,7 @@
             const f32x4 wo4 = *reinterpret_cast<lds_f32x4 *>((uintptr_t)(b6_opaque(lds0 + (uint32_t)(kB6_WO + 64 * W)) + (uint32_t)(16 * g)));
 #pragma unroll
             for (int dt = 0; dt < 2; ++dt) {
-                const uint32_t so = b6_opaque(lds0 + (uint32_t)(kB6_ST + 1024 * W)) + (uint32_t)(j * 64 + 16 * g) + (uint32_t)(dt * kActTile * 4);
+                const uint32_t so = b6_opaque(lds0 + (uint32_t)(kB6_ST + 1024 * W)) + (uint32_t)(j * 64 + 16 * g) + (uint32_t)(dt * (kB6STG / 2));
                 const f32x4 a1 = *reinterpret_cast<lds_f32x4 *>((uintptr_t)so);
                 const f32x4 a2 = *reinterpret_cast<lds_f32x4 *>((uintptr_t)(so + kB6STG));
                 const f32x4 a3 = *reinterpret_cast<lds_f32x4 *>((uintptr_t)(so + 2 * kB6STG));
diff --git a/ptranking_amd/csrc/scorer_x6.hip b/ptranking_amd/csrc/scorer_x6.hip
--- a/ptranking_amd/csrc/scorer_x6.hip
+++ b/ptranking_amd/csrc/scorer_x6.hip
@@ -200,6 +200,8 @@
     uint32_t jX = (uint32_t)j * (uint32_t)(F * 4) + (uint32_t)g * 32, l16 = (uint32_t)(j * 64 + g * 16);
     uint32_t jH = (uint32_t)j * kDropRowMul + (uint32_t)g * kDropFgMul + a.seed_lo, jK = jH + (uint32_t)g * kDropFgMul;
     asm volatile("" : "+v"(jX), "+v"(l16), "+v"(jH), "+v"(jK));
+    uint32_t l16h = (uint32_t)(j * 32 + g * 16);
+    asm volatile("" : "+v"(l16h));
     auto load_xq = [&](f32x4 (&rw)[DT][2], int t32, int s, int q) __attribute__((always_inline)) {
         const int dt = q >> 1, h = q & 1;
         const int left = F * 4 - 128 * s - 16 * h;
@@ -250,6 +252,14 @@
             asm volatile("" : "+v"(o));
             return o;
         };
+        auto store_off_last = [&](int layer, int dt) __attribute__((always_inline)) {
+            const uint32_t rt = (uint32_t)(t32 + 16 * dt) >> 4;
+            const uint32_t l = l16h;
+            const bool in = __builtin_amdgcn_inverse_ballot_w64(rt < nrt ? 0x00000000FFFFFFFFull : 0ull);
+            uint32_t o = in ? l + (rt * (uint32_t)(kActTile * 4) + (uint32_t)layer * layer_bytes + (uint32_t)(kActLastOff * 4)) : kX6Oob;
+            asm volatile("" : "+v"(o));
+            return o;
+        };
         auto epilogue = [&](auto mt_, int site) __attribute__((always_inline)) {
             constexpr int mt = decltype(mt_)::value;
 #pragma unroll
@@ -266,7 +276,8 @@
                 if constexpr (STORE) {
                     f32x4 o = h;
                     if (mt == kMT - 1 && g == 1) o[0] = 1.0f;
-                    x6_store16(asrd, store_off(site - 1, dt) + X6_TSTRIDE * mt, o);
+                    if constexpr (mt == kMT - 1) x6_store16(asrd, store_off_last(site - 1, dt), o);
+                    else x6_store16(asrd, store_off(site - 1, dt) + X6_TSTRIDE * mt, o);
                 }
                 split_pack4(h, bp[mt >> 1][dt], 2 * (mt & 1));
                 if (mt == kMT - 1) {
@@ -287,7 +298,10 @@
                 acc[mt][dt] = bn;
 #pragma unroll
                 for (int c = 0; c < 4; ++c) { h[c] = relu1(h[c]); sc[dt] = fmaf(h[c], w4[c], sc[dt]); }
-                if constexpr (STORE) x6_store16(asrd, store_off(NL - 1, dt) + X6_TSTRIDE * mt, h);
+                if constexpr (STORE) {
+                    if constexpr (mt == kMT - 1) x6_store16(asrd, store_off_last(NL - 1, dt), h);
+                    else x6_store16(asrd, store_off(NL - 1, dt) + X6_TSTRIDE * mt, h);
+                }
             }
         };
 
@@ -391,7 +405,7 @@
         return PTR_ERR_UNSUPPORTED;
     }
     if (train && (uint64_t)NL * (uint64_t)act_layer_floats(R) * 4 >= kX6BufLimit) {
-        set_error("%s: NL * ceil16(R) * 448 bytes of activations exceed the 4 GB a buffer resource addresses (R=%d): split the batch", who, R);
+        set_error("%s: NL * ceil16(R) * 416 bytes of activations exceed the 4 GB a buffer resource addresses (R=%d): split the batch", who, R);
         return PTR_ERR_UNSUPPORTED;
     }
     MlpArgs a{R, F, NL, train ? p_drop : 0.0f, (uint32_t)seed, (uint32_t)(seed >> 32)};
diff --git a/ptranking_amd/scorer.py b/ptranking_amd/scorer.py
--- a/ptranking_amd/scorer.py
+++ b/ptranking_amd/scorer.py
@@ -10,10 +10,11 @@
 
 HIDDEN = 100
 ACT_LD = 112
+ACT_COLS = 104
 
 
 def acts_floats(R, NL):
-    return NL * ((R + 15) // 16) * 16 * ACT_LD
+    return NL * ((R + 15) // 16) * 16 * ACT_COLS
 
 
 def alloc_acts(R, NL, device):
@@ -22,7 +23,11 @@
 
 def acts_rowmajor(acts, R, NL):
     T = (R + 15) // 16
-    return acts[:NL * T * 16 * ACT_LD].view(NL, T, 7, 16, 16).permute(0, 1, 3, 2, 4).reshape(NL, T * 16, ACT_LD)[:, :R]
+    tiles = acts[:NL * T * 16 * ACT_COLS].view(NL, T, 16 * ACT_COLS)
+    out = acts.new_zeros(NL, T, 16, ACT_LD)
+    out[..., :96] = tiles[..., :6 * 256].view(NL, T, 6, 16, 16).permute(0, 1, 3, 2, 4).reshape(NL, T, 16, 96)
+    out[..., 96:ACT_COLS] = tiles[..., 6 * 256:].view(NL, T, 16, 8)
+    return out.view(NL, T * 16, ACT_LD)[:, :R]
 
 
 _STACK_AF = {'R', 'LR', 'E', 'SE', 'CE', 'GE', 'S', 'T'}
```

Result: no change. 5.426 million, median of 6 (+0.4%).
